# Lacadame/DiffSci

Hardware: AMD Instinct MI355X
Metric: samples/sec (50-step Karras Heun), PUNetG 64ch 128x128 (higher is better)
Workload: dtype f32 (3x3 convs: fp16 hi+lo split, 3 fp16 MFMA products, fp32 accumulate)

## Files before the change

diffsci_amd/_native.py:

```python
import ctypes
import os
from ctypes import POINTER, Structure, c_char_p, c_float, c_int, c_longlong, c_size_t, c_uint32, c_uint64, c_void_p

_HERE = os.path.dirname(os.path.abspath(__file__))
LIB_PATH = os.environ.get("DIFFSCI_HIP_LIB") or os.path.join(_HERE, "_lib", "libdiffsci_hip.so")

ABI_VERSION = 4
DS_IN_NETWORK, DS_IN_SCORE, DS_IN_DRIFT, DS_IN_FLOW = 0, 1, 2, 3
DS_LOAD_PLAIN, DS_LOAD_MAXPOOL2, DS_LOAD_UPSAMPLE2, DS_LOAD_AVGPOOL2 = 0, 1, 2, 3
DS_PAD_CIRCULAR = 16
DS_RES1_UPSAMPLED = 32


class EvalCoef(Structure):
    _fields_ = [("c_out", c_float), ("c_skip", c_float), ("sigma_sq", c_float),
                ("neg_mult", c_float), ("neg_lang", c_float), ("guidance", c_float),
                ("one_minus_guidance", c_float), ("input_kind", c_int), ("stochastic", c_int),
                ("scaled", c_int), ("scale", c_float), ("scale_mult", c_float), ("next_scale", c_float), ("xin_copies", c_int),
                ("nonfinite", c_void_p)]


class NativeLibraryError(RuntimeError):
    pass


_P = c_void_p
_PROTOS = {
    "ds_version": (c_int, []),
    "ds_last_error": (c_char_p, []),
    "ds_device_info": (c_int, [POINTER(c_int), POINTER(c_int), ctypes.c_char_p, c_int]),
    "ds_karras_scale": (c_int, [_P, _P, c_float, c_size_t, _P]),
    "ds_karras_drift": (c_int, [_P, _P, _P, _P, POINTER(EvalCoef), c_size_t, _P]),
    "ds_karras_score": (c_int, [_P, _P, _P, _P, POINTER(EvalCoef), c_size_t, _P]),
    "ds_philox_normal": (c_int, [_P, _P, c_uint64, c_size_t, _P]),
    "ds_karras_euler": (c_int, [_P, _P, _P, _P, _P, POINTER(EvalCoef), c_float, c_float,
                                _P, _P, c_uint64, c_float, c_float, c_size_t, _P]),
    "ds_karras_heun": (c_int, [_P, _P, _P, _P, _P, POINTER(EvalCoef), _P, _P, POINTER(EvalCoef),
                               c_float, c_float, c_size_t, _P]),
    "ds_karras_churn": (c_int, [_P, _P, _P, _P, _P, c_uint64, c_float, c_float, c_float, c_float, c_int, c_size_t, _P]),
    "ds_karras_denoiser": (c_int, [_P, _P, _P, _P, c_float, c_float, _P, _P, c_int, c_size_t, _P]),
    "ds_inorm_silu": (c_int, [_P, _P, _P, _P, c_int, c_int, c_int, c_float, c_int, _P]),
    "ds_conv2d_packed_floats": (c_size_t, [c_int, c_int, c_int]),
    "ds_conv2d_pack_weights": (c_int, [_P, _P, c_int, c_int, c_int, _P]),
    "ds_conv2d": (c_int, [_P, _P, _P, _P, _P, c_int, _P, _P, c_int, c_int, c_int, c_int, c_int,
                          c_int, c_int, _P]),
    "ds_conv2d_x6_packed_bytes": (c_size_t, [c_int, c_int]),
    "ds_conv2d_x6_pack_weights": (c_int, [_P, _P, c_int, c_int, _P]),
    "ds_conv2d_x6": (c_int, [_P, _P, _P, _P, _P, c_int, _P, _P, c_int, c_int, c_int, c_int, c_int, c_int, _P]),
    "ds_conv2d_h3_packed_bytes": (c_size_t, [c_int, c_int]),
    "ds_conv2d_h3_pack_weights": (c_int, [_P, _P, c_int, c_int, c_int, _P]),
    "ds_conv2d_h3": (c_int, [_P, _P, _P, c_int, _P, _P, c_int, _P, _P, c_int, c_int, c_int, c_int, c_int, c_int, _P, _P, _P, _P, _P]),
    "ds_absmax_rows": (c_int, [_P, _P, c_int, c_size_t, c_size_t, _P]),
    "ds_amax_merge": (c_int, [_P, _P, _P, c_int, _P]),
    "ds_absmax_channels": (c_int, [_P, _P, _P, _P, _P, c_int, c_int, c_size_t, c_int, _P]),
    "ds_input_amax": (c_int, [_P, c_int, c_int, _P, _P, _P, c_int, c_int, c_size_t, c_int, _P]),
    "ds_fill_u32": (c_int, [_P, c_uint32, c_size_t, _P]),
    "ds_conv2d_h3_up_supported": (c_int, [c_int, c_int]),
    "ds_conv2d_h3_up_packed_bytes": (c_size_t, [c_int, c_int]),
    "ds_conv2d_h3_up_pack_weights": (c_int, [_P, _P, c_int, c_int, c_int, _P]),
    "ds_conv2d_h3_up": (c_int, [_P, _P, _P, c_int, _P, _P, c_int, _P, _P, c_int, c_int, c_int, c_int, c_int, c_int, _P, _P, _P, _P, _P]),
    "ds_table_apply_images": (c_int, [_P, _P, _P, c_int, c_int, c_int, c_int, _P]),
    "ds_conv2d_h3_up_img": (c_int, [_P, _P, _P, c_int, _P, _P, c_int, _P, _P, c_int, c_int, c_int, c_int, c_int, _P, _P, _P]),
    "ds_conv_tile_count": (c_int, [c_int, c_int]),
    "ds_inorm_table": (c_int, [_P, _P, _P, _P, c_int, c_int, c_int, c_int, c_float, c_int, _P]),
    "ds_gnorm1_table": (c_int, [_P, _P, c_int, c_int, _P, c_int, c_int, _P, _P, _P, _P, c_int, c_int, c_longlong,
                                c_float, c_int, _P]),
    "ds_gnorm1_stats_tiles": (c_int, [_P, _P, c_int, c_int, _P, c_int, c_int, c_int, c_longlong, c_float, c_int, _P]),
    "ds_conv2d_direct": (c_int, [_P, _P, _P, _P, c_int, c_int, c_int, c_int, c_int, c_int, _P]),
    "ds_conv3d_direct": (c_int, [_P, _P, _P, _P, _P, c_int, _P, _P, c_int, c_int, c_int, c_int, c_int, c_int, c_int, _P]),
    "ds_volume_to_slices": (c_int, [_P, _P, c_int, c_int, c_int, c_size_t, c_int, c_int, c_int, _P]),
    "ds_slices_to_volume": (c_int, [_P, _P, _P, _P, c_int, c_int, c_int, c_size_t, c_int, _P]),
    "ds_conv_images_bytes": (c_size_t, [c_int, c_int, c_int, c_int]),
    "ds_inorm_silu_images_supported": (c_int, [c_int, c_int]),
    "ds_inorm_silu_images": (c_int, [_P, _P, _P, _P, c_int, c_int, c_int, c_int, c_float, c_int, _P]),
    "ds_conv2d_h3_img": (c_int, [_P, _P, _P, c_int, _P, _P, c_int, _P, _P, c_int, c_int, c_int, c_int, c_int, c_int, _P, _P, _P]),
    "ds_gnorm1_apply_images": (c_int, [_P, _P, _P, _P, _P, _P, _P, c_int, c_int, c_int, c_int, c_int, c_int, c_int, _P]),
    "ds_volume_stat_tiles": (c_int, [c_int, c_size_t]),
    "ds_volume_to_slices_act": (c_int, [_P, _P, _P, c_int, c_int, c_int, c_size_t, c_int, _P]),
    "ds_wrap_pad_slices": (c_int, [_P, c_int, c_int, c_int, c_size_t, _P]),
    "ds_slices_to_volume_stats": (c_int, [_P, _P, _P, _P, _P, c_int, c_int, c_int, c_size_t, c_int, _P]),
    "ds_slice_tables": (c_int, [_P, _P, _P, _P, c_int, c_int, c_int, c_int, c_longlong, c_float, c_int, c_int, _P]),
    "ds_avgpool3d": (c_int, [_P, _P, c_int, c_int, c_int, c_int, _P]),
    "ds_upsample3d": (c_int, [_P, _P, c_int, c_int, c_int, c_int, _P]),
    "ds_avgpool3d_f": (c_int, [_P, _P, c_int, c_int, c_int, c_int, c_int, _P]),
    "ds_upsample_f": (c_int, [_P, _P, c_int, c_int, c_int, c_int, c_int, c_int, _P]),
    "ds_conv1x1_h3_packed_bytes": (c_size_t, [c_int, c_int]),
    "ds_conv1x1_h3_pack_weights": (c_int, [_P, _P, c_int, c_int, c_int, _P]),
    "ds_conv1x1_h3": (c_int, [_P, _P, _P, c_int, _P, _P, c_int, _P, _P, c_int, c_int, c_int, c_int, c_int, c_int, _P, _P, _P, c_int, _P]),
    "ds_attention": (c_int, [_P, _P, c_int, c_int, c_int, _P]),
    "ds_attention_generic": (c_int, [_P, _P, c_int, c_int, c_int, _P]),
    "ds_attention_h3": (c_int, [_P, _P, c_int, c_int, c_int, _P, _P, _P]),
    "ds_attention_h3_workspace_bytes": (c_size_t, [c_int, c_int, c_int]),
    "ds_attention_h3_ws": (c_int, [_P, _P, _P, c_int, c_int, c_int, _P, _P, _P]),
    "ds_attention_h3_heads_workspace_bytes": (c_size_t, [c_int, c_int, c_int, c_int]),
    "ds_attention_h3_heads": (c_int, [_P, _P, _P, c_int, c_int, c_int, c_int, _P, _P, _P]),
    "ds_attention_heads_generic": (c_int, [_P, _P, c_int, c_int, c_int, c_int, _P]),
    "ds_token_l2_normalize": (c_int, [_P, c_int, c_int, c_int, c_int, c_int, c_float, c_float, _P]),
    "ds_linear": (c_int, [_P, _P, _P, _P, c_int, c_int, c_int, c_int, _P]),
    "ds_fourier_features": (c_int, [_P, _P, _P, _P, c_int, c_int, c_int, _P]),
    "ds_fourier_channels": (c_int, [_P, _P, _P, c_int, c_int, c_int, c_size_t, _P]),
    "ds_gnorm1_workspace_bytes": (c_size_t, [c_int]),
    "ds_gnorm1_stats": (c_int, [_P, _P, _P, c_int, c_int, c_int, c_float, c_int, _P]),
    "ds_gnorm1_apply": (c_int, [_P, _P, _P, _P, _P, _P, _P, c_int, c_int, c_int, c_int, c_int, c_int, c_int, _P]),
    "ds_gnorm1_apply_poolf": (c_int, [_P, _P, _P, _P, _P, _P, _P, c_int, c_int, c_int, c_int, c_int, c_int, c_int, _P]),
    "ds_concat2": (c_int, [_P, _P, _P, c_int, c_size_t, c_size_t, _P]),
    "ds_add_act": (c_int, [_P, _P, _P, c_int, c_int, c_int, c_int, _P]),
    "ds_mask_blend": (c_int, [_P, _P, _P, _P, c_size_t, c_int, _P]),
    "ds_axpby": (c_int, [_P, _P, c_float, _P, c_float, c_size_t, _P]),
    "ds_div_scalar": (c_int, [_P, _P, c_float, c_size_t, _P]),
    "ds_batchnorm_eval": (c_int, [_P, _P, _P, _P, _P, _P, c_float, c_float, c_int, c_int, c_int, c_int, c_size_t, _P]),
    "ds_lerp_stack": (c_int, [_P, _P, _P, c_int, c_size_t, _P]),
    "ds_add": (c_int, [_P, _P, _P, c_size_t, _P]),
    "ds_graph_begin_capture": (c_int, [_P]),
    "ds_graph_end_capture": (c_int, [_P, POINTER(_P), POINTER(c_int)]),
    "ds_graph_launch": (c_int, [_P, _P]),
    "ds_graph_destroy": (c_int, [_P]),
}

_lib = None


def exported_symbols():
    return sorted(_PROTOS)


def lib():
    global _lib
    if _lib is not None:
        return _lib
    if not os.path.exists(LIB_PATH):
        raise NativeLibraryError(
            f"{LIB_PATH} is missing: diffsci_amd has no CPU or PyTorch fallback. "
            "Run `python build.py` (needs hipcc; cross-compiles for gfx950 without a GPU).")
    try:
        L = ctypes.CDLL(LIB_PATH)
    except OSError as e:
        raise NativeLibraryError(f"cannot load {LIB_PATH}: {e}") from e
    for name, (res, args) in _PROTOS.items():
        try:
            fn = getattr(L, name)
        except AttributeError as e:
            raise NativeLibraryError(f"{LIB_PATH} does not export {name}; rebuild with build.py") from e
        fn.restype = res
        fn.argtypes = args
    if L.ds_version() != ABI_VERSION:
        raise NativeLibraryError(f"ABI version {L.ds_version()} != {ABI_VERSION}; rebuild with build.py")
    _lib = L
    return L


def check(rc, what):
    if rc != 0:
        msg = lib().ds_last_error().decode("utf-8", "replace")
        raise RuntimeError(f"{what} failed (status {rc}): {msg}")
```

diffsci_amd/csrc/ds_conv3h.hip:

```cpp
#include "ds_common.h"
#include <cstring>
#include "ds_conv3h_args.h"

#ifdef DS_STAMP
unsigned long long* g_stamps = nullptr;
#define STAMP_SLOTS 16
#define STAMP_AT(slot) a.stamps[((size_t)(blockIdx.z * gridDim.y + blockIdx.y) * gridDim.x + blockIdx.x) * STAMP_SLOTS + (slot)]
#define STAMP(slot) do { if (threadIdx.x == 0) STAMP_AT(slot) = __builtin_amdgcn_s_memrealtime(); } while (0)
#define STAMP_CLK(slot) do { if (threadIdx.x == 0) STAMP_AT(slot) = __builtin_amdgcn_s_memtime(); } while (0)
#define STAMP_PLACE() do { if (threadIdx.x == 0) { STAMP_AT(8) = __builtin_amdgcn_s_getreg((31 << 11) | 4); STAMP_AT(9) = __builtin_amdgcn_s_getreg((31 << 11) | 20); } } while (0)
#else
#define STAMP(slot) do {} while (0)
#define STAMP_CLK(slot) do {} while (0)
#define STAMP_PLACE() do {} while (0)
#endif

namespace {

using namespace ds_conv3;

template <int MT> struct Frags { f16x8 a[2][MT]; f16x8 b[2][2]; };

template <int MODE, bool W16, bool PRE, bool CIRC, int NW, bool S16 = false, bool IMGIN = false, bool TWO = false, bool VEC = false>
__global__ __launch_bounds__(64 * NW, TWO ? 2 : NW / 2) void k_conv3h(const Conv3hArgs a) {
// ... 385 lines not shown
    }
  };

  if constexpr (!IMGIN && !PRE) __builtin_amdgcn_sched_barrier(0);
  const unsigned amax_bits = ds_epi::act_bits((IMGIN || PRE) ? nullptr : a.in_amax, b);
  if constexpr (IMGIN) x_dma(0, 0); else
  x_fetch(0);
  rows_fetch(0);
  const float bias_shift = ds_epi::fetch_bias_shift(a.bias, a.shift, a.shift_stride, b, (cot + (TWO ? (tid >> 7) & 1 : 0)) * COT, a.Cout, COTS);
  w_fetch(0, 0);
  if (n_steps > 1) w_fetch(1, 1);
  STAMP(1);
  if constexpr (!IMGIN && !PRE) __builtin_amdgcn_sched_barrier(0);
  ascale = ds_epi::act_scale_of(PRE ? 0u : amax_bits, a.wshift);
  if constexpr (VEC && PRE) {
    typedef const __attribute__((address_space(4))) f32x4* cptr;
    const float inv0 = ((cptr)(reinterpret_cast<const f32x4*>(pre_b)))[0][3];
    ascale.inv_scale = inv0 == 0.f ? 1.0f : inv0;
    rows_park(0);
    __syncthreads();
  }
  if constexpr (!IMGIN) x_store(0);
  ds_epi::commit_bias_shift(BS, bias_shift, COTS);
  __syncthreads();
  STAMP(2);
  STAMP_CLK(6);

  f32x4 acc16[M16][4];
  if constexpr (S16) {
#pragma unroll
    for (int m = 0; m < M16; ++m)
#pragma unroll
      for (int n = 0; n < 4; ++n)
#pragma unroll
        for (int q = 0; q < 4; ++q) acc16[m][n][q] = 0.f;
    const int i16 = lane & 15, h16 = (lane >> 4) & 1;
    const bool tapB = lane >= 32;
    const int wlane = h16 * COT + i16 + 32 * mh + cw * WSLAB_VEC;
    int xlane[4];
#pragma unroll
    for (int n = 0; n < 4; ++n)
      xlane[n] = h16 * HS + (wave_row + ROWS_PER_R * (n >> 1)) * PW + (W16 ? (n & 1) * PW + i16 : 16 * (n & 1) + i16);
    struct F16 { f16x8 a[2][M16]; f16x8 b[2][4]; };
    auto pair = [&](int slotA, int kyA, int kxA, int xbA, int slotB, int kyB, int kxB, int xbB) __attribute__((always_inline)) {
      const int wofs = (tapB ? slotB * WSV + kxB * 2 * COT : slotA * WSV + kxA * 2 * COT) + wlane;
      const int xofs = tapB ? xbB * XBV + kyB * PW + kxB : xbA * XBV + kyA * PW + kxA;
      F16 f;
#pragma unroll
      for (int p = 0; p < 2; ++p) {
#pragma unroll
        for (int m = 0; m < M16; ++m) f.a[p][m] = *reinterpret_cast<const f16x8*>(&Ws[wofs + p * 6 * COT + 16 * m]);
#pragma unroll
        for (int n = 0; n < 4; ++n) f.b[p][n] = *reinterpret_cast<const f16x8*>(&Xs[xofs + p * PS + xlane[n]]);
      }
      constexpr int PA[3] = {1, 0, 0};
      constexpr int PB[3] = {0, 1, 0};
#pragma unroll
      for (int t = 0; t < 3; ++t)
#pragma unroll
        for (int m = 0; m < M16; ++m)
#pragma unroll
          for (int n = 0; n < 4; ++n)
            acc16[m][n] = __builtin_amdgcn_mfma_f32_16x16x32_f16(f.a[PA[t]][m], f.b[PB[t]][n], acc16[m][n], 0, 0, 0);
    };
    const bool early_stage = a.two_early != 0;
    auto stage_in = [&](int chunk, int ky) __attribute__((always_inline)) {
      const int g = chunk * 3 + ky;
      if (g + 2 < n_steps) w_fetch(g + 2, (ky + 2) % 3);
#ifdef DS_STAMP
      const bool fetch = !a.no_stage;
#else
      constexpr bool fetch = true;
#endif
      if constexpr (IMGIN) {
        if (ky == 0 && chunk + 1 < a.n_chunks) x_dma(chunk + 1, (chunk + 1) & 1);
      } else
      if (fetch && ky == 0 && chunk + 1 < a.n_chunks) { rows_fetch(chunk + 1); x_fetch(chunk + 1); }
      if constexpr (TWO && !IMGIN) {
        if (early_stage && wv < 4 && fetch && ky == 1 && chunk + 1 < a.n_chunks) x_store((chunk & 1) ^ 1);
      }
      __builtin_amdgcn_sched_barrier(0);
    };
    auto stage_out = [&](int chunk, int ky, int xbuf) __attribute__((always_inline)) {
      __builtin_amdgcn_sched_barrier(0);
#ifdef DS_STAMP
      const bool store = a.no_stage != 1;
#else
      constexpr bool store = true;
#endif
      if constexpr (!IMGIN) {
        if (store && ky == 0 && chunk + 1 < a.n_chunks) rows_park(xbuf ^ 1);
        if (store && ky == 1 && chunk + 1 < a.n_chunks && !(TWO && early_stage && wv < 4)) x_store(xbuf ^ 1);
      }
      __syncthreads();
    };
    for (int chunk = 0; chunk < a.n_chunks; chunk += 2) {
      stage_in(chunk, 0);     pair(0, 0, 0, 0, 0, 0, 1, 0); pair(0, 0, 2, 0, 1, 1, 0, 0);   stage_out(chunk, 0, 0);
      stage_in(chunk, 1);     pair(1, 1, 1, 0, 1, 1, 2, 0);                                 stage_out(chunk, 1, 0);
      stage_in(chunk, 2);     pair(2, 2, 0, 0, 2, 2, 1, 0); pair(2, 2, 2, 0, 0, 0, 0, 1);   stage_out(chunk, 2, 0);
      stage_in(chunk + 1, 0); pair(0, 0, 1, 1, 0, 0, 2, 1);                                 stage_out(chunk + 1, 0, 1);
      stage_in(chunk + 1, 1); pair(1, 1, 0, 1, 1, 1, 1, 1); pair(1, 1, 2, 1, 2, 2, 0, 1);   stage_out(chunk + 1, 1, 1);
      stage_in(chunk + 1, 2); pair(2, 2, 1, 1, 2, 2, 2, 1);                                 stage_out(chunk + 1, 2, 1);
    }
  } else {
  FragsT fA, fB;
  frag_load(fA, 0, 0, 0, 0);

  auto step = [&](FragsT& cur, FragsT& oth, int chunk, int ky, int xbuf) __attribute__((always_inline)) {
    const int g = chunk * 3 + ky;
    const int slot = ky;
    const bool more_chunks = chunk + 1 < a.n_chunks;
    if (g + 2 < n_steps) w_fetch(g + 2, (ky + 2) % 3);
    if (ky == 0 && more_chunks) x_fetch(chunk + 1);
    __builtin_amdgcn_sched_barrier(0);
    frag_load(oth, slot, xbuf, ky, 1);
    frag_mma(cur);
    reads_between_mfmas();
    __builtin_amdgcn_sched_barrier(0);
    frag_load(cur, slot, xbuf, ky, 2);
    frag_mma(oth);
    reads_between_mfmas();
    __builtin_amdgcn_sched_barrier(0);
    if (g + 1 < n_steps) {
      const int nky = ky == 2 ? 0 : ky + 1;
      frag_load(oth, nky, ky == 2 ? xbuf ^ 1 : xbuf, nky, 0);
    }
    frag_mma(cur);
    if (g + 1 < n_steps) reads_between_mfmas();
    __builtin_amdgcn_sched_barrier(0);
    if (ky == 1 && more_chunks) x_store(xbuf ^ 1);
    __syncthreads();
  };

  int chunk = 0;
  for (; chunk + 1 < a.n_chunks; chunk += 2) {
    step(fA, fB, chunk, 0, 0);
    step(fB, fA, chunk, 1, 0);
    step(fA, fB, chunk, 2, 0);
    step(fB, fA, chunk + 1, 0, 1);
    step(fA, fB, chunk + 1, 1, 1);
    step(fB, fA, chunk + 1, 2, 1);
  }
  if (chunk < a.n_chunks) {
    step(fA, fB, chunk, 0, 0);
    step(fB, fA, chunk, 1, 0);
    step(fA, fB, chunk, 2, 0);
  }

  }
  STAMP(3);
  STAMP_CLK(7);
  {
    ds_epi::Args e;
    e.out = a.out; e.bias = a.bias; e.shift = a.shift; e.res1 = a.res1; e.res2 = a.res2; e.res1_up = a.res1_up;
    e.unscale = PRE ? ds_epi::unscale_from_inv(ascale.inv_scale, a.wshift) : ds_epi::unscale_from_in(ascale.in_scale, a.wshift);
    e.shift_stride = a.shift_stride;
    e.out_amax = a.out_amax ? a.out_amax + b : nullptr;
    e.b = b; e.co_base = (cot + cw) * COT + 32 * mh; e.y0 = y0 + wave_row; e.x0 = x0;
    e.Cout = a.Cout; e.H = a.H; e.W = a.W;
    e.tile_stats = a.tile_stats; e.tile = ty * a.tiles_x + tx; e.ntiles = a.tiles_x * a.tiles_y;
    constexpr int WTILE = 32 * MT * 2 * 32;
    float* tile = reinterpret_cast<float*>(smem) + wv * WTILE;
    if constexpr (S16) {
      ds_epi::store_tile16<W16, MT>(acc16, tile, BS + 32 * mh + 128 * cw, e);
    } else {
      ds_epi::store_tile<W16, MT>(acc, tile, BS + 32 * mh, e);
    }
    if (a.tile_stats) {
      __syncthreads();
      if constexpr (TWO) {
        if (tid < 128) {
          e.co_base = (cot + (tid >> 6)) * COT;
          ds_epi::store_tile_stats<2>(reinterpret_cast<const float*>(smem) + (tid >> 6) * 4 * WTILE, WTILE, e, tid & 63);
        }
      } else {
        e.co_base = cot * COT;
        ds_epi::store_tile_stats<MT>(reinterpret_cast<const float*>(smem), WTILE, e);
      }
    }
  }
#ifdef DS_STAMP
  STAMP(4);
  asm volatile("s_waitcnt vmcnt(0)" ::: "memory");
  STAMP(5);
#endif
}

__global__ void k_pack3h(_Float16* packed, const float* __restrict__ w, int Cout, int Cin, int n_chunks, float scale,
                         size_t total) {
  size_t i = (size_t)blockIdx.x * blockDim.x + threadIdx.x;
  if (i >= total) return;
  size_t t = i;
  const int c8 = t % 8; t /= 8;
  const int co64 = t % COT; t /= COT;
  const int h = t % 2; t /= 2;
  const int kx = t % 3; t /= 3;
  const int piece = t % 2; t /= 2;
  const int ky = t % 3; t /= 3;
  const int chunk = t % n_chunks; t /= n_chunks;
  const int cot = (int)t;
  const int co = cot * COT + co64, ci = chunk * KC + 8 * h + c8;
  float v = 0.f;
  if (co < Cout && ci < Cin) v = w[((size_t)co * Cin + ci) * 9 + ky * 3 + kx] * scale;
  const _Float16 hi = (_Float16)v;
  const _Float16 lo = (_Float16)(v - (float)hi);
  packed[i] = piece == 0 ? hi : lo;
}

template <int MODE, bool W16, bool PRE, bool CIRC, int NW, bool S16 = false, bool IMGIN = false, bool TWO = false, bool VEC = false>
int launch_conv3h_w(const Conv3hArgs& a, hipStream_t s) {
  constexpr int LDSB = TWO ? LDS_BYTES_TWO : (S16 ? LDS_BYTES16 : LDS_BYTES);
  {
    const int rc = ds::ensure_dynamic_lds<&k_conv3h<MODE, W16, PRE, CIRC, NW, S16, IMGIN, TWO, VEC>>(LDSB, "hipFuncSetAttribute(conv3h)");
    if (rc != DS_OK) return rc;
  }
  const long long tiles = (long long)a.tiles_y * a.tiles_x;
  DS_REQUIRE(tiles > 0 && tiles < 65536 && a.B < 65536, DS_ERR_SHAPE,
             "ds_conv2d_h3: %lld pixel tiles x %d samples exceed the grid limits (65535 each)", tiles, a.B);
  hipLaunchKernelGGL((k_conv3h<MODE, W16, PRE, CIRC, NW, S16, IMGIN, TWO, VEC>), dim3((unsigned)(TWO ? a.n_cot / 2 : a.n_cot), (unsigned)tiles, (unsigned)a.B),
                     dim3(64 * NW), LDSB, s, a);
  DS_CHECK_LAUNCH("ds_conv2d_h3");
  return DS_OK;
}

inline bool conv3h_shape16() {
  static const bool on = [] { const char* e = getenv("DS_CONV_SHAPE"); return !(e && atoi(e) == 32); }();
  return on;
}

inline int conv3h_waves(bool pre) {
  static const int forced = [] { const char* e = getenv("DS_CONV_WAVES"); const int v = e ? atoi(e) : 0; return (v == 4 || v == 8) ? v : 0; }();
  return forced ? forced : (pre ? 8 : 4);
}

inline int conv3h_waves16() {
  static const int v = [] { const char* e = getenv("DS_CONV_WAVES16"); return (e && atoi(e) == 8) ? 8 : 4; }();
  return v;
}

inline int conv3h_two() {
  static const int v = [] { const char* e = getenv("DS_CONV_TWO"); return e ? atoi(e) : 1; }();
  return v;
}
inline long long conv3h_two_min() {
  static const long long v = [] { const char* e = getenv("DS_CONV_TWO_MIN"); return e ? atoll(e) : 256ll; }();
  return v;
}

inline bool conv3h_vec() {
  static const bool on = [] { const char* e = getenv("DS_CONV_VEC"); return !(e && atoi(e) == 0); }();
  return on;
}

template <int MODE, bool W16, bool PRE, bool CIRC>
int launch_conv3h_c(const Conv3hArgs& a, hipStream_t s) {
  bool vec = false;
  if constexpr (MODE == DS_LOAD_PLAIN && !W16)
    vec = conv3h_vec() && a.W % 32 == 0 && a.ox == 0 && a.Cin % KC == 0 && (reinterpret_cast<uintptr_t>(a.in) & 15u) == 0;
  if constexpr (MODE == DS_LOAD_PLAIN) {
    const int two = conv3h_two();
    if (conv3h_shape16() && a.n_chunks % 2 == 0 && a.n_cot % 2 == 0 && ((two == 1 && PRE && a.n_cot == 2 && (long long)a.tiles_y * a.tiles_x * a.B >= conv3h_two_min()) || two == 2)) {
      if constexpr (!W16) { if (vec) return launch_conv3h_w<MODE, W16, PRE, CIRC, 8, true, false, true, true>(a, s); }
      return launch_conv3h_w<MODE, W16, PRE, CIRC, 8, true, false, true>(a, s);
    }
  }
  if (conv3h_shape16() && a.n_chunks % 2 == 0) {
    if constexpr (PRE && MODE == DS_LOAD_PLAIN) {
      if (conv3h_waves16() == 8 && a.n_chunks <= 8) return launch_conv3h_w<MODE, W16, PRE, CIRC, 8, true>(a, s);
    }
    if constexpr (MODE == DS_LOAD_PLAIN && !W16) { if (vec) return launch_conv3h_w<MODE, W16, PRE, CIRC, 4, true, false, false, true>(a, s); }
    return launch_conv3h_w<MODE, W16, PRE, CIRC, 4, true>(a, s);
  }
  if constexpr (MODE == DS_LOAD_MAXPOOL2) return launch_conv3h_w<MODE, W16, PRE, CIRC, 4>(a, s);
  else return conv3h_waves(PRE) == 8 ? launch_conv3h_w<MODE, W16, PRE, CIRC, 8>(a, s) : launch_conv3h_w<MODE, W16, PRE, CIRC, 4>(a, s);
}

template <int MODE, bool W16, bool PRE>
int launch_conv3h(const Conv3hArgs& a, hipStream_t s) {
  return a.circular ? launch_conv3h_c<MODE, W16, PRE, true>(a, s) : launch_conv3h_c<MODE, W16, PRE, false>(a, s);
}

}

extern "C" {

size_t ds_conv2d_h3_packed_bytes(int Cout, int Cin) {
  if (Cout <= 0 || Cin <= 0) return 0;
  const size_t n_cot = (Cout + COT - 1) / COT, n_chunks = (Cin + KC - 1) / KC;
  return n_cot * n_chunks * 3 * (size_t)WSLAB_VEC * 16;
}

int ds_conv2d_h3_pack_weights(void* packed, const float* w, int Cout, int Cin, int wshift, void* stream) {
  DS_REQUIRE(packed && w, DS_ERR_NULL, "ds_conv2d_h3_pack_weights: NULL pointer");
  DS_REQUIRE(Cout > 0 && Cin > 0, DS_ERR_SHAPE, "ds_conv2d_h3_pack_weights: Cout=%d Cin=%d", Cout, Cin);
  DS_REQUIRE(wshift >= -40 && wshift <= 40, DS_ERR_SHAPE, "ds_conv2d_h3_pack_weights: wshift %d out of range", wshift);
  const int n_chunks = (Cin + KC - 1) / KC;
  const size_t total = ds_conv2d_h3_packed_bytes(Cout, Cin) / 2;
  hipLaunchKernelGGL(k_pack3h, dim3((unsigned)((total + 255) / 256)), dim3(256), 0, ds::as_stream(stream),
                     reinterpret_cast<_Float16*>(packed), w, Cout, Cin, n_chunks, ldexpf(1.0f, wshift), total);
  DS_CHECK_LAUNCH("ds_conv2d_h3_pack_weights");
  return DS_OK;
}

int ds_conv2d_h3(float* out, const float* in, const void* w_packed, int wshift, const float* bias, const float* shift,
                 int shift_stride, const float* res1, const float* res2, int B, int Cin, int Cout, int H, int W,
                 int load_mode, const float* prenorm, float* tile_stats, const unsigned* in_amax, unsigned* out_amax,
                 void* stream) {
  DS_REQUIRE(out && in && w_packed, DS_ERR_NULL, "ds_conv2d_h3: NULL pointer");
  DS_REQUIRE(!(prenorm && in_amax), DS_ERR_UNSUPPORTED, "ds_conv2d_h3: in_amax is for raw inputs (with prenorm the table's fourth column carries the exponent)");
  DS_REQUIRE(B >= 0 && Cin > 0 && Cout > 0 && H > 0 && W > 0, DS_ERR_SHAPE,
             "ds_conv2d_h3: bad shape B=%d Cin=%d Cout=%d H=%d W=%d", B, Cin, Cout, H, W);
  const int circular = (load_mode & DS_PAD_CIRCULAR) ? 1 : 0;
  const int res1_up = (load_mode & DS_RES1_UPSAMPLED) ? 1 : 0;
  const int oy = (int)((load_mode >> 8) & 15) - (((load_mode >> 8) & 8) ? 16 : 0);
  const int ox = (int)((load_mode >> 12) & 15) - (((load_mode >> 12) & 8) ? 16 : 0);
  load_mode &= ~(DS_PAD_CIRCULAR | DS_RES1_UPSAMPLED | 0xff00);
  DS_REQUIRE(!circular || (H >= (oy < 0 ? -oy : oy) + 1 && W >= (ox < 0 ? -ox : ox) + 1), DS_ERR_SHAPE,
             "ds_conv2d_h3: periodic padding with tap offset (%d, %d) needs a field at least as large as the window's reach (%d x %d)", oy, ox, H, W);
  DS_REQUIRE(!res1_up || (res1 && H % 2 == 0 && W % 2 == 0), DS_ERR_SHAPE, "ds_conv2d_h3: RES1_UPSAMPLED needs res1 and even H, W");
  DS_REQUIRE(load_mode >= 0 && load_mode <= 2, DS_ERR_UNSUPPORTED, "ds_conv2d_h3: load_mode %d", load_mode);
  DS_REQUIRE(load_mode != DS_LOAD_UPSAMPLE2 || (H % 2 == 0 && W % 2 == 0), DS_ERR_SHAPE,
             "ds_conv2d_h3: UPSAMPLE2 needs even output H, W (got %d x %d)", H, W);
  DS_REQUIRE(shift == nullptr || shift_stride == 0 || shift_stride >= Cout, DS_ERR_SHAPE,
             "ds_conv2d_h3: shift_stride %d < Cout %d", shift_stride, Cout);
  DS_REQUIRE((reinterpret_cast<uintptr_t>(w_packed) & 15u) == 0, DS_ERR_SHAPE, "ds_conv2d_h3: w_packed must be 16-byte aligned");
  DS_REQUIRE(load_mode != DS_LOAD_MAXPOOL2 || (reinterpret_cast<uintptr_t>(in) & 7u) == 0, DS_ERR_SHAPE,
             "ds_conv2d_h3: MAXPOOL2 input must be 8-byte aligned");
  DS_REQUIRE(wshift >= -40 && wshift <= 40, DS_ERR_SHAPE, "ds_conv2d_h3: wshift %d out of range", wshift);
  DS_REQUIRE(prenorm == nullptr || load_mode != DS_LOAD_MAXPOOL2, DS_ERR_UNSUPPORTED,
             "ds_conv2d_h3: prenorm cannot be combined with the max-pool load (pooling follows the activation)");
  DS_REQUIRE((reinterpret_cast<uintptr_t>(prenorm) & 15u) == 0, DS_ERR_SHAPE, "ds_conv2d_h3: prenorm must be 16-byte aligned");
  if (B == 0) return DS_OK;
  Conv3hArgs a;
  a.prenorm = prenorm; a.tile_stats = tile_stats; a.circular = circular; a.res1_up = res1_up; a.oy = oy; a.ox = ox;
  a.ntiles_magic40 = 0; a.ncot_magic40 = 0; a.pc_prio = 0; a.pc_skew_mask = 0;
  {
    static const int early = [] { const char* e = getenv("DS_CONV_TWO_EARLY"); return e ? atoi(e) : 1; }();
    a.two_early = early;
  }
  a.out = out; a.in = in; a.wp = reinterpret_cast<const u32x4*>(w_packed); a.bias = bias; a.shift = shift;
  a.res1 = res1; a.res2 = res2; a.shift_stride = shift_stride;
  a.wshift = wshift; a.in_amax = in_amax; a.out_amax = out_amax;
  a.B = B; a.Cin = Cin; a.Cout = Cout; a.H = H; a.W = W;
  a.Hin = load_mode == DS_LOAD_MAXPOOL2 ? 2 * H : (load_mode == DS_LOAD_UPSAMPLE2 ? H / 2 : H);
  a.Win = load_mode == DS_LOAD_MAXPOOL2 ? 2 * W : (load_mode == DS_LOAD_UPSAMPLE2 ? W / 2 : W);
  DS_REQUIRE((long long)Cin * a.Hin * a.Win < (1ll << 31), DS_ERR_SHAPE, "ds_conv2d_h3: per-sample input exceeds 2^31 floats");
  const long long pad32 = (long long)((W + 31) / 32 * 32) * ((H + 7) / 8 * 8);
  const long long pad16 = (long long)((W + 15) / 16 * 16) * ((H + 15) / 16 * 16);
  const bool w16 = pad16 < pad32;
  const int TW = w16 ? 16 : 32, TH = w16 ? 16 : 8;
  a.tiles_x = (W + TW - 1) / TW; a.tiles_y = (H + TH - 1) / TH;
  a.n_cot = (Cout + COT - 1) / COT;
  a.n_chunks = (Cin + KC - 1) / KC;
  a.tiles_x_magic = a.tiles_x == 1 ? 0u : (unsigned)((1ull << 32) / (unsigned)a.tiles_x) + 1u;
#ifdef DS_STAMP
  {
    static const struct Stg { unsigned ticks = 0, lo = 256, hi = 512; Stg() { const char* e = getenv("DS_CONV_STAGGER"); if (e) sscanf(e, "%u,%u,%u", &ticks, &lo, &hi); } } stg;
    a.stagger_ticks = stg.ticks; a.stagger_lo = stg.lo; a.stagger_hi = stg.hi;
    static const unsigned nostage = [] { const char* e = getenv("DS_CONV_NOSTAGE"); return e ? (unsigned)atoi(e) : 0u; }();
    a.no_stage = nostage;
  }
#endif
#ifdef DS_STAMP
  a.stamps = g_stamps;
#endif
  hipStream_t s = ds::as_stream(stream);
  if (!w16 && load_mode == DS_LOAD_PLAIN && conv3h_shape16()) {
    bool launched = false;
    const int rc = conv3p_try_launch(a, s, &launched);
    if (rc != DS_OK || launched) return rc;
  }
#define DS_L3(M, W) (prenorm ? launch_conv3h<M, W, true>(a, s) : launch_conv3h<M, W, false>(a, s))
  if (w16) {
    if (load_mode == DS_LOAD_PLAIN) return DS_L3(DS_LOAD_PLAIN, true);
    if (load_mode == DS_LOAD_MAXPOOL2) return launch_conv3h<DS_LOAD_MAXPOOL2, true, false>(a, s);
    return DS_L3(DS_LOAD_UPSAMPLE2, true);
  }
  if (load_mode == DS_LOAD_PLAIN) return DS_L3(DS_LOAD_PLAIN, false);
  if (load_mode == DS_LOAD_MAXPOOL2) return launch_conv3h<DS_LOAD_MAXPOOL2, false, false>(a, s);
  return DS_L3(DS_LOAD_UPSAMPLE2, false);
#undef DS_L3
}

size_t ds_conv_images_bytes(int B, int C, int H, int W) {
  if (B <= 0 || C <= 0 || H <= 0 || W <= 0) return 0;
  return (size_t)B * ((C + KC - 1) / KC) * 4 * (size_t)(H + 2) * (W + 2) * 16;
}

int ds_conv2d_h3_img(float* out, const void* images, const void* w_packed, int wshift, const float* bias, const float* shift,
                     int shift_stride, const float* res1, const float* res2, int B, int Cin, int Cout, int H, int W,
                     int flags, float* tile_stats, unsigned* out_amax, void* stream) {
  DS_REQUIRE(out && images && w_packed, DS_ERR_NULL, "ds_conv2d_h3_img: NULL pointer");
  DS_REQUIRE((flags & ~DS_RES1_UPSAMPLED) == 0, DS_ERR_UNSUPPORTED, "ds_conv2d_h3_img: flags %d (DS_RES1_UPSAMPLED only)", flags);
  DS_REQUIRE(!(flags & DS_RES1_UPSAMPLED) || (res1 && H % 2 == 0 && W % 2 == 0 && (reinterpret_cast<uintptr_t>(res1) & 7u) == 0),
             DS_ERR_SHAPE, "ds_conv2d_h3_img: RES1_UPSAMPLED needs res1 [B, Cout, H/2, W/2] (8-byte aligned) and even H, W");
  DS_REQUIRE(B >= 0 && Cin > 0 && Cout > 0 && H > 0 && W > 0, DS_ERR_SHAPE,
             "ds_conv2d_h3_img: bad shape B=%d Cin=%d Cout=%d H=%d W=%d", B, Cin, Cout, H, W);
  DS_REQUIRE(((Cin + KC - 1) / KC) % 2 == 0, DS_ERR_UNSUPPORTED,
             "ds_conv2d_h3_img: the image-input kernel is the 16x16x32 variant: an even number of 16-channel chunks (Cin = %d)", Cin);
  DS_REQUIRE(shift == nullptr || shift_stride == 0 || shift_stride >= Cout, DS_ERR_SHAPE,
             "ds_conv2d_h3_img: shift_stride %d < Cout %d", shift_stride, Cout);
  DS_REQUIRE((reinterpret_cast<uintptr_t>(w_packed) & 15u) == 0 && (reinterpret_cast<uintptr_t>(images) & 15u) == 0, DS_ERR_SHAPE,
             "ds_conv2d_h3_img: images and w_packed must be 16-byte aligned");
  DS_REQUIRE(wshift >= -40 && wshift <= 40, DS_ERR_SHAPE, "ds_conv2d_h3_img: wshift %d out of range", wshift);
  DS_REQUIRE((long long)4 * (H + 2) * (W + 2) < (1ll << 27), DS_ERR_SHAPE, "ds_conv2d_h3_img: image planes too large");
  if (B == 0) return DS_OK;
  Conv3hArgs a;
  memset(&a, 0, sizeof(a));
  a.out = out; a.in = reinterpret_cast<const float*>(images); a.wp = reinterpret_cast<const u32x4*>(w_packed);
  a.bias = bias; a.shift = shift; a.res1 = res1; a.res2 = res2; a.shift_stride = shift_stride; a.tile_stats = tile_stats;
  a.res1_up = (flags & DS_RES1_UPSAMPLED) ? 1 : 0;
  a.wshift = wshift; a.out_amax = out_amax;
  a.B = B; a.Cin = Cin; a.Cout = Cout; a.H = H; a.W = W; a.Hin = H; a.Win = W;
  const long long pad32 = (long long)((W + 31) / 32 * 32) * ((H + 7) / 8 * 8);
  const long long pad16 = (long long)((W + 15) / 16 * 16) * ((H + 15) / 16 * 16);
  const bool w16 = pad16 < pad32;
  const int TW = w16 ? 16 : 32, TH = w16 ? 16 : 8;
  a.tiles_x = (W + TW - 1) / TW; a.tiles_y = (H + TH - 1) / TH;
  a.n_cot = (Cout + COT - 1) / COT;
  a.n_chunks = (Cin + KC - 1) / KC;
  a.tiles_x_magic = a.tiles_x == 1 ? 0u : (unsigned)((1ull << 32) / (unsigned)a.tiles_x) + 1u;
#ifdef DS_STAMP
  a.stamps = g_stamps;
#endif
  hipStream_t s = ds::as_stream(stream);
  if (!w16) {
    bool launched = false;
    const int rc = conv3p_try_launch_img(a, s, &launched);
    if (rc != DS_OK || launched) return rc;
  }
  return w16 ? launch_conv3h_w<DS_LOAD_PLAIN, true, false, false, 4, true, true>(a, s)
             : launch_conv3h_w<DS_LOAD_PLAIN, false, false, false, 4, true, true>(a, s);
}

}
```

diffsci_amd/csrc/ds_conv3h_args.h:

```cpp
#pragma once
#include "ds_common.h"
#include "ds_conv_epilogue.h"
#include "ds_h3_common.h"

namespace ds_conv3 {

using ds_epi::f32x16;
using ds_epi::f32x4;
using ds_h3::u32x4;
using ds_h3::f16x8;
using ds_h3::split2;
using ds_h3::fast_silu;

constexpr int COT = 64, NT = 256;
constexpr int KC = 16;
template <bool W16> struct Geo {
  static constexpr int TH = W16 ? 16 : 8, TW = W16 ? 16 : 32;
  static constexpr int PH = TH + 2, PW = TW + 2, NPOS = PH * PW;
  static constexpr int XITEMS = 2 * NPOS;
  static constexpr int XBUF_VEC = 2 * 2 * NPOS;
};
constexpr int XBUF_VEC = Geo<false>::XBUF_VEC;
constexpr int HPAD16 = 12;
constexpr int XBUF_VEC16 = XBUF_VEC + 2 * HPAD16;
constexpr int WSLAB_VEC = 2 * 3 * 2 * COT;
constexpr int WPIECES = WSLAB_VEC / 64;
constexpr int STAGE_BYTES = (2 * XBUF_VEC + 3 * WSLAB_VEC) * 16;
constexpr int LDS_BYTES = STAGE_BYTES + 128 * 4;
constexpr int STAGE_BYTES16 = (2 * XBUF_VEC16 + 3 * WSLAB_VEC) * 16;
constexpr int LDS_BYTES16 = STAGE_BYTES16 + 128 * 4;
static_assert(2 * LDS_BYTES16 <= 160 * 1024, "two workgroups per CU");
constexpr int TWO_STAGE_BYTES = (2 * XBUF_VEC16 + 3 * 2 * WSLAB_VEC) * 16;
constexpr int TWO_EPI_BYTES = 8 * 64 * 2 * 32 * 4;
static_assert(TWO_EPI_BYTES >= TWO_STAGE_BYTES, "bias / shift rows behind the larger of the two");
constexpr int LDS_BYTES_TWO = TWO_EPI_BYTES + 2 * 128 * 4;

struct Conv3hArgs {
  float* out;
  const float* in;
  const u32x4* wp;
  const float* bias;
  const float* shift;
  const float* res1;
  const float* res2;
  const float* prenorm;
  float* tile_stats;
  const unsigned* in_amax;
  unsigned* out_amax;
  int wshift;
  int shift_stride;
  int res1_up;
  int circular;
  int oy, ox;
  int B, Cin, Cout, H, W, Hin, Win;
  int tiles_x, tiles_y, n_cot, n_chunks;
  unsigned tiles_x_magic;
  unsigned long long ntiles_magic40, ncot_magic40;
  int pc_prio;
  int pc_skew_mask;
  int two_early;
#ifdef DS_STAMP
  unsigned long long* stamps;
  unsigned stagger_lo, stagger_hi, stagger_ticks;
  unsigned no_stage;
#endif
};


int conv3p_try_launch(const Conv3hArgs& a, hipStream_t s, bool* launched);
int conv3p_try_launch_img(const Conv3hArgs& a, hipStream_t s, bool* launched);

}
```

diffsci_amd/csrc/ds_conv3p.hip:

```cpp
#include "ds_conv3h_args.h"

#include <atomic>
#include <cstdlib>
#include <type_traits>

namespace ds_conv3 {
namespace {

constexpr int P_WOFF = 2 * XBUF_VEC16 * 16;
constexpr int P_WSLOTS = 4;
constexpr int P_OUTOFF = P_WOFF + P_WSLOTS * WSLAB_VEC * 16;
constexpr int P_BSOFF = P_OUTOFF + 4 * 16384;
constexpr int P_BS_FLOATS = 132;
constexpr int P_LDS = P_BSOFF + 2 * P_BS_FLOATS * 4;
static_assert(P_LDS <= 160 * 1024, "one workgroup per CU");

#ifdef DS_STAMP
#define PSTAMP_SLOTS 64
#define PSTAMP(slot) do { if (a.stamps && (wv == 0 || wv == 4) && lane == 0 && (slot) < PSTAMP_SLOTS) a.stamps[((size_t)blockIdx.x * 2 + (wv >> 2)) * PSTAMP_SLOTS + (slot)] = __builtin_amdgcn_s_memtime(); } while (0)
#else
#define PSTAMP(slot) do {} while (0)
#endif
#ifdef DS_STAMP
#define PSTAMP_FINE(k) do { if (it == 1 && last_of_item) PSTAMP(48 + (k)); } while (0)
#else
#define PSTAMP_FINE(k) do {} while (0)
#endif

#define DS_VMCNT_CASE(n) case n: asm volatile("s_waitcnt vmcnt(" #n ")" ::: "memory"); break;
__device__ __forceinline__ void bar_counted(int young) {
  const int y = __builtin_amdgcn_readfirstlane(young);
  switch (y < 63 ? y : 63) {
    DS_VMCNT_CASE(0) DS_VMCNT_CASE(1) DS_VMCNT_CASE(2) DS_VMCNT_CASE(3) DS_VMCNT_CASE(4) DS_VMCNT_CASE(5) DS_VMCNT_CASE(6) DS_VMCNT_CASE(7)
    DS_VMCNT_CASE(8) DS_VMCNT_CASE(9) DS_VMCNT_CASE(10) DS_VMCNT_CASE(11) DS_VMCNT_CASE(12) DS_VMCNT_CASE(13) DS_VMCNT_CASE(14) DS_VMCNT_CASE(15)
    DS_VMCNT_CASE(16) DS_VMCNT_CASE(17) DS_VMCNT_CASE(18) DS_VMCNT_CASE(19) DS_VMCNT_CASE(20) DS_VMCNT_CASE(21) DS_VMCNT_CASE(22) DS_VMCNT_CASE(23)
    DS_VMCNT_CASE(24) DS_VMCNT_CASE(25) DS_VMCNT_CASE(26) DS_VMCNT_CASE(27) DS_VMCNT_CASE(28) DS_VMCNT_CASE(29) DS_VMCNT_CASE(30) DS_VMCNT_CASE(31)
    DS_VMCNT_CASE(32) DS_VMCNT_CASE(33) DS_VMCNT_CASE(34) DS_VMCNT_CASE(35) DS_VMCNT_CASE(36) DS_VMCNT_CASE(37) DS_VMCNT_CASE(38) DS_VMCNT_CASE(39)
    DS_VMCNT_CASE(40) DS_VMCNT_CASE(41) DS_VMCNT_CASE(42) DS_VMCNT_CASE(43) DS_VMCNT_CASE(44) DS_VMCNT_CASE(45) DS_VMCNT_CASE(46) DS_VMCNT_CASE(47)
    DS_VMCNT_CASE(48) DS_VMCNT_CASE(49) DS_VMCNT_CASE(50) DS_VMCNT_CASE(51) DS_VMCNT_CASE(52) DS_VMCNT_CASE(53) DS_VMCNT_CASE(54) DS_VMCNT_CASE(55)
    DS_VMCNT_CASE(56) DS_VMCNT_CASE(57) DS_VMCNT_CASE(58) DS_VMCNT_CASE(59) DS_VMCNT_CASE(60) DS_VMCNT_CASE(61) DS_VMCNT_CASE(62)
    default: asm volatile("s_waitcnt vmcnt(63)" ::: "memory"); break;
  }
  asm volatile("s_waitcnt lgkmcnt(0)\n\ts_barrier" ::: "memory");
}
#undef DS_VMCNT_CASE

struct Item { int cot, b, y0, x0, tile; };
#ifndef DS_PC_FETCH_LATE
#define DS_PC_FETCH_LATE 0
#endif
#ifndef DS_PC_SPREAD
#define DS_PC_SPREAD 1
#endif
#ifndef DS_PC_IMG_CDMA
#define DS_PC_IMG_CDMA 0
#endif
#ifndef DS_PC_CDMA
#define DS_PC_CDMA 1
#endif
#define DS_LPI 8

template <int XI> struct Packed { u32x4 h[XI], l[XI]; };
template <int BK> struct ResRegs { f32x4 r1[BK], r2[BK]; };
struct Frag { f16x8 a[2][4], b[2][4]; };

__device__ __forceinline__ void lds_dma16(const void* gsrc, unsigned lane_bytes, unsigned lds) {
  asm volatile("s_mov_b32 m0, %0\n\ts_nop 0\n\tglobal_load_lds_dwordx4 %1, %2" : : "s"(lds), "v"(lane_bytes), "s"(gsrc) : "memory", "m0");
}
__device__ __forceinline__ unsigned lds_address(const void* p) {
  return (unsigned)(unsigned long long)(const __attribute__((address_space(3))) void*)p;
}
__device__ __forceinline__ unsigned const_u32(const void* p, size_t i) {
  typedef const __attribute__((address_space(4))) unsigned* cptr;
  return ((cptr)p)[i];
}

template <bool PRE, bool CIRC, int NRES, int NPW, bool VEC = false, bool IMG = false>
__global__ __launch_bounds__(256 + 64 * NPW, NPW == 4 ? 2 : 3) void k_conv3p(const Conv3hArgs a) {
  static_assert(NPW == 4 || NPW == 8, "four or eight producer waves");
  static_assert(!VEC || NPW == 4, "16-byte patch loads: the four-producer form");
  static_assert(!IMG || (!PRE && !CIRC && !VEC && NPW == 4), "image input: plain zero-padded four-producer form");
  constexpr int XI = NPW == 4 ? 3 : 2;
  constexpr int BK = NPW == 4 ? 4 : 2;
  using Packed = ds_conv3::Packed<XI>;
  using ResRegs = ds_conv3::ResRegs<BK>;
  constexpr int PW = Geo<false>::PW, NPOS = Geo<false>::NPOS;
  constexpr int HS = NPOS + HPAD16, PS = 2 * NPOS + HPAD16, XBV = XBUF_VEC16;
  extern __shared__ __attribute__((aligned(16))) unsigned char smem[];
  u32x4* Xs = reinterpret_cast<u32x4*>(smem);
  u32x4* Ws = reinterpret_cast<u32x4*>(smem + P_WOFF);
  float* OUT = reinterpret_cast<float*>(smem + P_OUTOFF);
  float* BS = reinterpret_cast<float*>(smem + P_BSOFF);
  const int tid = threadIdx.x, lane = tid & 63;
  const int wv = __builtin_amdgcn_readfirstlane(tid >> 6);
  const bool consumer = wv < 4;
  const int rw = wv & 3;
  const int ptid = tid - 256;
  const int pw = wv - 4;
  const int rws = NPW == 4 ? rw : ((pw >> 1) & 3);
  const int joff = NPW == 4 ? 0 : 8 * (pw & 1);

  const unsigned ntiles = (unsigned)(a.tiles_x * a.tiles_y);
  const unsigned total = (unsigned)a.n_cot * ntiles * (unsigned)a.B;
  const unsigned Q = gridDim.x >> 3, xcd = blockIdx.x & 7u, q = blockIdx.x >> 3;
  const unsigned per = total >> 3, rem = total & 7u;
  const unsigned first = xcd * per + (xcd < rem ? xcd : rem), cnt = per + (xcd < rem ? 1u : 0u);
  const int n_items = q < cnt ? (int)((cnt - q + Q - 1) / Q) : 0;
  if (n_items == 0) return;
  auto div40 = [](unsigned n, unsigned long long magic) __attribute__((always_inline)) { return (unsigned)(((unsigned long long)n * magic) >> 40); };
  auto item_of = [&](int k) __attribute__((always_inline)) {
    const unsigned logical = first + q + Q * (unsigned)k;
    Item it;
    const unsigned rest = div40(logical, a.ncot_magic40);
    it.cot = (int)(logical - rest * (unsigned)a.n_cot);
    const unsigned bb = div40(rest, a.ntiles_magic40);
    it.tile = (int)(rest - bb * ntiles);
    it.b = (int)bb;
    const int ty = a.tiles_x == 1 ? it.tile : (int)__umulhi((unsigned)it.tile, a.tiles_x_magic);
    const int tx = it.tile - ty * a.tiles_x;
    it.y0 = 8 * ty; it.x0 = 32 * tx;
    return it;
  };
  const int n_chunks = a.n_chunks, n_steps = 3 * n_chunks;
  const int HW = a.H * a.W;

  f32x4 acc[4][4];
  const int i16 = lane & 15, h16 = (lane >> 4) & 1, g16 = lane >> 4;
  const bool tapB = lane >= 32;
  const int wlane = h16 * COT + i16;
  int xlane[4];
#pragma unroll
  for (int n = 0; n < 4; ++n) xlane[n] = h16 * HS + (2 * rw + (n >> 1)) * PW + 16 * (n & 1) + i16;
  auto load_pair = [&](Frag& f, int slotA, int kyA, int kxA, int xbA, int slotB, int kyB, int kxB, int xbB) __attribute__((always_inline)) {
    const int wofs = (tapB ? slotB * WSLAB_VEC + kxB * 2 * COT : slotA * WSLAB_VEC + kxA * 2 * COT) + wlane;
    const int xofs = tapB ? xbB * XBV + kyB * PW + kxB : xbA * XBV + kyA * PW + kxA;
#pragma unroll
    for (int p = 0; p < 2; ++p) {
#pragma unroll
      for (int m = 0; m < 4; ++m) f.a[p][m] = *reinterpret_cast<const f16x8*>(&Ws[wofs + p * 6 * COT + 16 * m]);
#pragma unroll
      for (int n = 0; n < 4; ++n) f.b[p][n] = *reinterpret_cast<const f16x8*>(&Xs[xofs + p * PS + xlane[n]]);
    }
  };
  auto mma_pair = [&](const Frag& f) __attribute__((always_inline)) {
    constexpr int PA[3] = {1, 0, 0};
    constexpr int PB[3] = {0, 1, 0};
#pragma unroll
    for (int t = 0; t < 3; ++t)
#pragma unroll
      for (int m = 0; m < 4; ++m)
#pragma unroll
        for (int n = 0; n < 4; ++n)
          acc[m][n] = __builtin_amdgcn_mfma_f32_16x16x32_f16(f.a[PA[t]][m], f.b[PB[t]][n], acc[m][n], 0, 0, 0);
  };
  auto reads_between = [&]() __attribute__((always_inline)) {
    __builtin_amdgcn_sched_group_barrier(0x008, 16, 0);
#pragma unroll
    for (int i = 0; i < 16; ++i) {
      __builtin_amdgcn_sched_group_barrier(0x008, 1, 0);
      __builtin_amdgcn_sched_group_barrier(0x100, 1, 0);
    }
    __builtin_amdgcn_sched_group_barrier(0x008, 16, 0);
  };
  auto park_tile = [&](int par) __attribute__((always_inline)) {
    const float* bs = BS + par * P_BS_FLOATS;
    float* tile = OUT + rw * 4096;
    const float unscale = bs[128];
    float bsv[4][4];
#pragma unroll
    for (int m = 0; m < 4; ++m)
#pragma unroll
      for (int e = 0; e < 4; ++e) {
        const int co = 16 * m + 4 * g16 + e;
        bsv[m][e] = bs[co] + bs[64 + co];
      }
    __builtin_amdgcn_sched_barrier(0);
#pragma unroll
    for (int m = 0; m < 4; ++m)
#pragma unroll
      for (int e = 0; e < 4; ++e) {
        const int co = 16 * m + 4 * g16 + e;
#pragma unroll
        for (int n = 0; n < 4; ++n) {
          tile[(co * 2 + (n >> 1)) * 32 + 16 * (n & 1) + i16] = __builtin_fmaf(acc[m][n][e], unscale, bsv[m][e]);
          acc[m][n][e] = 0.f;
        }
      }
  };

  const int tail_h = (rw >> 1) & 1;
  auto item_h = [&](int i) __attribute__((always_inline)) { return NPW == 8 ? ((pw >> 2) & 1) : (i == 0 ? 0 : (i == 1 ? 1 : tail_h)); };
  int xlds[XI], xrow[XI], xcol[XI];
  const bool live_tail = NPW == 4 ? (NT + (ptid & (NT / 2 - 1)) < NPOS) : (lane < 21);
  auto live = [&](int i) __attribute__((always_inline)) { return i < XI - 1 || live_tail; };
#pragma unroll
  for (int i = 0; i < XI; ++i) {
    int pos;
    if (NPW == 4) pos = i < 2 ? (ptid & 255) : NT + (ptid & (NT / 2 - 1));
    else pos = i == 0 ? 64 * (pw & 3) + lane : 256 + 21 * (pw & 3) + (lane < 21 ? lane : 20);
    xrow[i] = pos / PW;
    xcol[i] = pos - xrow[i] * PW;
    xlds[i] = item_h(i) * HS + pos;
  }
  int vr[XI], vx[XI], vch[XI], vlds[XI], vrow[XI];
  const bool halo_live = lane < 20;
  if constexpr (VEC) {
#pragma unroll
    for (int i = 0; i < XI; ++i) {
      vr[i] = 0; vx[i] = 0; vch[i] = 0; vlds[i] = 0; vrow[i] = 0;
      if (i < XI - 1 || pw < 2) {
        const int u = i * 256 + (ptid & 255);
        const int q = u & 3, G = u >> 5;
        const int h = G >= 10 ? 1 : 0, Gp = G - 10 * h;
        int r, g;
        if (Gp < 8) { r = 4 * (Gp >> 2) + ((u >> 3) & 3); g = 2 * (Gp & 3) + ((u >> 2) & 1); }
        else { r = 8 + ((u >> 3) & 1); g = 4 * (Gp - 8) + 2 * ((u >> 4) & 1) + ((u >> 2) & 1); }
        vr[i] = r; vx[i] = 4 * g;
        vch[i] = (8 * h + 2 * q) * HW;
        vlds[i] = 16 * (h * HS + r * PW + 1 + 4 * g) + 4 * q;
        vrow[i] = 8 * h + 2 * q;
      } else {
        const int e = halo_live ? lane : 19, h = pw - 2;
        vr[i] = e >> 1; vx[i] = (e & 1) ? PW - 2 : -1;
        vch[i] = 8 * h * HW;
        vlds[i] = 16 * (h * HS + vr[i] * PW + vx[i] + 1);
        vrow[i] = 8 * h;
      }
    }
  }
  auto pad_vec = [&](int c) __attribute__((always_inline)) { return c < HPAD16 ? NPOS + c : PS + NPOS + (c - HPAD16); };
  constexpr int NINST = (XBV + 63) / 64;
  const int Wp = a.W + 2, Hp = a.H + 2;
  unsigned dbase[6] = {};
  if constexpr (IMG) {
#pragma unroll
    for (int i = 0; i < 6; ++i) {
      const int k = pw + 4 * i;
      const int L = (k < NINST - 1 ? 64 * k : XBV - 64) + lane;
      const int piece = L >= PS ? 1 : 0, Lp = L - piece * PS;
      const int hh = Lp >= HS ? 1 : 0;
      int pos = Lp - hh * HS;
      pos = pos < NPOS ? pos : NPOS - 1;
      const int r = pos / PW, col = pos - r * PW;
      dbase[i] = 16u * (unsigned)(((2 * piece + hh) * Hp + r) * Wp + col);
    }
  }
  int i_k = 0, i_chunk = 0, i_b = 0;
  unsigned i_off = 0;
  auto xdma = [&](int buf) __attribute__((always_inline)) {
    const bool valid = i_k < n_items;
    if (valid && i_chunk == 0) { const Item it = item_of(i_k); i_off = 16u * (unsigned)(it.y0 * Wp + it.x0); i_b = it.b; }
    const u32x4* src = reinterpret_cast<const u32x4*>(a.in) + ((size_t)i_b * n_chunks + i_chunk) * 4 * (size_t)(Hp * Wp);
    u32x4* dst = Xs + buf * XBV;
    int n = 0;
#pragma unroll
    for (int i = 0; i < 6; ++i) {
      const int k = pw + 4 * i;
      if (k < NINST) { lds_dma16(src, dbase[i] + i_off, lds_address(dst + (k < NINST - 1 ? 64 * k : XBV - 64))); ++n; }
    }
    if (valid && ++i_chunk == n_chunks) { i_chunk = 0; ++i_k; }
    return n;
  };
  int f_k = 0, f_chunk = 0, f_b = 0;
  int xoff[XI] = {};
  unsigned f_xvalid = 0;
  float f_in_scale = 1.f;
  auto plan_fetch = [&](const Item& it) __attribute__((always_inline)) {
    f_xvalid = 0;
    if constexpr (VEC) {
#pragma unroll
      for (int i = 0; i < XI; ++i) {
        const bool halo = i == XI - 1 && pw >= 2;
        int gy = it.y0 + vr[i] - 1 + a.oy, gx = it.x0 + vx[i];
        if (CIRC) {
          gy = gy < 0 ? gy + a.H : (gy >= a.H ? gy - a.H : gy);
          gx = gx < 0 ? gx + a.W : (gx >= a.W ? gx - a.W : gx);
          gy = gy >= a.H ? a.H - 1 : gy;
        }
        const bool ok = (!halo || halo_live) && gy >= 0 && gy < a.H && gx >= 0 && gx < a.W;
        xoff[i] = ok ? gy * a.W + gx : 0;
        if (ok) f_xvalid |= 1u << i;
      }
      f_b = it.b;
      if constexpr (!PRE) f_in_scale = ds_epi::act_scale_of(a.in_amax ? const_u32(a.in_amax, it.b) : 0u, a.wshift).in_scale;
      return;
    }
#pragma unroll
    for (int i = 0; i < XI; ++i) {
      int gy = it.y0 + xrow[i] - 1 + a.oy, gx = it.x0 + xcol[i] - 1 + a.ox;
      if (CIRC) {
        gy = gy < 0 ? gy + a.H : (gy >= a.H ? gy - a.H : gy);
        gx = gx < 0 ? gx + a.W : (gx >= a.W ? gx - a.W : gx);
        gy = gy >= a.H ? a.H - 1 : gy;
        gx = gx >= a.W ? a.W - 1 : gx;
      }
      const bool ok = live(i) && gy >= 0 && gy < a.H && gx >= 0 && gx < a.W;
      xoff[i] = ok ? gy * a.W + gx : 0;
      if (ok) f_xvalid |= 1u << i;
    }
    f_b = it.b;
    if constexpr (!PRE) f_in_scale = ds_epi::act_scale_of(a.in_amax ? const_u32(a.in_amax, it.b) : 0u, a.wshift).in_scale;
  };
  const float* f_src = a.in;
  auto fetch_begin = [&](unsigned& tag, int& trow, float& tscale) __attribute__((always_inline)) {
    const bool valid = f_k < n_items;
    if (valid && f_chunk == 0) plan_fetch(item_of(f_k));
    tag = valid ? (0x80000000u | f_xvalid) : 0u;
    trow = (f_b * n_chunks + f_chunk) * KC;
    tscale = f_in_scale;
    f_src = a.in + ((size_t)f_b * a.Cin + (size_t)f_chunk * KC) * HW;
    if (valid && ++f_chunk == n_chunks) { f_chunk = 0; ++f_k; }
  };
  auto fetch_item = [&](auto halo_tag, float (&xr)[XI][8], int i) __attribute__((always_inline)) {
    constexpr bool HALO = decltype(halo_tag)::value;
    if constexpr (VEC) {
      const float* p0 = f_src + vch[i] + xoff[i];
      if (HALO && i == XI - 1) {
#pragma unroll
        for (int k = 0; k < 8; ++k) xr[i][k] = p0[(size_t)k * HW];
      } else {
        const f32x4 t0 = *reinterpret_cast<const f32x4*>(p0);
        const f32x4 t1 = *reinterpret_cast<const f32x4*>(p0 + HW);
#pragma unroll
        for (int k = 0; k < 4; ++k) { xr[i][k] = t0[k]; xr[i][4 + k] = t1[k]; }
      }
    } else {
      const float* p0 = f_src + xoff[i] + (size_t)(8 * item_h(i)) * HW;
#pragma unroll
      for (int k = 0; k < 8; ++k) xr[i][k] = p0[(size_t)k * HW];
    }
  };
  auto fetch_count = [&](auto halo_tag) __attribute__((always_inline)) {
    constexpr bool HALO = decltype(halo_tag)::value;
    return VEC ? (PRE ? 1 : 0) + (HALO ? 2 * (XI - 1) + 8 : 2 * XI) : DS_LPI * XI;
  };
  auto rows_fetch = [&](f32x4& prow, int trow) __attribute__((always_inline)) {
    if constexpr (VEC && PRE) prow = reinterpret_cast<const f32x4*>(a.prenorm)[trow + (lane & 15)];
  };
  auto rows_park = [&](const f32x4& prow, int buf) __attribute__((always_inline)) {
    if constexpr (VEC && PRE) {
      if (pw == 0 && lane < 16) Xs[buf * XBV + pad_vec(lane)] = __builtin_bit_cast(u32x4, prow);
    }
  };
  auto fetch = [&](auto halo_tag, float (&xr)[XI][8], f32x4& prow, unsigned& tag, int& trow, float& tscale) __attribute__((always_inline)) {
    fetch_begin(tag, trow, tscale);
    rows_fetch(prow, trow);
#pragma unroll
    for (int i = 0; i < XI; ++i) fetch_item(halo_tag, xr, i);
    return fetch_count(halo_tag);
  };
  auto activate_item = [&](auto halo_tag, float (&xr)[XI][8], unsigned tag, int trow, float tscale, Packed& pk, int i, int buf) __attribute__((always_inline)) {
    constexpr bool HALO = decltype(halo_tag)::value;
    if constexpr (VEC) {
      if (!(HALO && i == XI - 1)) {
        if constexpr (PRE) {
          const u32x4* rows = Xs + buf * XBV;
          const f32x4 p0 = __builtin_bit_cast(f32x4, rows[pad_vec(vrow[i])]);
          const f32x4 p1 = __builtin_bit_cast(f32x4, rows[pad_vec(vrow[i] + 1)]);
          const float inv = p0[3] == 0.f ? 1.0f : p0[3];
#pragma unroll
          for (int k = 0; k < 4; ++k) {
            xr[i][k] = ds_h3::fast_silu_scaled((xr[i][k] - p0[0]) * p0[1] + p0[2], inv);
            xr[i][4 + k] = ds_h3::fast_silu_scaled((xr[i][4 + k] - p1[0]) * p1[1] + p1[2], inv);
          }
        }
        const bool item_ok = (tag >> i) & 1u;
#pragma unroll
        for (int k = 0; k < 4; ++k) {
          float v0 = item_ok ? xr[i][k] : 0.f;
          float v1 = item_ok ? xr[i][4 + k] : 0.f;
          if constexpr (!PRE) { v0 *= tscale; v1 *= tscale; }
          unsigned ph, pl;
          split2(v0, v1, ph, pl);
          pk.h[i][k] = ph; pk.l[i][k] = pl;
        }
        return;
      }
    }
    if constexpr (PRE) {
      typedef const __attribute__((address_space(4))) f32x4* cptr;
      cptr pp = (cptr)(reinterpret_cast<const f32x4*>(a.prenorm)) + trow;
      const int h = VEC ? pw - 2 : item_h(i);
      f32x4 p[8];
#pragma unroll
      for (int k = 0; k < 8; ++k) p[k] = pp[8 * h + k];
      const float inv = p[0][3] == 0.f ? 1.0f : p[0][3];
#pragma unroll
      for (int k = 0; k < 8; ++k) xr[i][k] = ds_h3::fast_silu_scaled((xr[i][k] - p[k][0]) * p[k][1] + p[k][2], inv);
    }
    const bool item_ok = (tag >> i) & 1u;
#pragma unroll
    for (int k = 0; k < 4; ++k) {
      float v0 = item_ok ? xr[i][2 * k] : 0.f;
      float v1 = item_ok ? xr[i][2 * k + 1] : 0.f;
      if constexpr (!PRE) { v0 *= tscale; v1 *= tscale; }
      unsigned ph, pl;
      split2(v0, v1, ph, pl);
      pk.h[i][k] = ph; pk.l[i][k] = pl;
    }
  };
  auto activate = [&](auto halo_tag, float (&xr)[XI][8], unsigned tag, int trow, float tscale, Packed& pk, int buf) __attribute__((always_inline)) {
#pragma unroll
    for (int i = 0; i < XI; ++i) activate_item(halo_tag, xr, tag, trow, tscale, pk, i, buf);
  };
  auto activate_first_slots = [&](auto halo_tag, float (&xr)[XI][8], unsigned tag, int trow, float tscale, Packed& pk, int buf) __attribute__((always_inline)) {
#pragma unroll
    for (int i = 0; i < XI - 1; ++i) activate_item(halo_tag, xr, tag, trow, tscale, pk, i, buf);
  };
  auto fetch_beside_last_slot = [&](auto halo_tag, float (&xn)[XI][8], f32x4& prown, unsigned& tagn, int& trown, float& tscn,
                                    float (&xo)[XI][8], unsigned tago, int trowo, float tsco, Packed& pk, int bufo) __attribute__((always_inline)) {
#if DS_PC_FETCH_LATE == 1
    activate_item(halo_tag, xo, tago, trowo, tsco, pk, XI - 1, bufo);
    __builtin_amdgcn_sched_barrier(0);
    fetch_begin(tagn, trown, tscn);
    rows_fetch(prown, trown);
#pragma unroll
    for (int i = 0; i < XI; ++i) fetch_item(halo_tag, xn, i);
#elif DS_PC_FETCH_LATE == 2
    fetch_begin(tagn, trown, tscn);
    rows_fetch(prown, trown);
#pragma unroll
    for (int i = 0; i < XI; ++i) fetch_item(halo_tag, xn, i);
    __builtin_amdgcn_sched_barrier(0);
    activate_item(halo_tag, xo, tago, trowo, tsco, pk, XI - 1, bufo);
#else
    fetch_begin(tagn, trown, tscn);
    rows_fetch(prown, trown);
#pragma unroll
    for (int i = 0; i < XI - 1; ++i) fetch_item(halo_tag, xn, i);
    __builtin_amdgcn_sched_barrier(0);
    activate_item(halo_tag, xo, tago, trowo, tsco, pk, XI - 1, bufo);
    __builtin_amdgcn_sched_barrier(0);
    fetch_item(halo_tag, xn, XI - 1);
#endif
    return fetch_count(halo_tag);
  };
  auto store_x = [&](auto halo_tag, const Packed& pk, unsigned tag, int buf) __attribute__((always_inline)) {
    constexpr bool HALO = decltype(halo_tag)::value;
    if (!(tag >> 31)) return;
    if constexpr (VEC) {
      unsigned char* xbytes = smem + (size_t)buf * XBV * 16;
#pragma unroll
      for (int i = 0; i < XI; ++i) {
        if (HALO && i == XI - 1) {
          if (halo_live) {
            *reinterpret_cast<u32x4*>(xbytes + vlds[i]) = pk.h[i];
            *reinterpret_cast<u32x4*>(xbytes + vlds[i] + PS * 16) = pk.l[i];
          }
        } else {
#pragma unroll
          for (int k = 0; k < 4; ++k) {
            *reinterpret_cast<unsigned*>(xbytes + vlds[i] + 16 * k) = pk.h[i][k];
            *reinterpret_cast<unsigned*>(xbytes + vlds[i] + 16 * k + PS * 16) = pk.l[i][k];
          }
        }
      }
      return;
    }
    u32x4* xb = Xs + buf * XBV;
#pragma unroll
    for (int i = 0; i < XI; ++i) {
      if (live(i)) {
        xb[xlds[i]] = pk.h[i];
        xb[PS + xlds[i]] = pk.l[i];
      }
    }
  };
  int w_k = 0, w_step = 0, w_cot = 0;
  constexpr bool cdma = DS_PC_CDMA != 0 && (!IMG || DS_PC_IMG_CDMA != 0);
  auto wdma = [&](int slot, int widx, int nwv) __attribute__((always_inline)) {
    const bool valid = w_k < n_items;
    if (valid && w_step == 0) w_cot = item_of(w_k).cot;
    const u32x4* src = a.wp + ((size_t)w_cot * n_steps + w_step) * WSLAB_VEC;
    u32x4* dst = Ws + slot * WSLAB_VEC;
#pragma unroll
    for (int i = 0; i < 3; ++i) {
      const int k = widx + nwv * i;
      if (k < 12) lds_dma16(src + 64 * k, 16u * (unsigned)lane, lds_address(dst + 64 * k));
    }
    if (valid && ++w_step == n_steps) { w_step = 0; ++w_k; }
    return 0;
  };
  auto bs_fetch = [&](const Item& it, float& vb, float& vs) __attribute__((always_inline)) {
    const int co = it.cot * COT + (ptid & 63);
    vb = a.bias ? a.bias[co] : 0.f;
    vs = a.shift ? a.shift[(size_t)it.b * a.shift_stride + co] : 0.f;
  };
  auto unscale_of = [&](const Item& it) __attribute__((always_inline)) {
    if constexpr (PRE) {
      const float inv = __builtin_bit_cast(float, const_u32(a.prenorm, (size_t)it.b * n_chunks * KC * 4 + 3));
      return ds_epi::unscale_from_inv(inv == 0.f ? 1.0f : inv, a.wshift);
    } else {
      return ds_epi::act_scale_of(a.in_amax ? const_u32(a.in_amax, it.b) : 0u, a.wshift).unscale;
    }
  };
  auto bs_commit = [&](float vb, float vs, float unscale, int par) __attribute__((always_inline)) {
    if (ptid < 128) BS[par * P_BS_FLOATS + ptid] = ptid < 64 ? vb : vs;
    else if (ptid == 128) BS[par * P_BS_FLOATS + 128] = unscale;
  };

  int s_b = 0, s_cot = 0, s_tile = 0;
  f32x4 pend0[BK];
  size_t s_idx = 0;
  const size_t s_step = 4 * (size_t)HW;
  float s_amax = 0.f;
  const int p4 = 4 * (lane & 7);
  const bool stats = a.tile_stats != nullptr, want_amax = a.out_amax != nullptr;
  constexpr int nres = BK * NRES;
  auto plan_store = [&](const Item& it) __attribute__((always_inline)) {
    s_b = it.b; s_cot = it.cot; s_tile = it.tile;
    const int gy = it.y0 + 2 * rws + ((lane >> 3) & 1), gx = it.x0 + p4;
    const size_t ch = (size_t)it.b * a.Cout + it.cot * COT + 4 * joff + (lane >> 4);
    s_idx = ch * HW + (size_t)gy * a.W + gx;
    s_amax = 0.f;
  };
  auto res_prefetch = [&](ResRegs& R, int half) __attribute__((always_inline)) {
#pragma unroll
    for (int k = 0; k < BK; ++k) {
      const int j = half * BK + k;
      if constexpr (NRES >= 1) R.r1[k] = *reinterpret_cast<const f32x4*>(a.res1 + s_idx + (size_t)j * s_step);
      if constexpr (NRES >= 2) R.r2[k] = *reinterpret_cast<const f32x4*>(a.res2 + s_idx + (size_t)j * s_step);
    }
    return nres;
  };
  auto store_batch = [&](const ResRegs& R, int half) __attribute__((always_inline)) {
    float* tile = OUT + rws * 4096;
    f32x4 v[BK];
#pragma unroll
    for (int k = 0; k < BK; ++k) {
      const int seg = (joff + half * BK + k) * 8 + (lane >> 3);
      v[k] = *reinterpret_cast<const f32x4*>(&tile[seg * 32 + p4]);
    }
    if constexpr (NRES >= 1) {
#pragma unroll
      for (int k = 0; k < BK; ++k) v[k] = v[k] + R.r1[k];
    }
    if constexpr (NRES >= 2) {
#pragma unroll
      for (int k = 0; k < BK; ++k) v[k] = v[k] + R.r2[k];
    }
#pragma unroll
    for (int k = 0; k < BK; ++k) *reinterpret_cast<f32x4*>(a.out + s_idx + (size_t)(half * BK + k) * s_step) = v[k];
    if (want_amax) {
#pragma unroll
      for (int k = 0; k < BK; ++k) s_amax = fmaxf(s_amax, ds_epi::abs_max4(v[k]));
    }
    if (stats) {
      f32x4 o[BK];
#pragma unroll
      for (int k = 0; k < BK; ++k) {
        const float K = ds_epi::row16_first(v[k].x);
        const f32x4 d = v[k] - K;
        const float sv = ds_epi::row16_sum((d.x + d.y) + (d.z + d.w));
        const float qv = ds_epi::row16_sum((d.x * d.x + d.y * d.y) + (d.z * d.z + d.w * d.w));
        o[k] = f32x4{K, sv, qv, 64.f};
      }
      if (NPW == 8 && half == 0) {
#pragma unroll
        for (int k = 0; k < BK; ++k) pend0[k] = o[k];
      } else if ((lane & 15) == 0) {
        if (NPW == 8 && half == 1) {
#pragma unroll
          for (int k = 0; k < BK; ++k) *reinterpret_cast<f32x4*>(&tile[4 * (4 * (joff + k) + (lane >> 4))]) = pend0[k];
        }
#pragma unroll
        for (int k = 0; k < BK; ++k) *reinterpret_cast<f32x4*>(&tile[4 * (4 * (joff + half * BK + k) + (lane >> 4))]) = o[k];
      }
    }
    return BK;
  };
  auto commit_amax_asm = [&]() __attribute__((always_inline)) {
    float m = s_amax;
#pragma unroll
    for (int o = 32; o > 0; o >>= 1) m = fmaxf(m, __shfl_xor(m, o, 64));
    if (lane == 0) atomicMax(a.out_amax + s_b, __builtin_bit_cast(unsigned, m));
  };
  auto store_stats = [&]() __attribute__((always_inline)) {
    const float* tiles = OUT;
    f32x4 pw[4];
#pragma unroll
    for (int w = 0; w < 4; ++w) pw[w] = *reinterpret_cast<const f32x4*>(&tiles[w * 4096 + 4 * lane]);
    const float K = pw[0][0];
    float S = 0.f, Qs = 0.f, n = 0.f;
#pragma unroll
    for (int w = 0; w < 4; ++w) {
      const float dk = pw[w][3] > 0.f ? pw[w][0] - K : 0.f;
      S += pw[w][1] + pw[w][3] * dk;
      Qs += pw[w][2] + 2.f * dk * pw[w][1] + pw[w][3] * dk * dk;
      n += pw[w][3];
    }
    *reinterpret_cast<f32x4*>(a.tile_stats + (((size_t)s_b * a.Cout + s_cot * COT + lane) * ntiles + s_tile) * 4) = f32x4{K, S, Qs, n};
  };

  float xrA[XI][8], xrB[XI][8];
  unsigned tagA = 0, tagB = 0, tagP = 0;
  int trowA = 0, trowB = 0;
  float tscA = 1.f, tscB = 1.f;
  Packed pk;
  f32x4 prowA = {0.f, 0.f, 0.f, 0.f}, prowB = {0.f, 0.f, 0.f, 0.f};
  ResRegs RA, RB;
  float bsb = 0.f, bss = 0.f;
  Frag F0, F1;

  auto run = [&](auto role_tag) __attribute__((always_inline)) {
    constexpr int ROLE = decltype(role_tag)::value;
    constexpr bool CONS = ROLE == 0;
    const std::integral_constant<bool, ROLE == 2> halo{};
    int young = 0, prev = 0, nx = 0;
    const int ndma = NPW == 4 ? 3 : (pw < 4 ? 2 : 1);
    auto barrier = [&]() __attribute__((always_inline)) {
      if constexpr (CONS) bar_counted(cdma ? 3 : 0);
      else {
        if constexpr (IMG) bar_counted(prev + nx + (cdma ? 0 : ndma) + young);
        else bar_counted(cdma ? 63 : prev + ndma + young);
        prev = young; young = 0; nx = 0;
      }
    };
    int stamp = 1;
    (void)stamp;
    constexpr bool SPREAD = DS_PC_SPREAD != 0;
    auto chunk_pair = [&](auto base_tag, Frag& Fa, Frag& Fb, bool head, bool second, bool last_of_item, int it) __attribute__((always_inline)) {
      constexpr int B = decltype(base_tag)::value;
      constexpr int E0 = (B + 0) & 3, E1 = (B + 1) & 3, E2 = (B + 2) & 3;
      constexpr int O0 = (B + 3) & 3, O1 = (B + 4) & 3, O2 = (B + 5) & 3;
      constexpr int N0 = (B + 6) & 3;
      constexpr int G[10][8] = {{E0, 0, 0, 0, E0, 0, 1, 0}, {E0, 0, 2, 0, E1, 1, 0, 0}, {E1, 1, 1, 0, E1, 1, 2, 0}, {E2, 2, 0, 0, E2, 2, 1, 0},
                                {E2, 2, 2, 0, O0, 0, 0, 1}, {O0, 0, 1, 1, O0, 0, 2, 1}, {O1, 1, 0, 1, O1, 1, 1, 1}, {O1, 1, 2, 1, O2, 2, 0, 1},
                                {O2, 2, 1, 1, O2, 2, 2, 1}, {N0, 0, 0, 0, N0, 0, 1, 0}};
      auto group = [&](auto k_tag) __attribute__((always_inline)) {
        constexpr int k = decltype(k_tag)::value;
        if constexpr (NPW == 4) {
          Frag& cur = (k & 1) ? Fb : Fa;
          Frag& nxt = (k & 1) ? Fa : Fb;
          load_pair(nxt, G[k + 1][0], G[k + 1][1], G[k + 1][2], G[k + 1][3], G[k + 1][4], G[k + 1][5], G[k + 1][6], G[k + 1][7]);
          mma_pair(cur);
          reads_between();
        } else {
          load_pair(Fa, G[k][0], G[k][1], G[k][2], G[k][3], G[k][4], G[k][5], G[k][6], G[k][7]);
          mma_pair(Fa);
        }
      };
#define DS_GROUP(k) group(std::integral_constant<int, k>{})
      if constexpr (CONS) {
        if (cdma) { wdma((B + 3) & 3, rw, 4); __builtin_amdgcn_sched_barrier(0); }
        if (head) park_tile((it - 1) & 1);
        DS_GROUP(0); DS_GROUP(1);
      } else {
        if constexpr (IMG) nx = xdma(1);
        if (!cdma) wdma((B + 3) & 3, pw, NPW);
        __builtin_amdgcn_sched_barrier(0);
        if (head) { plan_store(item_of(it - 1)); young += res_prefetch(RA, 0); }
        if constexpr (!IMG) {
          young += fetch_beside_last_slot(halo, xrB, prowB, tagB, trowB, tscB, xrA, tagA, trowA, tscA, pk, 1);
          tagP = tagA;
        }
      }
      if (stamp < 48) PSTAMP(stamp);
      ++stamp;
      barrier();
      if constexpr (CONS) {
        if (cdma) { wdma((B + 4) & 3, rw, 4); __builtin_amdgcn_sched_barrier(0); }
        DS_GROUP(2);
      } else {
        if (!cdma) wdma((B + 4) & 3, pw, NPW);
        __builtin_amdgcn_sched_barrier(0);
        if constexpr (!IMG) {
          store_x(halo, pk, tagP, 1);
          rows_park(prowB, 0);
        }
        if (head) {
          young += store_batch(RA, 0);
          young += res_prefetch(RB, 1);
        }
        if constexpr (SPREAD) {
          if (second) { young += store_batch(RA, 2); young += res_prefetch(RB, 3); }
        }
      }
      if (stamp < 48) PSTAMP(stamp);
      ++stamp;
      barrier();
      if constexpr (CONS) {
        if (cdma) { wdma((B + 5) & 3, rw, 4); __builtin_amdgcn_sched_barrier(0); }
        DS_GROUP(3); DS_GROUP(4);
      } else {
        if (!cdma) wdma((B + 5) & 3, pw, NPW);
        __builtin_amdgcn_sched_barrier(0);
        if constexpr (!IMG) activate_first_slots(halo, xrB, tagB, trowB, tscB, pk, 0);
        __builtin_amdgcn_sched_barrier(0);
        if constexpr (!SPREAD) {
          if (head) {
            young += store_batch(RB, 1);
            young += res_prefetch(RA, 2);
          }
        }
      }
      if (stamp < 48) PSTAMP(stamp);
      ++stamp;
      barrier();
      if constexpr (CONS) {
        if (cdma) { wdma((B + 6) & 3, rw, 4); __builtin_amdgcn_sched_barrier(0); }
        DS_GROUP(5);
      } else {
        PSTAMP_FINE(0);
        if constexpr (IMG) nx = xdma(0);
        if (!cdma) wdma((B + 6) & 3, pw, NPW);
        __builtin_amdgcn_sched_barrier(0);
        PSTAMP_FINE(1);
        if constexpr (!IMG) young += fetch_beside_last_slot(halo, xrA, prowA, tagA, trowA, tscA, xrB, tagB, trowB, tscB, pk, 0);
        __builtin_amdgcn_sched_barrier(0);
        PSTAMP_FINE(2);
        if constexpr (!SPREAD) {
          if (head) {
            young += store_batch(RA, 2);
            young += res_prefetch(RB, 3);
          }
        }
        if (last_of_item && it + 1 < n_items) bs_fetch(item_of(it + 1), bsb, bss);
      }
      if (stamp < 48) PSTAMP(stamp);
      ++stamp;
      barrier();
      if constexpr (CONS) {
        if (cdma) { wdma((B + 7) & 3, rw, 4); __builtin_amdgcn_sched_barrier(0); }
        DS_GROUP(6); DS_GROUP(7);
      } else {
        PSTAMP_FINE(4);
        if (!cdma) wdma((B + 7) & 3, pw, NPW);
        __builtin_amdgcn_sched_barrier(0);
        PSTAMP_FINE(5);
        if constexpr (!IMG) {
          store_x(halo, pk, tagB, 0);
          rows_park(prowA, 1);
        }
        PSTAMP_FINE(6);
        if constexpr (SPREAD) {
          if (head) { young += store_batch(RB, 1); young += res_prefetch(RA, 2); }
          if (second) { young += store_batch(RB, 3); if (want_amax) commit_amax_asm(); }
        } else {
          if (head) {
            young += store_batch(RB, 3);
            if (want_amax) commit_amax_asm();
          }
        }
      }
      if (stamp < 48) PSTAMP(stamp);
      ++stamp;
      barrier();
      if constexpr (CONS) {
        if (cdma) { wdma((B + 8) & 3, rw, 4); __builtin_amdgcn_sched_barrier(0); }
        DS_GROUP(8);
      } else {
        if (!cdma) wdma((B + 8) & 3, pw, NPW);
        __builtin_amdgcn_sched_barrier(0);
        if constexpr (!IMG) activate_first_slots(halo, xrA, tagA, trowA, tscA, pk, 1);
        __builtin_amdgcn_sched_barrier(0);
        if ((SPREAD ? second : head) && stats && wv == 4) store_stats();
        if (last_of_item && it + 1 < n_items) bs_commit(bsb, bss, unscale_of(item_of(it + 1)), (it + 1) & 1);
      }
      if (stamp < 48) PSTAMP(stamp);
      ++stamp;
      barrier();
#undef DS_GROUP
    };

    {
      const unsigned skew = (blockIdx.x * 11u) & (unsigned)a.pc_skew_mask;
      for (unsigned i = 0; i < skew; ++i) __builtin_amdgcn_s_sleep(8);
    }
    if constexpr (!CONS) {
      if constexpr (IMG) xdma(0);
      if (!cdma) { wdma(0, pw, NPW); wdma(1, pw, NPW); wdma(2, pw, NPW); }
      if constexpr (!IMG) {
        fetch(halo, xrB, prowB, tagB, trowB, tscB);
        fetch(halo, xrA, prowA, tagA, trowA, tscA);
      }
      bs_fetch(item_of(0), bsb, bss);
      if constexpr (VEC && PRE) {
        asm volatile("s_waitcnt vmcnt(0)" ::: "memory");
        rows_park(prowB, 0);
        rows_park(prowA, 1);
        asm volatile("s_waitcnt lgkmcnt(0)\n\ts_barrier" ::: "memory");
      }
      if constexpr (!IMG) {
        activate(halo, xrB, tagB, trowB, tscB, pk, 0);
        store_x(halo, pk, tagB, 0);
        activate_first_slots(halo, xrA, tagA, trowA, tscA, pk, 1);
      }
      bs_commit(bsb, bss, unscale_of(item_of(0)), 0);
      if constexpr (VEC || IMG) asm volatile("s_waitcnt vmcnt(0)" ::: "memory");
      else asm volatile("s_waitcnt vmcnt(20)" ::: "memory");
    } else {
      if (cdma) { wdma(0, rw, 4); wdma(1, rw, 4); wdma(2, rw, 4); }
      if constexpr (VEC && PRE) asm volatile("s_waitcnt lgkmcnt(0)\n\ts_barrier" ::: "memory");
#pragma unroll
      for (int m = 0; m < 4; ++m)
#pragma unroll
        for (int n = 0; n < 4; ++n)
#pragma unroll
          for (int e = 0; e < 4; ++e) acc[m][n][e] = 0.f;
    }
    PSTAMP(0);
    if constexpr (CONS) asm volatile("s_waitcnt vmcnt(0)" ::: "memory");
    asm volatile("s_waitcnt lgkmcnt(0)\n\ts_barrier" ::: "memory");
    young = 0; prev = (VEC || IMG) ? 0 : DS_LPI * XI;
    if constexpr (CONS && NPW == 4) load_pair(F0, 0, 0, 0, 0, 0, 0, 1, 0);

    const int ncp = n_chunks >> 1;
    for (int it = 0; it < n_items; ++it) {
      for (int cp = 0; cp < ncp; cp += 2) {
        chunk_pair(std::integral_constant<int, 0>{}, F0, F1, cp == 0 && it > 0, false, false, it);
        if constexpr (NPW == 4) chunk_pair(std::integral_constant<int, 6>{}, F1, F0, false, cp == 0 && it > 0, cp + 2 == ncp, it);
        else chunk_pair(std::integral_constant<int, 6>{}, F0, F1, false, cp == 0 && it > 0, cp + 2 == ncp, it);
      }
    }
    if constexpr (CONS) {
      park_tile((n_items - 1) & 1);
    } else {
      plan_store(item_of(n_items - 1));
      res_prefetch(RA, 0);
    }
    bar_counted(0);
    if constexpr (!CONS) {
      store_batch(RA, 0);
      res_prefetch(RB, 1);
    }
    bar_counted(0);
    if constexpr (!CONS) {
      store_batch(RB, 1);
      res_prefetch(RA, 2);
      store_batch(RA, 2);
      res_prefetch(RB, 3);
      store_batch(RB, 3);
      if (want_amax) commit_amax_asm();
    }
    bar_counted(0);
    if constexpr (!CONS) {
      if (stats && wv == 4) store_stats();
    }
  };
  if (consumer) {
    run(std::integral_constant<int, 0>{});
  } else {
    if (a.pc_prio == 1) __builtin_amdgcn_s_setprio(1);
    else if (a.pc_prio == 2) __builtin_amdgcn_s_setprio(2);
    else if (a.pc_prio == 3) __builtin_amdgcn_s_setprio(3);
    if (VEC && pw >= 2) run(std::integral_constant<int, VEC ? 2 : 1>{});
    else run(std::integral_constant<int, 1>{});
  }
}

int conv3p_producer_waves() {
  static const int v = [] { const char* e = getenv("DS_CONV_PC_WAVES"); const int n = e ? atoi(e) : 4; return n == 8 ? 8 : 4; }();
  return v;
}

template <bool PRE, bool CIRC, int NRES, int NPW, bool VEC = false, bool IMG = false>
int launch_conv3p_w(const Conv3hArgs& a, int wgs, hipStream_t s) {
  const int rc = ds::ensure_dynamic_lds<&k_conv3p<PRE, CIRC, NRES, NPW, VEC, IMG>>(P_LDS, "hipFuncSetAttribute(conv3p)");
  if (rc != DS_OK) return rc;
  hipLaunchKernelGGL((k_conv3p<PRE, CIRC, NRES, NPW, VEC, IMG>), dim3((unsigned)wgs), dim3(256 + 64 * NPW), P_LDS, s, a);
  DS_CHECK_LAUNCH("ds_conv2d_h3 (persistent)");
  return DS_OK;
}
bool conv3p_vec() {
  static const bool on = [] { const char* e = getenv("DS_CONV_VEC"); return !(e && atoi(e) == 0); }();
  return on;
}
template <bool PRE, bool CIRC, int NRES>
int launch_conv3p_r(const Conv3hArgs& a, int wgs, hipStream_t s) {
  if (conv3p_producer_waves() == 8) return launch_conv3p_w<PRE, CIRC, NRES, 8>(a, wgs, s);
  if (conv3p_vec() && a.ox == 0 && (reinterpret_cast<uintptr_t>(a.in) & 15u) == 0) return launch_conv3p_w<PRE, CIRC, NRES, 4, true>(a, wgs, s);
  return launch_conv3p_w<PRE, CIRC, NRES, 4>(a, wgs, s);
}
void conv3p_fill_args(Conv3hArgs& a) {
  a.ntiles_magic40 = (1ull << 40) / (unsigned long long)(a.tiles_x * a.tiles_y) + 1ull;
  a.ncot_magic40 = (1ull << 40) / (unsigned long long)a.n_cot + 1ull;
  static const int prio = [] { const char* e = getenv("DS_CONV_PC_PRIO"); const int v = e ? atoi(e) : 0; return v < 0 || v > 3 ? 0 : v; }();
  a.pc_prio = prio;
  static const int skew = [] { const char* e = getenv("DS_CONV_PC_SKEW"); const int v = e ? atoi(e) : 0; return v < 0 || v > 31 ? 0 : v; }();
  a.pc_skew_mask = skew;
  if (!a.res1 && a.res2) { a.res1 = a.res2; a.res2 = nullptr; }
}
template <bool PRE, bool CIRC>
int launch_conv3p(Conv3hArgs a, int wgs, hipStream_t s) {
  conv3p_fill_args(a);
  if (!a.res1) return launch_conv3p_r<PRE, CIRC, 0>(a, wgs, s);
  return a.res2 ? launch_conv3p_r<PRE, CIRC, 2>(a, wgs, s) : launch_conv3p_r<PRE, CIRC, 1>(a, wgs, s);
}

int conv3p_mode() {
  static const int v = [] { const char* e = getenv("DS_CONV_PC"); return e ? atoi(e) : 2; }();
  return v;
}
int conv3p_min_items() {
  static const int v = [] { const char* e = getenv("DS_CONV_PC_MIN"); const int n = e ? atoi(e) : 1; return n < 1 ? 1 : n; }();
  return v;
}
int conv3p_cus() {
  static std::atomic<int> cus[64];
  int dev = 0;
  if (hipGetDevice(&dev) != hipSuccess) return 256;
  int c = cus[dev & 63].load(std::memory_order_acquire);
  if (c == 0) {
    hipDeviceProp_t p;
    c = hipGetDeviceProperties(&p, dev) == hipSuccess ? p.multiProcessorCount : 256;
    cus[dev & 63].store(c, std::memory_order_release);
  }
  return c;
}

}

int conv3p_try_launch_img(const Conv3hArgs& a0, hipStream_t s, bool* launched) {
  *launched = false;
  static const bool on = [] { const char* e = getenv("DS_CONV_PC_IMG"); return !(e && atoi(e) == 0); }();
  if (!on || conv3p_mode() == 0 || conv3p_producer_waves() != 4) return DS_OK;
  if (a0.H % 8 != 0 || a0.W % 32 != 0 || a0.Cout % COT != 0 || a0.Cin % (4 * KC) != 0 || a0.res1_up) return DS_OK;
  const long long total = (long long)a0.n_cot * a0.tiles_x * a0.tiles_y * a0.B;
  const int wgs = conv3p_cus() / 8 * 8;
  if (wgs <= 0 || total < (long long)wgs * conv3p_min_items() || total >= (1ll << 22)) return DS_OK;
  if ((long long)4 * (a0.H + 2) * (a0.W + 2) * 16 >= (1ll << 31)) return DS_OK;
  Conv3hArgs a = a0;
  conv3p_fill_args(a);
  int rc;
  if (!a.res1) rc = launch_conv3p_w<false, false, 0, 4, false, true>(a, wgs, s);
  else rc = a.res2 ? launch_conv3p_w<false, false, 2, 4, false, true>(a, wgs, s) : launch_conv3p_w<false, false, 1, 4, false, true>(a, wgs, s);
  if (rc == DS_OK) *launched = true;
  return rc;
}

int conv3p_try_launch(const Conv3hArgs& a, hipStream_t s, bool* launched) {
  *launched = false;
  const int mode = conv3p_mode();
  if (mode == 0) return DS_OK;
  if (a.H % 8 != 0 || a.W % 32 != 0 || a.Cout % COT != 0 || a.Cin % (4 * KC) != 0) return DS_OK;
  if (a.Hin != a.H || a.Win != a.W || a.res1_up) return DS_OK;
  const long long total = (long long)a.n_cot * a.tiles_x * a.tiles_y * a.B;
  const int wgs = conv3p_cus() / 8 * 8;
  if (wgs <= 0 || total < (long long)wgs * conv3p_min_items() || total >= (1ll << 22)) return DS_OK;
  if (a.n_cot % 2 == 0 && a.prenorm && mode < 2) return DS_OK;
  if (!a.prenorm && mode < 3) return DS_OK;
  int rc;
  if (a.prenorm) rc = a.circular ? launch_conv3p<true, true>(a, wgs, s) : launch_conv3p<true, false>(a, wgs, s);
  else rc = a.circular ? launch_conv3p<false, true>(a, wgs, s) : launch_conv3p<false, false>(a, wgs, s);
  if (rc == DS_OK) *launched = true;
  return rc;
}

}
```

diffsci_amd/models/nets/punetg.py:

```python
import math
import os
from typing import Any

import torch

from ... import ops
from ..._native import DS_LOAD_MAXPOOL2, DS_LOAD_UPSAMPLE2
from . import precision
from .punetg_config import PUNetGConfig


class _AffineHolder(torch.nn.Module):

    def __init__(self, C, affine=True):
        super().__init__()
        self.weight = torch.nn.Parameter(torch.ones(C)) if affine else None
        self.bias = torch.nn.Parameter(torch.zeros(C)) if affine else None


NORM_KINDS = {"GroupLN": 0, "GroupRMS": 1, "GroupPix": 3}


def make_norm(name, C, affine=True):
    if name == "GroupLN":
# ... 393 lines not shown
            trace.append(f"{name}: {times} x (k = {k}) at stride {stride} -> {rf}")
        if c.in_embedding:
            trace.append("convin is a per-pixel Fourier embedding: unchanged")
        else:
            widen(c.in_out_kernel_size, "convin")
        levels = len(c.channel_expansion)
        for lv in range(levels):
            for b in range(c.number_resnet_downward_block):
                widen(c.kernel_size, f"down[{lv}].resnet[{b}]", 2)
            widen(c.transition_scale_factor, f"down[{lv}].maxpool")
            stride *= c.transition_scale_factor
            widen(c.transition_kernel_size, f"down[{lv}].conv")
        for name, n in (("before_block", c.number_resnet_before_attn_block), ("attn_resnet_block", c.number_resnet_attn_block),
                        ("after_block", c.number_resnet_after_attn_block)):
            for b in range(n):
                widen(c.kernel_size, f"{name}[{b}]", 2)
        for lv in range(levels - 1, -1, -1):
            stride //= c.transition_scale_factor
            widen(c.transition_kernel_size, f"up[{lv}].conv")
            for b in range(c.number_resnet_upward_block):
                widen(c.kernel_size, f"up[{lv}].resnet[{b}]", 2)
        widen(c.in_out_kernel_size, "convout")
        return {'rf': rf, 'has_attention': False, 'num_attention_layers': 0, 'trace': trace, 'feasible_chunking': True,
                'downsampling_factor': c.transition_scale_factor ** levels,
                'config_summary': {k: getattr(c, k) for k in (
                    'number_resnet_attn_block', 'number_resnet_downward_block', 'number_resnet_upward_block',
                    'number_resnet_before_attn_block', 'number_resnet_after_attn_block', 'kernel_size', 'in_out_kernel_size',
                    'transition_kernel_size', 'transition_scale_factor', 'channel_expansion')}}

    def export_description(self) -> dict[str, Any]:
        cemb = self.conditional_embedding
        cemb_args = cemb.export_description() if getattr(cemb, "export_description", None) else None
        return dict(config=self.config.export_description(),
                    conditional_embedding_args=cemb_args,
                    has_conditional_embedding=cemb is not None)

    def set_conditional_embedding(self, conditional_embedding: torch.nn.Module | None = None):
        self.conditional_embedding = conditional_embedding

    @ops.device_guard
    def forward(self, x, t=None, y=None):
        out = self.forward_unguarded(x, t, y)
        if precision.needs_escalation(self, out, x):
            precision.escalate(self)
            out = self.forward_unguarded(x, t, y)
        return out

    @ops.device_guard
    def forward_unguarded(self, x, t=None, y=None):
        ops.require_device(x, "x")
        B = x.shape[0]
        ye = self.embed_condition(y)
        if ye is not None and ye.dim() > 2:
            shifts = self.field_shifts(None if t is None else self.embed_time(t.reshape(-1).to(x)), ye, B)
        else:
            if t is None:
                te = torch.zeros(B, self.config.model_channels, device=x.device)
                if ye is not None:
                    te = te + ye
            else:
                te = self.embed_time(t.reshape(-1).to(x), ye)
            shifts = self.time_shifts(te)
        return self.forward_with_shifts(x.contiguous(), shifts, row=None)

    def embed_condition(self, y):
        if y is None:
            return None
        ye = y if self.conditional_embedding is None else self.conditional_embedding(y)
        if ye.dim() == 2 + self.dim and self.dim == 2:
            if ye.shape[1] != self.config.model_channels:
                raise ValueError("a field-valued conditional embedding must have model_channels channels")
            ops.require_device(ye, "conditional embedding")
            return ye.detach().to(torch.float32).contiguous()
        if ye.dim() != 2:
            raise NotImplementedError("field-valued conditional embeddings are implemented for 2-D networks ([B, C, H, W])")
        return ye.to(torch.float32).contiguous()

    def condition_is_field(self, y):
        ye = None if y is None else self.embed_condition(y)
        return ye is not None and ye.dim() > 2

    def field_shifts(self, te, ye, B):
        if ye.shape[0] not in (1, B):
            raise ValueError("conditional embedding batch must be 1 or match x")
        if te is not None and te.shape[0] not in (1, B):
            raise ValueError("time batch must be 1 or match x")
        ws = self._ws
        field = ws.take((B,) + tuple(ye.shape[1:]), ye.device)
        if te is None:
            field.copy_(ye.expand(B, -1, -1, -1))
        else:
            torch.add(te[:, :, None, None].expand(B, -1, 1, 1), ye, out=field)
        return _FieldShifts(field, ws, self.conv_precision == "fp16x3", owned=True)

    def _field_shift(self, blk, fs, H, W):
        pk, ws = self._timeblock_convs(), fs.ws
        te, a0 = fs.level(H, W)
        B, dev = te.shape[0], te.device
        n = blk.timeblock.net
        a1 = fs.am.row() if fs.am is not None else None
        a2 = fs.am.row() if fs.am is not None else None
        h = ops.conv(te, pk[id(n[0])], bias=n[0].bias, out=ws.take((B, n[0].out_features, H, W), dev),
                     **self._amax_kw(in_amax=a0, out_amax=a1))
        ops.inorm_silu(h, None, None, kind=2, out=h)
        h2 = ops.conv(h, pk[id(n[2])], bias=n[2].bias, out=ws.take((B, n[2].out_features, H, W), dev),
                      **self._amax_kw(in_amax=a1, out_amax=a2))
        ops.inorm_silu(h2, None, None, kind=2, out=h2)
        out = ops.conv(h2, pk[id(n[4])], bias=n[4].bias, out=ws.take((B, n[4].out_features, H, W), dev), **self._amax_kw(in_amax=a2))
        ws.give(h)
        ws.give(h2)
        return out

    def _timeblock_convs(self):
        lins = list(self._timeblock_linears())
        sig = (self.conv_precision,) + tuple((l.weight.data_ptr(), l.weight._version) for l in lins)
        if getattr(self, "_tb_packed_sig", None) != sig:
            with torch.no_grad():
                self._tb_packed = {}
                for l in lins:
                    w = mp_weight(l.weight.detach()) if self.mp else l.weight.detach()
                    self._tb_packed[id(l)] = ops.pack_conv(w.reshape(w.shape[0], w.shape[1], 1, 1).contiguous(),
                                                           "fp16x3" if self.conv_precision == "fp16x3" else "fp32")
            self._tb_packed_sig = sig
        return self._tb_packed

    def embed_time(self, t, ye=None):
        if ye is not None and ye.shape[0] not in (1, t.numel()):
            raise ValueError("conditional embedding batch must be 1 or match t")
        return ops.fourier_features(t.contiguous(), self.time_projection.W, add=ye)

    def time_shifts(self, te):
        out = []
        pk = self.packed_weights() if self.mp else None

        def wgt(lin):
            return pk[(id(lin), "eff")] if pk is not None else lin.weight

        for blk in self._resblocks():
            n = blk.timeblock.net
            h = ops.linear(te, wgt(n[0]), n[0].bias, act=1)
            h = ops.linear(h, wgt(n[2]), n[2].bias, act=1)
            out.append(ops.linear(h, wgt(n[4]), n[4].bias, act=0))
        return out

    def _resblocks(self):
        for lv in self.downward_blocks:
            yield from lv
        yield from self.before_block
        yield from self.attn_resnet_block
        yield from self.after_block
        for lv in self.upward_blocks:
            yield from lv

    def _shift_of(self, blk, te):
        pk = self.packed_weights() if self.mp else None
        n = blk.timeblock.net
        wgt = (lambda lin: pk[(id(lin), "eff")]) if pk is not None else (lambda lin: lin.weight)
        h = ops.linear(te, wgt(n[0]), n[0].bias, act=1)
        h = ops.linear(h, wgt(n[2]), n[2].bias, act=1)
        return ops.linear(h, wgt(n[4]), n[4].bias, act=0)

    def _run_blocks(self, x, te, resnet_block, attn_block=()):
        if self.dim != 2:
            raise NotImplementedError("the public stage methods are implemented for 2-D networks")
        pk, ws = self.packed_weights(), self._ws
        h, hs, own = x, None, False
        for i, blk in enumerate(resnet_block):
            h2, hs2 = self._res(blk, h, self._shift_of(blk, te), pk, ws, xs=hs)
            if own:
                ws.give(h)
                if hs is not None:
                    ws.give(hs)
            h, hs, own = h2, hs2, True
            if i < len(attn_block):
                hs2 = self._stats_buf(ws, h.shape[0], h.shape[1], h.shape[2], h.shape[3], h.device)
                h2 = self._attention(attn_block[i], h, pk, ws, tile_stats=hs2)
                ws.give(h)
                if hs is not None:
                    ws.give(hs)
                h, hs = h2, hs2
        return h, hs, own

    def _release(self, h, hs, own):
        out = h.clone() if own else h
        if own:
            self._ws.give(h)
        if hs is not None:
            self._ws.give(hs)
        return out

    @ops.device_guard
    def resnet_block_forward(self, x, te, resnet_block):
        require_eval(self, self.config.dropout, self.config.cond_dropout, self.config.cond_drop)
        ops.require_device(x, "x")
        return self._release(*self._run_blocks(x.contiguous(), te, resnet_block))

    @ops.device_guard
    def resnet_attn_block_forward(self, x, te, resnet_block, attn_block):
        require_eval(self, self.config.dropout, self.config.cond_dropout, self.config.cond_drop)
        ops.require_device(x, "x")
        return self._release(*self._run_blocks(x.contiguous(), te, resnet_block, attn_block))

    def encode(self, x, te):
        pk = self.packed_weights()
        intermediate_outputs = []
        for resnet_block, downsampler in zip(self.downward_blocks, self.downsamplers):
            x = self.resnet_block_forward(x, te, resnet_block)
            intermediate_outputs.append(x.clone())
            x = self._conv(downsampler.conv, x, pk, load_mode=DS_LOAD_MAXPOOL2)
        return x, intermediate_outputs

    def decode(self, x, te, intermediate_outputs):
        pk = self.packed_weights()
        for resnet_block, upsampler in zip(self.upward_blocks, self.upsamplers):
            x = self._conv(upsampler.conv, x.contiguous(), pk, load_mode=DS_LOAD_UPSAMPLE2, res1=intermediate_outputs.pop())
            x = self.resnet_block_forward(x, te, resnet_block)
        return x

    def bottom_forward(self, x, te):
        x = self.resnet_block_forward(x, te, self.before_block)
        xa = self.resnet_attn_block_forward(x, te, self.attn_resnet_block, self.attn_block)
        x = ops.add(x, xa)
        return self.resnet_block_forward(x, te, self.after_block)

    def _conv_modules(self):
        if not isinstance(self.convin, _FourierInput):
            yield self.convin
        yield self.convout
        for blk in self._resblocks():
            yield blk.conv1
            yield blk.conv2
        for s in list(self.downsamplers) + list(self.upsamplers):
            yield s.conv

    def _timeblock_linears(self):
        for blk in self._resblocks():
            n = blk.timeblock.net
            yield from (n[0], n[2], n[4])

    def packed_weights(self):
        mods = list(self._conv_modules())
        tracked = [m.weight for m in mods]
        for a in self.attn_block:
            tracked += ([a.mhattn.q_proj_matrix, a.mhattn.k_proj_matrix, a.mhattn.v_proj_matrix, a.mhattn.o_proj_matrix]
                        if self.inhouse_attn else [a.mhattn.in_proj_weight, a.mhattn.out_proj.weight])
        if self.mp:
            tracked += [lin.weight for lin in self._timeblock_linears()]
        sig = (self.conv_precision, getattr(self, "upsample_parity", True), self.exact_input_layer) + tuple((t.data_ptr(), t._version) for t in tracked)
        if self._packed is not None and sig == self._packed_sig:
            return self._packed
        pk = {}
        with torch.no_grad():
            ups = {id(u.conv) for u in self.upsamplers} if getattr(self, "upsample_parity", True) else set()
            for m in mods:
                w = m.weight.detach()
                if getattr(m, "mp", False):
                    w = mp_weight(w)
                    pk[(id(m), "eff")] = w
                if self.dim == 2:
                    pk[id(m)] = ops.pack_conv(w, self.conv_precision, upsampled=id(m) in ups)
                    if m is self.convin and self.conv_precision == "fp16x3":
                        pk[(id(m), "wmax")] = w.abs().amax(dim=(0, 2, 3)).contiguous()
                        if self.exact_input_layer:
                            pk[(id(m), "exact")] = ops.pack_conv(w, "fp32")
                elif self.conv_precision == "fp16x3":
                    pk[(id(m), "3d")] = ops.pack_conv3d(w, upsampled=id(m) in ups)
            prec = "fp16x3" if self.conv_precision == "fp16x3" else "fp32"
            for a in self.attn_block:
                E = a.mhattn.embed_dim
                if self.inhouse_attn:
                    w_in, w_out = a.mhattn.projection_weights()
                else:
                    w_in, w_out = a.mhattn.in_proj_weight.detach(), a.mhattn.out_proj.weight.detach()
                pk[(id(a), "in")] = ops.pack_conv(w_in.reshape(3 * E, E, 1, 1), prec)
                pk[(id(a), "out")] = ops.pack_conv(w_out.reshape(E, E, 1, 1), prec)
            if self.mp:
                for lin in self._timeblock_linears():
                    pk[(id(lin), "eff")] = mp_weight(lin.weight.detach()).contiguous()
        self._packed, self._packed_sig = pk, sig
        return pk

    def _amax_kw(self, **kw):
        return kw if self.conv_precision == "fp16x3" else {}

    def _conv(self, m, x, pk, in_amax=None, out_amax=None, **kw):
        return ops.conv(x, pk[id(m)], bias=m.bias, circular=self.circular, **self._amax_kw(in_amax=in_amax, out_amax=out_amax), **kw)

    def _out_is_direct(self, m):
        return m.out_channels <= 4 and getattr(self, "direct_out", True) and self.config.in_out_kernel_size == 3

    def _out_conv(self, m, h, pk, out, circular, in_amax=None):
        if self._out_is_direct(m):
            return ops.conv_direct(h, pk.get((id(m), "eff"), m.weight), m.bias, circular=circular, out=out)
        return ops.conv(h, pk[id(m)], bias=m.bias, circular=circular, out=out, **self._amax_kw(in_amax=in_amax))

    def _fused(self):
        return self.fuse_norm and self.conv_precision == "fp16x3"

    def _stats_buf(self, ws, B, C, H, W, dev):
        if not self._fused():
            return None
        return ws.take((B, C, ops.conv_tile_count(H, W), 4), dev)

    def _res(self, blk, x, shift, pk, ws, res2=None, xs=None, want_stats=True, out_amax=None):
        B, C, H, W = x.shape
        dev = x.device
        if self.extra_residual is not None:
            er = self.extra_residual(x)
            ops.require_device(er, "extra_residual output")
            if tuple(er.shape) != tuple(x.shape):
                raise ValueError("extra_residual must preserve the shape of its input")
            saved, self.extra_residual = self.extra_residual, None
            try:
                y, _ = self._res(blk, x, shift, pk, ws, res2=None, xs=xs, want_stats=False)
            finally:
                self.extra_residual = saved
            ops.add(y, er.contiguous(), out=y)
            if res2 is not None:
                ops.add(y, res2, out=y)
            if out_amax is not None:
                ops.absmax_rows(y, out=out_amax)
            return y, None
        if isinstance(shift, _FieldShifts):
            yt = self._field_shift(blk, shift, H, W)
            got = self._res_body(blk, x, None, yt, pk, ws, res2, xs, want_stats, out_amax)
            ws.give(yt)
            return got
        yt = None
        if shift is not None and shift.dim() == 4:
            yt, shift = self._rescale_shift_field(shift, H, W), None
        return self._res_body(blk, x, shift, yt, pk, ws, res2, xs, want_stats, out_amax)

    def _res_body(self, blk, x, shift, yt, pk, ws, res2, xs, want_stats, out_amax):
        B, C, H, W = x.shape
        dev = x.device
        k1, k2 = self.norm_kinds
        w1, b1 = getattr(blk.gnorm1, "weight", None), getattr(blk.gnorm1, "bias", None)
        w2, b2 = getattr(blk.gnorm2, "weight", None), getattr(blk.gnorm2, "bias", None)
        if (self._fused() and xs is not None and (C + 63) // 64 <= self.fuse_max_cot and k1 != 3 and k2 != 3
                and self.config.kernel_size == 3):
            tab = ws.take((B, ops.table_channels(C), 4), dev)
            ops.inorm_table(xs, w1, b1, k1, H * W, eps=1e-5, out=tab)
            ys = self._stats_buf(ws, B, C, H, W, dev)
            y = self._conv(blk.conv1, x, pk, shift=shift, res1=yt, prenorm=tab, tile_stats=ys, out=ws.take(x.shape, dev))
            ops.inorm_table(ys, w2, b2, k2, H * W, eps=1e-5, out=tab)
            os_ = self._stats_buf(ws, B, C, H, W, dev) if want_stats else None
            out = self._conv(blk.conv2, y, pk, res1=x, res2=res2, prenorm=tab, tile_stats=os_, out=ws.take(x.shape, dev),
                             out_amax=out_amax)
            ws.give(y)
            ws.give(ys)
            ws.give(tab)
            return out, os_
        windowed = k1 in (0, 1) and k2 in (0, 1) and self._norms_in_window(blk)
        if windowed and self._norm_images_ok(blk, C, H, W, k1, k2):
            img = ops.inorm_silu_images(x, w1, b1, k1, eps=1e-5, out=ws.take((ops.conv_images_floats(B, C, H, W),), dev))
            y = ops.conv_img(img, pk[id(blk.conv1)], B, C, H, W, bias=blk.conv1.bias, shift=shift, res1=yt, out=ws.take(x.shape, dev))
            ops.inorm_silu_images(y, w2, b2, k2, eps=1e-5, out=img)
            os_ = self._stats_buf(ws, B, C, H, W, dev) if want_stats else None
            out = ops.conv_img(img, pk[id(blk.conv2)], B, C, H, W, bias=blk.conv2.bias, res1=x, res2=res2, tile_stats=os_,
                               out=ws.take(x.shape, dev), out_amax=out_amax)
            ws.give(img)
            ws.give(y)
            return out, os_
        if windowed and self._table_images_ok(blk, C, k1, k2) and self._fused() and xs is not None:
            tab = ws.take((B, ops.table_channels(C), 4), dev)
            ops.inorm_table(xs, w1, b1, k1, H * W, eps=1e-5, out=tab)
            img = ops.table_apply_images(x, tab, out=ws.take((ops.conv_images_floats(B, C, H, W),), dev))
            ys = self._stats_buf(ws, B, C, H, W, dev)
            y = ops.conv_img(img, pk[id(blk.conv1)], B, C, H, W, bias=blk.conv1.bias, shift=shift, res1=yt, tile_stats=ys,
                             out=ws.take(x.shape, dev))
            ops.inorm_table(ys, w2, b2, k2, H * W, eps=1e-5, out=tab)
            ops.table_apply_images(y, tab, out=img)
            os_ = self._stats_buf(ws, B, C, H, W, dev) if want_stats else None
            out = ops.conv_img(img, pk[id(blk.conv2)], B, C, H, W, bias=blk.conv2.bias, res1=x, res2=res2, tile_stats=os_,
                               out=ws.take(x.shape, dev), out_amax=out_amax)
            for t in (img, y, ys, tab):
                ws.give(t)
            return out, os_
        a = ops.inorm_silu(x, w1, b1, kind=k1, eps=1e-5, out=ws.take(x.shape, dev))
        y = self._conv(blk.conv1, a, pk, shift=shift, res1=yt, out=ws.take(x.shape, dev), in_amax=self._act_amax(a, windowed))
        ops.inorm_silu(y, w2, b2, kind=k2, eps=1e-5, out=a)
        os_ = self._stats_buf(ws, B, C, H, W, dev) if want_stats else None
        self._conv(blk.conv2, a, pk, res1=x, res2=res2, tile_stats=os_, out=y, in_amax=self._act_amax(a, windowed), out_amax=out_amax)
        ws.give(a)
        return y, os_

    def _consumes_stats(self, blk, C, H, W):
        if blk is None or not self._fused() or self.extra_residual is not None:
            return False
        k1, k2 = self.norm_kinds
        if (C + 63) // 64 <= self.fuse_max_cot and k1 != 3 and k2 != 3 and self.config.kernel_size == 3:
            return True
        windowed = k1 in (0, 1) and k2 in (0, 1) and self._norms_in_window(blk)
        if windowed and self._norm_images_ok(blk, C, H, W, k1, k2):
            return False
        return windowed and self._table_images_ok(blk, C, k1, k2)

    def _act_amax(self, a, windowed):
        if windowed or self.conv_precision != "fp16x3":
            return ops.NORMALISED
        return self._am.of(a) if self._am is not None else None

    def _norms_in_window(self, blk):
        return precision.norms_in_window(self._window_cache, id(blk), (blk.gnorm1, blk.gnorm2))

    def _table_images_ok(self, blk, C, k1, k2):
        return (getattr(self, "norm_images", True) and self.conv_precision == "fp16x3" and not self.circular
                and self.config.kernel_size == 3 and k1 in (0, 1, 2) and k2 in (0, 1, 2) and ((C + 15) // 16) % 2 == 0
                and blk.conv1.out_channels == C and blk.conv2.out_channels == C)

    def _norm_images_ok(self, blk, C, H, W, k1, k2):
        return (getattr(self, "norm_images", True) and self.conv_precision == "fp16x3" and not self.circular
                and self.config.kernel_size == 3 and k1 in (0, 1) and k2 in (0, 1) and ((C + 15) // 16) % 2 == 0
                and blk.conv1.out_channels == C and blk.conv2.out_channels == C and ops.inorm_silu_images_supported(H, W))

    @staticmethod
    def _rescale_shift_field(yt, H, W):
        h, w = yt.shape[2:]
        if (h, w) == (H, W):
            return yt
        if h > H:
            f = h // H
            if H * f != h or W * f != w:
                raise ValueError(f"yt_dims {(h, w)} and y_dims {(H, W)} are not compatible")
            return yt[:, :, ::f, ::f].contiguous()
        raise NotImplementedError("a conditional-embedding field coarser than a block's resolution (the reference's "
                                  "upscaling branch passes the factor as torch.nn.Upsample's size and fails as well)")

    def forward_with_shifts(self, x, shifts, row=None, out=None):
        require_eval(self, self.config.dropout, self.config.cond_dropout, self.config.cond_drop)
        if self.dim == 3:
            return self._forward3d(x, shifts, row=row, out=out)
        pk = self.packed_weights()
        ws = self._ws
        cfg = self.config
        B = x.shape[0]
        dev = x.device
        lazy_shifts = shifts if isinstance(shifts, _FieldShifts) else None
        it = iter(range(len(shifts))) if lazy_shifts is None else None

        def sh():
            if lazy_shifts is not None:
                return lazy_shifts
            s = shifts[next(it)]
            if s.dim() == 4:
                return s
            if row is not None:
                if s.dim() == 3:
                    if s.shape[1] != B:
                        raise ValueError("time embedding batch does not match x")
                    return s[row]
                return s[row:row + 1]
            if s.shape[0] not in (1, B):
                raise ValueError("time embedding batch does not match x")
            return s

        def give(t, ts):
            ws.give(t)
            if ts is not None:
                ws.give(ts)

        h3 = self.conv_precision == "fp16x3"
        lazy = h3 and not isinstance(self.convin, _FourierInput) and not self.exact_input_layer
        am = self._am = _AmaxArena(ws, B, dev, zero=not lazy) if h3 else None

        def slot(needed=True):
            return am.row() if (h3 and needed) else None

        def amax_of(t, ta):
            if not h3:
                return None
            return ta if ta is not None else am.of(t)

        try:
            H, W = x.shape[2:]
            xe = None
            if not cfg.bias:
                ones = ws.take((B, 1, H, W), dev)
                ones.fill_(1.0)
                xe = ops.concat2(x, ones, out=ws.take((B, x.shape[1] + 1, H, W), dev))
                ws.give(ones)
                x = xe
            ndown = len(self.downward_blocks)
            bottom = list(self.before_block) + list(self.attn_resnet_block) + list(self.after_block)

            def stats_for(nxt, C_, H_, W_):
                return self._stats_buf(ws, B, C_, H_, W_, dev) if self._consumes_stats(nxt, C_, H_, W_) else None

            def first_block_after_level(lv):
                if lv + 1 < ndown and len(self.downward_blocks[lv + 1]):
                    return self.downward_blocks[lv + 1][0]
                return bottom[0] if bottom else None
            if isinstance(self.convin, _FourierInput):
                hs = None
                h = ops.fourier_channels(x, self.convin.W, out=ws.take((B, cfg.model_channels, H, W), dev))
            elif h3 and self.exact_input_layer:
                hs = None
                h = ops.conv(x, pk[(id(self.convin), "exact")], bias=self.convin.bias, circular=self.circular,
                             out=ws.take((B, cfg.model_channels, H, W), dev))
            else:
                first = self.downward_blocks[0][0] if (ndown and len(self.downward_blocks[0])) else (bottom[0] if bottom else None)
                hs = stats_for(first, cfg.model_channels, H, W)
                h = self._conv(self.convin, x, pk, tile_stats=hs, out=ws.take((B, cfg.model_channels, H, W), dev),
                               in_amax=am.of_input(x, precision.input_layer_flag(self, dev), pk[(id(self.convin), "wmax")]) if h3 else None)
            ha = None
            if xe is not None:
                ws.give(xe)
            skips = []
            for lv, blocks in enumerate(self.downward_blocks):
                for j, blk in enumerate(blocks):
                    ha2 = slot(j == len(blocks) - 1)
                    nxt = blocks[j + 1] if j + 1 < len(blocks) else None
                    h2, hs2 = self._res(blk, h, sh(), pk, ws, xs=hs, out_amax=ha2,
                                        want_stats=self._consumes_stats(nxt, h.shape[1], h.shape[2], h.shape[3]))
                    give(h, hs)
                    h, hs, ha = h2, hs2, ha2
                skips.append(h)
                if hs is not None:
                    ws.give(hs)
                ds = self.downsamplers[lv].conv
                Ho, Wo = h.shape[2] // 2, h.shape[3] // 2
                hs = stats_for(first_block_after_level(lv), ds.out_channels, Ho, Wo)
                h = self._conv(ds, h, pk, load_mode=DS_LOAD_MAXPOOL2, tile_stats=hs,
                               out=ws.take((B, ds.out_channels, Ho, Wo), dev), in_amax=amax_of(h, ha))
                ha = None
            nattn, nafter = len(self.attn_resnet_block), len(self.after_block)
            for j, blk in enumerate(self.before_block):
                ha2 = slot(j == len(self.before_block) - 1 and nattn == 0 and nafter == 0 and ndown > 0)
                nxt = bottom[j + 1] if (j + 1 < len(self.before_block) or nattn > 0) else None
                h2, hs2 = self._res(blk, h, sh(), pk, ws, xs=hs, out_amax=ha2,
                                    want_stats=self._consumes_stats(nxt, h.shape[1], h.shape[2], h.shape[3]))
                give(h, hs)
                h, hs, ha = h2, hs2, ha2
            xa, xas, xaa = h, hs, ha
            for i, blk in enumerate(self.attn_resnet_block):
                last = i == nattn - 1
                attn_next = i < len(self.attn_block)
                xaa2 = slot(attn_next or (last and nafter == 0 and ndown > 0))
                nb = len(self.before_block)
                nxt = None if attn_next else (bottom[nb + i + 1] if nb + i + 1 < len(bottom) else None)
                xa2, xas2 = self._res(blk, xa, sh(), pk, ws, xs=xas,
                                      res2=h if (last and not attn_next) else None, out_amax=xaa2,
                                      want_stats=self._consumes_stats(nxt, xa.shape[1], xa.shape[2], xa.shape[3]))
                if xa is not h:
                    give(xa, xas)
                xa, xas, xaa = xa2, xas2, xaa2
                if attn_next:
                    nxt = bottom[nb + i + 1] if nb + i + 1 < len(bottom) else None
                    xas2 = stats_for(nxt, xa.shape[1], xa.shape[2], xa.shape[3])
                    xaa2 = slot(last and nafter == 0 and ndown > 0)
                    xa2 = self._attention(self.attn_block[i], xa, pk, ws, res2=h if last else None, tile_stats=xas2,
                                          in_amax=amax_of(xa, xaa), out_amax=xaa2)
                    give(xa, xas)
                    xa, xas, xaa = xa2, xas2, xaa2
            if nattn == 0:
                xa, xas, xaa = ops.add(h, h, out=ws.take(h.shape, dev)), None, None
            give(h, hs if xas is not hs else None)
            h, hs, ha = xa, xas, xaa
            for j, blk in enumerate(self.after_block):
                ha2 = slot(j == nafter - 1 and ndown > 0)
                nxt = self.after_block[j + 1] if j + 1 < nafter else None
                h2, hs2 = self._res(blk, h, sh(), pk, ws, xs=hs, out_amax=ha2,
                                    want_stats=self._consumes_stats(nxt, h.shape[1], h.shape[2], h.shape[3]))
                give(h, hs)
                h, hs, ha = h2, hs2, ha2
            nup = len(self.upward_blocks)
            direct_out = self._out_is_direct(self.convout)
            for lv, blocks in enumerate(self.upward_blocks):
                us = self.upsamplers[lv].conv
                skip = skips.pop()
                hs2 = stats_for(blocks[0] if len(blocks) else None, skip.shape[1], skip.shape[2], skip.shape[3])
                h2 = self._conv(us, h, pk, load_mode=DS_LOAD_UPSAMPLE2, res1=skip, tile_stats=hs2,
                                out=ws.take(skip.shape, dev), in_amax=amax_of(h, ha))
                give(h, hs)
                ws.give(skip)
                h, hs, ha = h2, hs2, None
                for j, blk in enumerate(blocks):
                    lastb = j == len(blocks) - 1
                    final = lv == nup - 1 and lastb
                    ha2 = slot(lastb and (not final or not direct_out))
                    nxt = None if lastb else blocks[j + 1]
                    h2, hs2 = self._res(blk, h, sh(), pk, ws, xs=hs, out_amax=ha2,
                                        want_stats=self._consumes_stats(nxt, h.shape[1], h.shape[2], h.shape[3]))
                    give(h, hs)
                    h, hs, ha = h2, hs2, ha2
            y = self._out_conv(self.convout, h, pk, out, self.circular, in_amax=None if direct_out else amax_of(h, ha))
            give(h, hs)
            return y
        finally:
            if am is not None:
                am.release()
            self._am = None
            if lazy_shifts is not None:
                lazy_shifts.release()

    def _forward3d(self, x, shifts, row=None, out=None):
        if x.dim() != 5:
            raise ValueError("a dimension=3 network takes [B, C, D, H, W] volumes")
        pk = self.packed_weights()
        ws = self._ws
        cfg = self.config
        B, dev = x.shape[0], x.device
        it = iter(range(len(shifts)))
        k1, k2 = self.norm_kinds

        def sh():
            s = shifts[next(it)]
            if row is not None:
                if s.dim() == 3:
                    if s.shape[1] != B:
                        raise ValueError("time embedding batch does not match x")
                    return s[row]
                return s[row:row + 1]
            if s.shape[0] not in (1, B):
                raise ValueError("time embedding batch does not match x")
            return s

        fold = self._fused() and self.extra_residual is None and k1 != 3 and k2 != 3 and cfg.kernel_size == 3

        def stats_buf(shape):
            Bc, C, D, H, W = shape
            return ws.take((Bc, C, ops.volume_stat_tiles(D, H * W), 4), dev)

        def conv(m, h, load_mode=0, dst=None, fresh=False, want_stats=False, normalised=False, **kw):
            f = {0: (1, 1), DS_LOAD_MAXPOOL2: (1, 2), DS_LOAD_UPSAMPLE2: (2, 1)}[load_mode]
            shape = (h.shape[0], m.out_channels) + tuple(v * f[0] // f[1] for v in h.shape[2:])
            if dst is None and not fresh:
                dst = ws.take(shape, dev)
            packs = pk.get((id(m), "3d"))
            k = m.weight.shape[-1]
            if packs is None and k != 3:
                raise NotImplementedError(f"{k}x{k}x{k} kernels on volumes are implemented on the fp16x3 convolution only "
                                          f"(conv_precision={self.conv_precision!r})")
            if packs is not None and ((m.out_channels > 4 and m.in_channels > 4) or k != 3):
                st = stats_buf(shape) if (fold and want_stats) else None
                return ops.conv3d_mfma(h, packs, bias=m.bias, circular=self.circular, load_mode=load_mode, out=dst, ws=ws,
                                       out_stats=st, in_amax=ops.NORMALISED if normalised else None, **kw), st
            return ops.conv3d(h, pk.get((id(m), "eff"), m.weight), bias=m.bias, circular=self.circular, load_mode=load_mode,
                              out=dst, **kw), None

        def give(t, ts=None):
            ws.give(t)
            if ts is not None:
                ws.give(ts)

        def res(blk, h, hs, res2=None, want_stats=True):
            w1, b1 = getattr(blk.gnorm1, "weight", None), getattr(blk.gnorm1, "bias", None)
            w2, b2 = getattr(blk.gnorm2, "weight", None), getattr(blk.gnorm2, "bias", None)
            C = h.shape[1]
            p1, p2 = pk.get((id(blk.conv1), "3d")), pk.get((id(blk.conv2), "3d"))
            windowed = k1 in (0, 1) and k2 in (0, 1) and self._norms_in_window(blk)
            if (fold and windowed and hs is not None and p1 is not None and p2 is not None and C > 4
                    and (C + 63) // 64 <= self.fuse_max_cot):
                tab = ops.inorm_table(hs, w1, b1, k1, h[0, 0].numel(), eps=1e-5, out=ws.take((B, ops.table_channels(C), 4), dev))
                os_ = stats_buf(h.shape) if want_stats else None
                y = ops.resblock3d_fused(h, tab, p1, blk.conv1.bias, sh(), p2, blk.conv2.bias, w2, b2, k2, res2=res2,
                                         out=ws.take(h.shape, dev), out_stats=os_, ws=ws, circular=self.circular)
                ws.give(tab)
                return y, os_
            a = ops.inorm_silu(h, w1, b1, kind=k1, eps=1e-5, out=ws.take(h.shape, dev))
            y, _ = conv(blk.conv1, a, shift=sh(), normalised=windowed)
            ops.inorm_silu(y, w2, b2, kind=k2, eps=1e-5, out=a)
            if self.extra_residual is None:
                _, os_ = conv(blk.conv2, a, res1=h, res2=res2, dst=y, want_stats=want_stats, normalised=windowed)
            else:
                conv(blk.conv2, a, res1=h, dst=y, normalised=windowed)
                ops.add(y, self.extra_residual(h).contiguous(), out=y)
                if res2 is not None:
                    ops.add(y, res2, out=y)
                os_ = None
            ws.give(a)
            return y, os_

        def attn(att, h, res2=None):
            Bq, E, D, H, W = h.shape
            r2 = None if res2 is None else res2.view(Bq, E, D * H, W)
            y = self._attention(att, h.view(Bq, E, D * H, W), pk, ws, res2=r2)
            o = ws.take(h.shape, dev)
            o.copy_(y.view(h.shape))
            ws.give(y)
            return o

        x = x.contiguous()
        xe = None
        if not cfg.bias:
            ones = ws.take((B, 1) + tuple(x.shape[2:]), dev)
            ones.fill_(1.0)
            xe = ops.concat2(x, ones, out=ws.take((B, x.shape[1] + 1) + tuple(x.shape[2:]), dev))
            ws.give(ones)
            x = xe
        hs = None
        if isinstance(self.convin, _FourierInput):
            h = ops.fourier_channels(x, self.convin.W, out=ws.take((B, cfg.model_channels) + tuple(x.shape[2:]), dev))
        else:
            h, hs = conv(self.convin, x, want_stats=True)
        if xe is not None:
            ws.give(xe)
        skips = []
        for lv, blocks in enumerate(self.downward_blocks):
            for blk in blocks:
                h2, hs2 = res(blk, h, hs)
                give(h, hs)
                h, hs = h2, hs2
            skips.append(h)
            if hs is not None:
                ws.give(hs)
            h, hs = conv(self.downsamplers[lv].conv, h, load_mode=DS_LOAD_MAXPOOL2, want_stats=True)
        for blk in self.before_block:
            h2, hs2 = res(blk, h, hs)
            give(h, hs)
            h, hs = h2, hs2
        xa, xas = h, hs
        nattn = len(self.attn_resnet_block)
        for i, blk in enumerate(self.attn_resnet_block):
            last = i == nattn - 1
            xa2, xas2 = res(blk, xa, xas, res2=h if (last and i >= len(self.attn_block)) else None)
            if xa is not h:
                give(xa, xas)
            xa, xas = xa2, xas2
            if i < len(self.attn_block):
                xa2 = attn(self.attn_block[i], xa, res2=h if last else None)
                give(xa, xas)
                xa, xas = xa2, None
        if nattn == 0:
            xa, xas = ops.add(h, h, out=ws.take(h.shape, dev)), None
        give(h, hs if xas is not hs else None)
        h, hs = xa, xas
        for blk in self.after_block:
            h2, hs2 = res(blk, h, hs)
            give(h, hs)
            h, hs = h2, hs2
        nup = len(self.upward_blocks)
        for lv, blocks in enumerate(self.upward_blocks):
            skip = skips.pop()
            h2, hs2 = conv(self.upsamplers[lv].conv, h, load_mode=DS_LOAD_UPSAMPLE2, res1=skip, want_stats=True)
            give(h, hs)
            ws.give(skip)
            h, hs = h2, hs2
            for j, blk in enumerate(blocks):
                final = lv == nup - 1 and j == len(blocks) - 1
                h2, hs2 = res(blk, h, hs, want_stats=not final)
                give(h, hs)
                h, hs = h2, hs2
        y, _ = conv(self.convout, h, dst=out, fresh=out is None)
        give(h, hs)
        return y

    def _attention(self, att, x, pk, ws, res2=None, tile_stats=None, in_amax=None, out_amax=None):
        B, E, Hh, Ww = x.shape
        L = Hh * Ww
        m = att.mhattn
        in_bias = None if self.inhouse_attn else m.in_proj_bias
        out_bias = None if self.inhouse_attn else m.out_proj.bias
        am = self._am if self.conv_precision == "fp16x3" else None
        own = None
        if am is None and self.conv_precision == "fp16x3":
            own = am = _AmaxArena(ws, B, x.device)
        split = 2 * E if E % 32 == 0 else 0
        a_qkv = am.rows(2) if am is not None else None
        a_o = am.row() if am is not None else None
        if am is not None and in_amax is None:
            in_amax = am.of(x)
        direct = not self.cosine_attn and split > 0
        qkv = ops.conv(x, pk[(id(att), "in")], bias=in_bias, out=ws.take((B, 3 * E, Hh, Ww), x.device),
                       **self._amax_kw(in_amax=in_amax, out_amax=a_qkv if direct else None, amax_split=split if direct else 0))
        if self.cosine_attn:
            ops.token_l2_normalize(qkv.view(B, 3 * E, L), 0, E, eps=1e-8, gain=math.sqrt(E))
            ops.token_l2_normalize(qkv.view(B, 3 * E, L), E, E, eps=1e-8, gain=1.0)
        if am is not None and not direct:
            ops.absmax_rows(qkv[:, :2 * E], out=a_qkv[:B])
            ops.absmax_rows(qkv[:, 2 * E:], out=a_qkv[B:])
        nws = ops.attention_workspace_floats(B, E, L, self.conv_precision)
        aws = ws.take((nws,), x.device) if nws else None
        o = ops.attention(qkv.view(B, 3 * E, L), E, out=ws.take((B, E, L), x.device),
                          precision=self.conv_precision, workspace=aws, **self._amax_kw(in_amax=a_qkv, out_amax=a_o))
        if aws is not None:
            ws.give(aws)
        res1 = x if self.config.attn_residual else None
        y = ops.conv(o.view(B, E, Hh, Ww), pk[(id(att), "out")], bias=out_bias,
                     res1=res1, res2=res2, tile_stats=tile_stats, out=ws.take(x.shape, x.device),
                     **self._amax_kw(in_amax=a_o, out_amax=out_amax))
        ws.give(qkv)
        ws.give(o)
        if own is not None:
            own.release()
        return y


class PUNetGCond(PUNetG):

    def __init__(self, config: PUNetGConfig, conditional_embedding: torch.nn.Module | None = None,
                 channel_conditional_items: list[str] | None = False, extra_residual: torch.nn.Module | None = None):
        super().__init__(config, conditional_embedding, extra_residual=extra_residual)
        self.channel_conditional_items = channel_conditional_items
        self._ycat = None
        self._ycat_static = {}

    def export_description(self) -> dict[str, Any]:
        args = super().export_description()
        args["channel_conditional_items"] = self.channel_conditional_items
        return args

    def _split_condition(self, y):
        if y is None:
            raise TypeError("PUNetGCond needs the condition dictionary y on every call (punetg.py:721-723)")
        fields = [y[item] for item in self.channel_conditional_items]
        rest = {k: v for k, v in y.items() if k not in self.channel_conditional_items}
        for f in fields:
            ops.require_device(f, "channel condition")
            if f.dim() < 3 or tuple(f.shape[2:]) != tuple(fields[0].shape[2:]) or f.shape[0] != fields[0].shape[0]:
                raise ValueError("channel condition fields must be [B or 1, C_i, *spatial] with equal batch and spatial sizes")
        shape = (fields[0].shape[0], sum(f.shape[1] for f in fields)) + tuple(fields[0].shape[2:])
        key = (shape, str(fields[0].device))
        buf = self._ycat_static.get(key)
        if buf is None:
            with torch.inference_mode(False):
                buf = torch.empty(shape, dtype=torch.float32, device=fields[0].device)
            self._ycat_static[key] = buf
        c0 = 0
        for f in fields:
            buf[:, c0:c0 + f.shape[1]].copy_(f)
            c0 += f.shape[1]
        return (rest if len(rest) else None), buf

    def _with_condition(self, x, ycat, ws):
        B = x.shape[0]
        yexp = None
# ... 40 lines not shown
```

diffsci_amd/ops.py:

```python
import ctypes

import torch

from . import _native as N
from ._native import EvalCoef


def require_device(t, what="tensor"):
    if not isinstance(t, torch.Tensor):
        raise TypeError(f"{what} must be a torch.Tensor")
    if not t.is_cuda:
        raise RuntimeError(
            f"{what} lives on {t.device}: diffsci_amd computes only on an AMD GPU through "
            "libdiffsci_hip.so (there is no CPU path; move the module and inputs to 'cuda').")
    if t.dtype != torch.float32:
        raise TypeError(f"{what} has dtype {t.dtype}; the HIP path is fp32 only")
    if t.device.index != torch.cuda.current_device():
        raise RuntimeError(f"{what} lives on {t.device} but the current device is cuda:{torch.cuda.current_device()}: "
                           "wrap the call in `with torch.cuda.device(tensor.device):` (KarrasModule / SIModule / the "
                           "networks do this for their own entry points)")


def on_device_of(t):
    return torch.cuda.device(t.device)
# ... 387 lines not shown
    circ = 1 if circular else 0
    N.check(N.lib().ds_volume_to_slices_act(_p(s1), _p(h.contiguous()), _p(tab1), B, C, D, H * W, circ, _stream()),
            "ds_volume_to_slices_act")
    s2 = take((ns, C, H, W))
    if not circular:
        s2[0].zero_()
        s2[ns - 1].zero_()
    ts = take((ns - 2, C, conv_tile_count(H, W), 4))
    rows, rows_buf = _slice_rows(shift, B, D, C, ws)
    _depth_taps(s1, s2, packs1, bias1, rows, N.DS_LOAD_PLAIN, bool(circular), tile_stats=ts, in_amax=NORMALISED)
    if circular:
        N.check(N.lib().ds_wrap_pad_slices(_p(s2), B, C, D, H * W, _stream()), "ds_wrap_pad_slices")
    tab2 = take((ns, table_channels(C), 4))
    N.check(N.lib().ds_slice_tables(_p(tab2), _p(ts), _p(w2), _p(b2), B, C, D, ts.shape[2], D * H * W, float(eps), int(kind2),
                                    circ, _stream()), "ds_slice_tables")
    _depth_taps(s2, s1, packs2, bias2, None, N.DS_LOAD_PLAIN, bool(circular), prenorm=tab2)
    _from_slices(out, s1, h, res2, B, C, D, H * W, out_stats)
    if ws is not None:
        for t in (s1, s2, ts, tab2, rows_buf):
            if t is not None:
                ws.give(t)
    return out


def conv3d_mfma(x, packs, bias=None, shift=None, res1=None, res2=None, load_mode=N.DS_LOAD_PLAIN, circular=False, out=None,
                ws=None, out_stats=None, in_amax=None):
    require_device(x, "x")
    B, Cin, Din, Hi, Wi = x.shape
    Cout = packs[0].Cout
    if load_mode == N.DS_LOAD_MAXPOOL2:
        if Din % 2 or Hi % 2 or Wi % 2:
            raise ValueError("pooling load needs an even input volume")
        D, H, W, depth_mode = Din // 2, Hi // 2, Wi // 2, 1
    elif load_mode == N.DS_LOAD_UPSAMPLE2:
        D, H, W, depth_mode = 2 * Din, 2 * Hi, 2 * Wi, 2
    else:
        D, H, W, depth_mode = Din, Hi, Wi, 0
    if out is None:
        out = torch.empty((B, Cout, D, H, W), dtype=torch.float32, device=x.device)
    elif tuple(out.shape) != (B, Cout, D, H, W):
        raise ValueError(f"out has shape {tuple(out.shape)}, expected {(B, Cout, D, H, W)}")
    for r in (res1, res2):
        if r is not None and tuple(r.shape) != (B, Cout, D, H, W):
            raise ValueError("residual shape mismatch")
    P = len(packs) // 2
    if circular and P > D:
        raise ValueError(f"periodic padding of {P} slices needs a depth of at least {P}; got {D}")
    ns = B * (D + 2 * P)

    def take(shape):
        return torch.empty(shape, dtype=torch.float32, device=x.device) if ws is None else ws.take(shape, x.device)
    s_in = take((ns, Cin, Hi, Wi))
    N.check(N.lib().ds_volume_to_slices(_p(s_in), _p(x.contiguous()), B, Cin, D, Hi * Wi, depth_mode, 1 if circular else 0, P,
                                        _stream()), "ds_volume_to_slices")
    s_out = take((ns, Cout, H, W))
    rows, rows_buf = _slice_rows(shift, B, D, Cout, ws, pad=P)
    am_buf = None
    if in_amax is not NORMALISED:
        if ws is None:
            in_amax = absmax_rows(s_in)
        else:
            am_buf = ws.take((ns,), x.device)
            in_amax = absmax_rows(s_in, out=amax_zero(am_buf.view(torch.int32)))
    _depth_taps(s_in, s_out, packs, bias, rows, load_mode, circular, in_amax=in_amax)
    _from_slices(out, s_out, res1, res2, B, Cout, D, H * W, out_stats, pad=P)
    if rows_buf is not None:
        ws.give(rows_buf)
    if am_buf is not None:
        ws.give(am_buf)
    if ws is not None:
        ws.give(s_in)
        ws.give(s_out)
    return out


def avgpool3d(x, out=None):
    require_device(x, "x")
    B, C, Di, Hi, Wi = x.shape
    if Di % 2 or Hi % 2 or Wi % 2:
        raise ValueError("avgpool3d needs even D, H, W")
    if out is None:
        out = torch.empty((B, C, Di // 2, Hi // 2, Wi // 2), dtype=torch.float32, device=x.device)
    N.check(N.lib().ds_avgpool3d(_p(out, "out"), _p(x, "x"), B * C, Di // 2, Hi // 2, Wi // 2, _stream()), "ds_avgpool3d")
    return out


def upsample3d(x, out=None):
    require_device(x, "x")
    B, C, Di, Hi, Wi = x.shape
    if out is None:
        out = torch.empty((B, C, 2 * Di, 2 * Hi, 2 * Wi), dtype=torch.float32, device=x.device)
    N.check(N.lib().ds_upsample3d(_p(out, "out"), _p(x, "x"), B * C, Di, Hi, Wi, _stream()), "ds_upsample3d")
    return out


def _factor(factor):
    import operator
    try:
        f = operator.index(factor)
    except TypeError:
        f = None
    if f is None or isinstance(factor, bool) or f < 1:
        raise ValueError(f"resampling factor {factor!r} must be an integer >= 1")
    return f


def _film_args(film, B, C):
    if film is None:
        return None, None, 0
    if film.dim() != 2 or film.shape[1] != 2 * C or film.shape[0] not in (1, B):
        raise ValueError("film must be [1 or B, 2C]")
    require_device(film, "film")
    if not film.is_contiguous():
        raise ValueError("film must be contiguous")
    return film.data_ptr(), film.data_ptr() + 4 * C, (0 if film.shape[0] == 1 else 2 * C)


def gnorm1_apply_poolf(x, stats, w, b, kind, factor, film=None, out=None):
    f = _factor(factor)
    require_device(x, "x")
    B, C, H, W = x.shape
    if f > min(H, W):
        raise ValueError(f"pooling factor {f} exceeds the field {H}x{W}")
    if out is None:
        out = torch.empty((B, C, H // f, W // f), dtype=torch.float32, device=x.device)
    elif tuple(out.shape) != (B, C, H // f, W // f):
        raise ValueError(f"out has shape {tuple(out.shape)}, expected {(B, C, H // f, W // f)}")
    f1, f2, stride = _film_args(film, B, C)
    N.check(N.lib().ds_gnorm1_apply_poolf(_p(out), _p(x), _p(stats), _p(w), _p(b), f1, f2, stride, B, C, H, W, int(kind), f,
                                          _stream()), "ds_gnorm1_apply_poolf")
    return out


def avgpool_f(x, factor, out=None):
    f = _factor(factor)
    require_device(x, "x")
    if x.dim() == 4:
        return gnorm1_apply_poolf(x, None, None, None, 2, f, out=out)
    if x.dim() != 5:
        raise ValueError("avgpool_f takes [B, C, H, W] fields or [B, C, D, H, W] volumes")
    B, C, Di, Hi, Wi = x.shape
    if f > min(Di, Hi, Wi):
        raise ValueError(f"pooling factor {f} exceeds the volume {Di}x{Hi}x{Wi}")
    shape = (B, C, Di // f, Hi // f, Wi // f)
    if out is None:
        out = torch.empty(shape, dtype=torch.float32, device=x.device)
    elif tuple(out.shape) != shape:
        raise ValueError(f"out has shape {tuple(out.shape)}, expected {shape}")
    N.check(N.lib().ds_avgpool3d_f(_p(out, "out"), _p(x, "x"), B * C, Di, Hi, Wi, f, _stream()), "ds_avgpool3d_f")
    return out


def upsample_f(x, factor, out=None):
    f = _factor(factor)
    require_device(x, "x")
    if x.dim() not in (4, 5):
        raise ValueError("upsample_f takes [B, C, H, W] fields or [B, C, D, H, W] volumes")
    vol = x.dim() == 5
    B, C = x.shape[:2]
    Di, Hi, Wi = (x.shape[2:] if vol else (1,) + tuple(x.shape[2:]))
    shape = (B, C) + ((f * Di,) if vol else ()) + (f * Hi, f * Wi)
    if out is None:
        out = torch.empty(shape, dtype=torch.float32, device=x.device)
    elif tuple(out.shape) != shape:
        raise ValueError(f"out has shape {tuple(out.shape)}, expected {shape}")
    N.check(N.lib().ds_upsample_f(_p(out, "out"), _p(x, "x"), B * C, Di, Hi, Wi, f, 1 if vol else 0, _stream()),
            "ds_upsample_f")
    return out


def gnorm1_stats(x, kind, eps=1e-5, stats=None, workspace=None):
    B, C = x.shape[0], x.shape[1]
    HW = x.numel() // max(B * C, 1)
    if stats is None:
        stats = torch.empty((B, 2), dtype=torch.float32, device=x.device)
    need = N.lib().ds_gnorm1_workspace_bytes(B)
    if workspace is None:
        workspace = torch.empty(need // 4, dtype=torch.float32, device=x.device)
    elif workspace.numel() * 4 < need:
        raise ValueError("gnorm1 workspace too small")
    N.check(N.lib().ds_gnorm1_stats(_p(stats), _p(workspace), _p(x), B, C, HW, float(eps), int(kind), _stream()),
            "ds_gnorm1_stats")
    return stats


def gnorm1_apply(x, stats, w, b, kind, pool=False, film=None, out=None):
    B, C, H, W = x.shape
    Ho, Wo = (H // 2, W // 2) if pool else (H, W)
    if out is None:
        out = torch.empty((B, C, Ho, Wo), dtype=torch.float32, device=x.device)
    f1 = f2 = None
    stride = 0
    if film is not None:
        if film.dim() != 2 or film.shape[1] != 2 * C or film.shape[0] not in (1, B):
            raise ValueError("film must be [1 or B, 2C]")
        require_device(film, "film")
        stride = 0 if film.shape[0] == 1 else 2 * C
        f1, f2 = film.data_ptr(), film.data_ptr() + 4 * C
    N.check(N.lib().ds_gnorm1_apply(_p(out), _p(x), _p(stats), _p(w), _p(b), f1, f2, stride, B, C, H, W, int(kind),
                                    1 if pool else 0, _stream()), "ds_gnorm1_apply")
    return out


def concat2(a, b, out=None):
    B = a.shape[0]
    na, nb = a.numel() // max(B, 1), b.numel() // max(B, 1)
    if out is None:
        out = torch.empty((B, a.shape[1] + b.shape[1]) + tuple(a.shape[2:]), dtype=torch.float32, device=a.device)
    N.check(N.lib().ds_concat2(_p(out), _p(a), _p(b), B, na, nb, _stream()), "ds_concat2")
    return out


def add_act(a, add=None, act=0, out=None):
    M, Nn = a.shape
    out = torch.empty_like(a) if out is None else out
    rows = 0
    if add is not None:
        add = add.reshape(-1, Nn)
        rows = add.shape[0]
    N.check(N.lib().ds_add_act(_p(out), _p(a), _p(add), rows, M, Nn, int(act), _stream()), "ds_add_act")
    return out


def pack_conv_weight(w):
    require_device(w, "conv weight")
    Cout, Cin, k, k2 = w.shape
    if k != k2 or k not in (1, 3):
        raise NotImplementedError(f"conv kernel {k}x{k2}: only 1x1 and 3x3 are implemented")
    n = N.lib().ds_conv2d_packed_floats(Cout, Cin, k)
    packed = torch.empty(n, dtype=torch.float32, device=w.device)
    N.check(N.lib().ds_conv2d_pack_weights(_p(packed), _p(w.contiguous()), Cout, Cin, k, _stream()),
            "ds_conv2d_pack_weights")
    return packed


class PackedConv:
    __slots__ = ("data", "Cout", "Cin", "ks", "kind", "wshift", "up", "up_wshift", "subs")

    def __init__(self, data, Cout, Cin, ks, kind, wshift=0, up=None, up_wshift=0, subs=None):
        self.data, self.Cout, self.Cin, self.ks, self.kind, self.wshift = data, Cout, Cin, ks, kind, wshift
        self.up, self.up_wshift = up, up_wshift
        self.subs = subs

    @property
    def x6(self):
        return self.kind == "bf16x6"


CONV_PRECISIONS = ("fp16x3", "bf16x6", "fp32")


def pack_conv(w, precision="bf16x6", upsampled=False):
    require_device(w, "conv weight")
    if precision not in CONV_PRECISIONS:
        raise ValueError(f"unknown conv precision {precision!r}; choose from {CONV_PRECISIONS}")
    Cout, Cin, k, k2 = w.shape
    w = w.contiguous()
    if k != k2 or k % 2 == 0:
        raise NotImplementedError(f"conv kernel {k}x{k2}: square kernels of odd size are implemented")
    if k > 3:
        if precision != "fp16x3":
            raise NotImplementedError(f"{k}x{k} kernels are implemented on the fp16x3 convolution only (conv_precision={precision!r})")
        ng = (k + 2) // 3
        starts = [min(3 * g, k - 3) for g in range(ng)]
        subs = []
        for gy, sy in enumerate(starts):
            for gx, sx in enumerate(starts):
                blk = w[:, :, sy:sy + 3, sx:sx + 3].clone()
                blk[:, :, :3 * gy - sy, :] = 0
                blk[:, :, :, :3 * gx - sx] = 0
                subs.append((sy + 1 - k // 2, sx + 1 - k // 2, pack_conv(blk.contiguous(), "fp16x3")))
        return PackedConv(None, Cout, Cin, k, "fp16x3", subs=subs)
    if precision == "bf16x6" and k == 3:
        nbytes = N.lib().ds_conv2d_x6_packed_bytes(Cout, Cin)
        data = torch.empty(nbytes // 4, dtype=torch.float32, device=w.device)
        N.check(N.lib().ds_conv2d_x6_pack_weights(data.data_ptr(), _p(w), Cout, Cin, _stream()),
                "ds_conv2d_x6_pack_weights")
        return PackedConv(data, Cout, Cin, 3, "bf16x6")
    if precision == "fp16x3" and k in (1, 3):
        wmax = float(w.abs().max())
        wshift = 0
        if wmax > 0 and wmax == wmax and wmax != float("inf"):
            import math
            wshift = max(-40, min(40, 13 - math.floor(math.log2(wmax))))
        size_fn, pack_fn = ((N.lib().ds_conv2d_h3_packed_bytes, N.lib().ds_conv2d_h3_pack_weights) if k == 3 else
                            (N.lib().ds_conv1x1_h3_packed_bytes, N.lib().ds_conv1x1_h3_pack_weights))
        data = torch.empty(size_fn(Cout, Cin) // 4, dtype=torch.float32, device=w.device)
        N.check(pack_fn(data.data_ptr(), _p(w), Cout, Cin, wshift, _stream()), "ds_conv*_h3_pack_weights")
        up, up_wshift = None, 0
        if upsampled and k == 3:
            up_wshift = max(-40, wshift - 2)
            up = torch.empty(N.lib().ds_conv2d_h3_up_packed_bytes(Cout, Cin) // 4, dtype=torch.float32, device=w.device)
            N.check(N.lib().ds_conv2d_h3_up_pack_weights(up.data_ptr(), _p(w), Cout, Cin, up_wshift, _stream()),
                    "ds_conv2d_h3_up_pack_weights")
        return PackedConv(data, Cout, Cin, k, "fp16x3", wshift, up, up_wshift)
    return PackedConv(pack_conv_weight(w), Cout, Cin, k, "fp32")


def conv(x, pw, **kw):
    if pw.subs is None:
        return conv2d(x, pw.data, pw.Cout, pw.ks, kind=pw.kind, wshift=pw.wshift, w_up=pw.up, up_wshift=pw.up_wshift, **kw)
    if kw.get("res1_upsampled", False):
        raise NotImplementedError("res1_upsampled with kernels larger than 3x3")
    stats, out, out_amax = kw.pop("tile_stats", None), kw.pop("out", None), kw.pop("out_amax", None)
    first = dict(bias=kw.pop("bias", None), shift=kw.pop("shift", None), res1=kw.pop("res1", None), res2=kw.pop("res2", None))
    if kw.get("in_amax", None) is None and kw.get("prenorm", None) is None:
        kw["in_amax"] = absmax_rows(x)
    n = len(pw.subs)
    for i, (oy, ox, sub) in enumerate(pw.subs):
        extra = first if i == 0 else dict(res1=out)
        out = conv2d(x, sub.data, sub.Cout, 3, kind="fp16x3", wshift=sub.wshift, tap_offset=(oy, ox), out=out,
                     tile_stats=stats if i == n - 1 else None, out_amax=out_amax if i == n - 1 else None, **extra, **kw)
    return out


def conv_direct(x, w, bias=None, circular=False, out=None):
    B, Cin, H, W = x.shape
    Cout = w.shape[0]
    if tuple(w.shape) != (Cout, Cin, 3, 3):
        raise ValueError("conv_direct: weight must be [Cout, Cin, 3, 3]")
    if out is None:
        out = torch.empty((B, Cout, H, W), dtype=torch.float32, device=x.device)
    elif tuple(out.shape) != (B, Cout, H, W):
        raise ValueError(f"out has shape {tuple(out.shape)}, expected {(B, Cout, H, W)}")
    N.check(N.lib().ds_conv2d_direct(_p(out), _p(x), _p(w), _p(bias), B, Cin, Cout, H, W, 1 if circular else 0,
                                     _stream()), "ds_conv2d_direct")
    return out


def conv_tile_count(H, W):
    return N.lib().ds_conv_tile_count(int(H), int(W))


def table_channels(C):
    return (C + 15) // 16 * 16


def inorm_table(tile_stats, w, b, kind, count, eps=1e-5, out=None):
    B, C, nt, _ = tile_stats.shape
    if out is None:
        out = torch.empty((B, table_channels(C), 4), dtype=torch.float32, device=tile_stats.device)
    elif tuple(out.shape) != (B, table_channels(C), 4):
        raise ValueError(f"table must be {(B, table_channels(C), 4)}")
    N.check(N.lib().ds_inorm_table(_p(out), _p(tile_stats), _p(w), _p(b), B, C, nt, int(count), float(eps), int(kind),
                                   _stream()), "ds_inorm_table")
    return out


def gnorm1_table(stats_a, w, b, kind, count, stats_b=None, film=None, eps=1e-5, out=None):
    B, Ca, nta, _ = stats_a.shape
    Cb, ntb = (0, 0) if stats_b is None else (stats_b.shape[1], stats_b.shape[2])
    C = Ca + Cb
    if out is None:
        out = torch.empty((B, table_channels(C), 4), dtype=torch.float32, device=stats_a.device)
    elif tuple(out.shape) != (B, table_channels(C), 4):
        raise ValueError(f"table must be {(B, table_channels(C), 4)}")
    f1 = f2 = None
    stride = 0
    if film is not None:
        if film.dim() != 2 or film.shape[1] != 2 * C or film.shape[0] not in (1, B):
            raise ValueError("film must be [1 or B, 2C]")
        require_device(film, "film")
        stride = 0 if film.shape[0] == 1 else 2 * C
        f1, f2 = film.data_ptr(), film.data_ptr() + 4 * C
    N.check(N.lib().ds_gnorm1_table(_p(out), _p(stats_a), Ca, nta, _p(stats_b), Cb, ntb, _p(w), _p(b), f1, f2, stride,
                                    B, int(count), float(eps), int(kind), _stream()), "ds_gnorm1_table")
    return out


def gnorm1_stats_tiles(stats_a, kind, count, stats_b=None, eps=1e-5, stats=None):
    require_device(stats_a, "stats_a")
    B, Ca, nta, _ = stats_a.shape
    Cb, ntb = (0, 0) if stats_b is None else (stats_b.shape[1], stats_b.shape[2])
    if stats is None:
        stats = torch.empty((B, 2), dtype=torch.float32, device=stats_a.device)
    elif tuple(stats.shape) != (B, 2):
        raise ValueError(f"stats must be {(B, 2)}")
    N.check(N.lib().ds_gnorm1_stats_tiles(_p(stats), _p(stats_a), Ca, nta, _p(stats_b), Cb, ntb, B, int(count), float(eps),
                                          int(kind), _stream()), "ds_gnorm1_stats_tiles")
    return stats


def conv2d(x, w_packed, Cout, ks, bias=None, shift=None, res1=None, res2=None,
           load_mode=N.DS_LOAD_PLAIN, out=None, kind="fp32", wshift=0, prenorm=None, tile_stats=None, circular=False,
           res1_upsampled=False, w_up=None, up_wshift=0, tap_offset=None, in_amax=None, out_amax=None, amax_split=0):
    B, Cin, Hin, Win = x.shape
    if load_mode in (N.DS_LOAD_MAXPOOL2, N.DS_LOAD_AVGPOOL2):
        if Hin % 2 or Win % 2:
            raise ValueError("pooling load needs even input H, W")
        if (load_mode == N.DS_LOAD_AVGPOOL2) != (kind == "fp16x3" and ks == 1):
            raise ValueError("load modes: AVGPOOL2 is for the fp16x3 1x1 kernel, MAXPOOL2 for the others")
        H, W = Hin // 2, Win // 2
    elif load_mode == N.DS_LOAD_UPSAMPLE2:
        H, W = Hin * 2, Win * 2
    else:
        H, W = Hin, Win
    if out is None:
        out = torch.empty((B, Cout, H, W), dtype=torch.float32, device=x.device)
    elif tuple(out.shape) != (B, Cout, H, W):
        raise ValueError(f"out has shape {tuple(out.shape)}, expected {(B, Cout, H, W)}")
    expect = {"bf16x6": lambda: N.lib().ds_conv2d_x6_packed_bytes(Cout, Cin) // 4,
              "fp16x3": lambda: (N.lib().ds_conv2d_h3_packed_bytes if ks == 3 else
                                 N.lib().ds_conv1x1_h3_packed_bytes)(Cout, Cin) // 4,
              "fp32": lambda: N.lib().ds_conv2d_packed_floats(Cout, Cin, ks)}[kind]()
    if w_packed.numel() != expect or (kind == "bf16x6" and ks != 3) or ks not in (1, 3):
        raise ValueError("packed weight size does not match (Cout, Cin, ks)")
    stride = 0
    if shift is not None:
        if shift.dim() != 2 or shift.shape[1] != Cout or shift.shape[0] not in (1, B):
            raise ValueError(f"shift must be [1 or B, Cout]; got {tuple(shift.shape)}")
        stride = 0 if shift.shape[0] == 1 else Cout
    if res1_upsampled:
        if kind != "fp16x3" or ks != 3 or res1 is None or H % 2 or W % 2 or tuple(res1.shape) != (B, Cout, H // 2, W // 2):
            raise ValueError("res1_upsampled: fp16x3 3x3 convolution with res1 of shape [B, Cout, H/2, W/2]")
    for r in ((res2,) if res1_upsampled else (res1, res2)):
        if r is not None and tuple(r.shape) != (B, Cout, H, W):
            raise ValueError("residual shape mismatch")
    if bias is not None and bias.numel() != Cout:
        raise ValueError("bias must have Cout entries")
    if (prenorm is not None or tile_stats is not None) and kind != "fp16x3":
        raise ValueError("prenorm / tile_stats are features of the fp16x3 kernels")
    pin = pout = None
    if kind == "fp16x3":
        pin = _in_amax(x, in_amax, B, raw=prenorm is None)
        if amax_split and (ks != 1 or amax_split % 64):
            raise ValueError("amax_split: the fp16x3 1x1 convolution, a multiple of 64")
        pout = _pi(out_amax, 2 * B if amax_split else B, "out_amax")
    elif out_amax is not None:
        raise ValueError("out_amax is a feature of the fp16x3 kernels (use absmax_rows on the result)")
    if circular and ks == 3 and kind != "fp16x3":
        raise NotImplementedError("periodic padding is implemented in the fp16x3 convolution only")
    if prenorm is not None and (ks != 3 or tuple(prenorm.shape) != (B, table_channels(Cin), 4)):
        raise ValueError(f"prenorm must be [B, ceil16(Cin), 4] on a 3x3 convolution; got {tuple(prenorm.shape)}")
    if tile_stats is not None and tuple(tile_stats.shape) != (B, Cout, conv_tile_count(H, W), 4):
        raise ValueError(f"tile_stats must be {(B, Cout, conv_tile_count(H, W), 4)}; got {tuple(tile_stats.shape)}")
    tap = 0
    if tap_offset is not None and tuple(tap_offset) != (0, 0):
        oy, ox = (int(v) for v in tap_offset)
        if kind != "fp16x3" or ks != 3 or not (-8 <= oy <= 7 and -8 <= ox <= 7):
            raise ValueError("tap_offset: fp16x3 3x3 convolution, offsets in [-8, 7]")
        tap = ((oy & 15) << 8) | ((ox & 15) << 12)
        w_up = None
    if kind == "fp16x3" and ks == 1:
        N.check(N.lib().ds_conv1x1_h3(_p(out), _p(x), _p(w_packed), int(wshift), _p(bias), _p(shift), stride,
                                      _p(res1), _p(res2), B, Cin, Cout, H, W, load_mode, _p(tile_stats), pin, pout,
                                      int(amax_split), _stream()), "ds_conv1x1_h3")
    elif kind == "fp16x3" and load_mode == N.DS_LOAD_UPSAMPLE2 and w_up is not None \
            and N.lib().ds_conv2d_h3_up_supported(Hin, Win):
        if w_up.numel() != N.lib().ds_conv2d_h3_up_packed_bytes(Cout, Cin) // 4:
            raise ValueError("w_up size does not match (Cout, Cin)")
        N.check(N.lib().ds_conv2d_h3_up(_p(out), _p(x), _p(w_up), int(up_wshift), _p(bias), _p(shift), stride,
                                        _p(res1), _p(res2), B, Cin, Cout, Hin, Win,
                                        (N.DS_PAD_CIRCULAR if circular else 0) | (N.DS_RES1_UPSAMPLED if res1_upsampled else 0),
                                        _p(prenorm), _p(tile_stats), pin, pout, _stream()), "ds_conv2d_h3_up")
    elif kind == "fp16x3":
        N.check(N.lib().ds_conv2d_h3(_p(out), _p(x), _p(w_packed), int(wshift), _p(bias), _p(shift), stride,
                                     _p(res1), _p(res2), B, Cin, Cout, H, W,
                                     load_mode | tap | (N.DS_PAD_CIRCULAR if circular else 0) | (N.DS_RES1_UPSAMPLED if res1_upsampled else 0),
                                     _p(prenorm), _p(tile_stats), pin, pout,
                                     _stream()), "ds_conv2d_h3")
    elif kind == "bf16x6":
        N.check(N.lib().ds_conv2d_x6(_p(out), _p(x), _p(w_packed), _p(bias), _p(shift), stride, _p(res1),
                                     _p(res2), B, Cin, Cout, H, W, load_mode, _stream()), "ds_conv2d_x6")
    else:
        N.check(N.lib().ds_conv2d(_p(out), _p(x), _p(w_packed), _p(bias), _p(shift), stride, _p(res1), _p(res2),
                                  B, Cin, Cout, H, W, ks, load_mode, _stream()), "ds_conv2d")
    return out


def conv_images_floats(B, C, H, W):
    return N.lib().ds_conv_images_bytes(int(B), int(C), int(H), int(W)) // 4


def inorm_silu_images_supported(H, W):
    return bool(N.lib().ds_inorm_silu_images_supported(int(H), int(W)))


def inorm_silu_images(x, w, b, kind, eps=1e-5, out=None):
    require_device(x, "x")
    B, C, H, W = x.shape
    n = conv_images_floats(B, C, H, W)
    if out is None:
        out = torch.empty(n, dtype=torch.float32, device=x.device)
    elif out.numel() != n:
        raise ValueError("images buffer size does not match x")
    if w is not None and (w.numel() != C or b.numel() != C):
        raise ValueError("norm affine parameters must have C entries")
    N.check(N.lib().ds_inorm_silu_images(_p(out), _p(x), _p(w), _p(b), B, C, H, W, float(eps), int(kind), _stream()),
            "ds_inorm_silu_images")
    return out


def conv_img(images, pw, B, Cin, H, W, bias=None, shift=None, res1=None, res2=None, tile_stats=None, out=None,
             res1_upsampled=False, out_amax=None):
    require_device(images, "images")
    if pw.kind != "fp16x3" or pw.ks != 3 or pw.subs is not None:
        raise ValueError("conv_img: a 3x3 fp16x3 packing")
    Cout = pw.Cout
    if images.numel() != conv_images_floats(B, Cin, H, W):
        raise ValueError("images size does not match (B, Cin, H, W)")
    if out is None:
        out = torch.empty((B, Cout, H, W), dtype=torch.float32, device=images.device)
    elif tuple(out.shape) != (B, Cout, H, W):
        raise ValueError(f"out has shape {tuple(out.shape)}, expected {(B, Cout, H, W)}")
    stride = 0
    if shift is not None:
        if shift.dim() != 2 or shift.shape[1] != Cout or shift.shape[0] not in (1, B):
            raise ValueError(f"shift must be [1 or B, Cout]; got {tuple(shift.shape)}")
        stride = 0 if shift.shape[0] == 1 else Cout
    if res1_upsampled and (res1 is None or H % 2 or W % 2 or tuple(res1.shape) != (B, Cout, H // 2, W // 2)):
        raise ValueError("res1_upsampled: res1 of shape [B, Cout, H/2, W/2]")
    for r in ((res2,) if res1_upsampled else (res1, res2)):
        if r is not None and tuple(r.shape) != (B, Cout, H, W):
            raise ValueError("residual shape mismatch")
    if tile_stats is not None and tuple(tile_stats.shape) != (B, Cout, conv_tile_count(H, W), 4):
        raise ValueError(f"tile_stats must be {(B, Cout, conv_tile_count(H, W), 4)}")
    N.check(N.lib().ds_conv2d_h3_img(_p(out), _p(images), _p(pw.data), int(pw.wshift), _p(bias), _p(shift), stride, _p(res1),
                                     _p(res2), B, Cin, Cout, H, W, N.DS_RES1_UPSAMPLED if res1_upsampled else 0,
                                     _p(tile_stats), _pi(out_amax, B, "out_amax"), _stream()), "ds_conv2d_h3_img")
    return out


def table_apply_images(x, table, out=None):
    require_device(x, "x")
    require_device(table, "table")
    B, C, H, W = x.shape
    if tuple(table.shape) != (B, table_channels(C), 4):
        raise ValueError(f"table must be {(B, table_channels(C), 4)}; got {tuple(table.shape)}")
    n = conv_images_floats(B, C, H, W)
    if out is None:
        out = torch.empty(n, dtype=torch.float32, device=x.device)
    elif out.numel() != n:
        raise ValueError("images buffer size does not match x")
    N.check(N.lib().ds_table_apply_images(_p(out), _p(x), _p(table), B, C, H, W, _stream()), "ds_table_apply_images")
    return out


def conv_up_img_supported(pw, Hl, Wl):
    return (pw.kind == "fp16x3" and pw.ks == 3 and pw.subs is None and pw.up is not None
            and bool(N.lib().ds_conv2d_h3_up_supported(int(Hl), int(Wl))))


def conv_up_img(images, pw, B, Cin, Hl, Wl, bias=None, shift=None, res1=None, res2=None, tile_stats=None, out=None,
                out_amax=None):
    require_device(images, "images")
    if not conv_up_img_supported(pw, Hl, Wl):
        raise ValueError("conv_up_img: a 3x3 fp16x3 packing with parity kernels and an input of whole 8x32 / 16x16 tiles")
    Cout, H, W = pw.Cout, 2 * Hl, 2 * Wl
    if images.numel() != conv_images_floats(B, Cin, Hl, Wl):
        raise ValueError("images size does not match (B, Cin, Hl, Wl)")
    if out is None:
        out = torch.empty((B, Cout, H, W), dtype=torch.float32, device=images.device)
    elif tuple(out.shape) != (B, Cout, H, W):
        raise ValueError(f"out has shape {tuple(out.shape)}, expected {(B, Cout, H, W)}")
    stride = 0
    if shift is not None:
        if shift.dim() != 2 or shift.shape[1] != Cout or shift.shape[0] not in (1, B):
            raise ValueError(f"shift must be [1 or B, Cout]; got {tuple(shift.shape)}")
        stride = 0 if shift.shape[0] == 1 else Cout
    for r in (res1, res2):
        if r is not None and tuple(r.shape) != (B, Cout, H, W):
            raise ValueError("residual shape mismatch")
    if tile_stats is not None and tuple(tile_stats.shape) != (B, Cout, conv_tile_count(H, W), 4):
        raise ValueError(f"tile_stats must be {(B, Cout, conv_tile_count(H, W), 4)}")
    N.check(N.lib().ds_conv2d_h3_up_img(_p(out), _p(images), _p(pw.up), int(pw.up_wshift), _p(bias), _p(shift), stride, _p(res1),
                                        _p(res2), B, Cin, Cout, Hl, Wl, _p(tile_stats), _pi(out_amax, B, "out_amax"), _stream()),
            "ds_conv2d_h3_up_img")
    return out


def gnorm1_apply_images(x, stats, w, b, kind, pool=False, film=None, out=None):
    require_device(x, "x")
    B, C, H, W = x.shape
    if pool and (H % 2 or W % 2):
        raise ValueError("pooling needs even H, W")
    Ho, Wo = (H // 2, W // 2) if pool else (H, W)
    n = conv_images_floats(B, C, Ho, Wo)
    if out is None:
        out = torch.empty(n, dtype=torch.float32, device=x.device)
    elif out.numel() != n:
        raise ValueError("images buffer size does not match x")
    f1 = f2 = None
    stride = 0
    if film is not None:
        if film.dim() != 2 or film.shape[1] != 2 * C or film.shape[0] not in (1, B):
            raise ValueError("film must be [1 or B, 2C]")
        require_device(film, "film")
        stride = 0 if film.shape[0] == 1 else 2 * C
        f1, f2 = film.data_ptr(), film.data_ptr() + 4 * C
    N.check(N.lib().ds_gnorm1_apply_images(_p(out), _p(x), _p(stats), _p(w), _p(b), f1, f2, stride, B, C, Ho, Wo, int(kind),
                                           1 if pool else 0, _stream()), "ds_gnorm1_apply_images")
    return out


def token_l2_normalize(x, c0, C, eps=1e-8, gain=1.0):
    require_device(x, "x")
    B, Ctot, L = x.shape
    N.check(N.lib().ds_token_l2_normalize(_p(x), B, Ctot, int(c0), int(C), L, float(eps), float(gain), _stream()),
            "ds_token_l2_normalize")
    return x


ATTN_IMAGES_MIN_L = 2048
ATTN_IMAGES_MIN_L_WIDE = 1024


def _attention_uses_images(E, L, precision):
    if precision != "fp16x3" or E not in (32, 64, 128, 256) or L % 32:
        return False
    return L >= ATTN_IMAGES_MIN_L or (E == 256 and L >= ATTN_IMAGES_MIN_L_WIDE)


def _check_heads(E, heads):
    heads = int(heads)
    if heads < 1 or E % heads:
        raise ValueError(f"attention: E={E} is not a multiple of heads={heads}")
    return heads


def attention_workspace_floats(B, E, L, precision="fp16x3", heads=1):
    heads = _check_heads(E, heads)
    if heads > 1:
        if _attention_uses_images(E // heads, L, precision):
            return N.lib().ds_attention_h3_heads_workspace_bytes(B, E, heads, L) // 4
        return 0
    if _attention_uses_images(E, L, precision):
        return N.lib().ds_attention_h3_workspace_bytes(B, E, L) // 4
    return 0


def attention(qkv, E, out=None, precision="fp32", workspace=None, in_amax=None, out_amax=None, heads=1):
    B, E3, L = qkv.shape
    if E3 != 3 * E:
        raise ValueError("qkv must be [B, 3E, L]")
    heads = _check_heads(E, heads)
    if heads > 1:
        return _attention_heads(qkv, E, heads, out, precision, workspace, in_amax, out_amax)
    if out is None:
        out = torch.empty((B, E, L), dtype=torch.float32, device=qkv.device)
    h3 = precision == "fp16x3" and L % 32 == 0 and E in (32, 64, 128, 256)
    if h3:
        if in_amax is None:
            in_amax = amax_new(2 * B, qkv.device)
            absmax_rows(qkv[:, :2 * E], out=in_amax[:B])
            absmax_rows(qkv[:, 2 * E:], out=in_amax[B:])
        pin, pout = (None if in_amax is NORMALISED else _pi(in_amax, 2 * B, "in_amax")), _pi(out_amax, B, "out_amax")
    if h3 and _attention_uses_images(E, L, precision):
        need = attention_workspace_floats(B, E, L)
        if workspace is None:
            workspace = torch.empty(need, dtype=torch.float32, device=qkv.device)
        elif workspace.numel() < need:
            raise ValueError("attention workspace too small")
        N.check(N.lib().ds_attention_h3_ws(_p(out), _p(qkv), _p(workspace, "workspace"), B, E, L, pin, pout, _stream()),
                "ds_attention_h3_ws")
    elif h3:
        N.check(N.lib().ds_attention_h3(_p(out), _p(qkv), B, E, L, pin, pout, _stream()), "ds_attention_h3")
    else:
        if L % 32 != 0 or E not in (32, 64, 128, 256, 384, 512):
            N.check(N.lib().ds_attention_generic(_p(out), _p(qkv), B, E, L, _stream()), "ds_attention_generic")
        else:
            N.check(N.lib().ds_attention(_p(out), _p(qkv), B, E, L, _stream()), "ds_attention")
        if out_amax is not None:
            absmax_rows(out, B, out=out_amax)
    return out


def _attention_heads(qkv, E, heads, out, precision, workspace, in_amax, out_amax):
    B, _, L = qkv.shape
    if out is None:
        out = torch.empty((B, E, L), dtype=torch.float32, device=qkv.device)
    d = E // heads
    if precision == "fp16x3" and L % 32 == 0 and d in (32, 64, 128, 256):
        if in_amax is None:
            in_amax = amax_new(2 * B, qkv.device)
            absmax_rows(qkv[:, :2 * E], out=in_amax[:B])
            absmax_rows(qkv[:, 2 * E:], out=in_amax[B:])
        pin, pout = (None if in_amax is NORMALISED else _pi(in_amax, 2 * B, "in_amax")), _pi(out_amax, B, "out_amax")
        need = attention_workspace_floats(B, E, L, precision, heads)
        if need and workspace is None:
            workspace = torch.empty(need, dtype=torch.float32, device=qkv.device)
        elif need and workspace.numel() < need:
            raise ValueError("attention workspace too small")
        pws = _p(workspace, "workspace") if need else None
        N.check(N.lib().ds_attention_h3_heads(_p(out), _p(qkv), pws, B, E, heads, L, pin, pout, _stream()),
                "ds_attention_h3_heads")
    else:
        N.check(N.lib().ds_attention_heads_generic(_p(out), _p(qkv), B, E, heads, L, _stream()), "ds_attention_heads_generic")
        if out_amax is not None:
            absmax_rows(out, B, out=out_amax)
    return out


def linear(x, w, b=None, act=0, out=None):
    M, K = x.shape
    Nn, K2 = w.shape
    if K != K2:
        raise ValueError("linear: inner dimensions differ")
    if out is None:
        out = torch.empty((M, Nn), dtype=torch.float32, device=x.device)
    N.check(N.lib().ds_linear(_p(out), _p(x), _p(w), _p(b), M, K, Nn, act, _stream()), "ds_linear")
    return out


def fourier_features(t, W, add=None, out=None):
    M, half = t.numel(), W.numel()
    if out is None:
        out = torch.empty((M, 2 * half), dtype=torch.float32, device=t.device)
    add_rows = 0
    if add is not None:
        add = add.reshape(-1, 2 * half)
        add_rows = add.shape[0]
    N.check(N.lib().ds_fourier_features(_p(out), _p(t), _p(W), _p(add), add_rows, M, half, _stream()),
            "ds_fourier_features")
    return out


def fourier_channels(x, W, out=None):
    require_device(x, "x")
    B, C = x.shape[0], x.shape[1]
    if W.dim() != 2 or W.shape[0] != C:
        raise ValueError(f"fourier_channels: W must be [{C}, D]; got {tuple(W.shape)}")
    D = W.shape[1]
    HW = x.numel() // max(B * C, 1)
    if out is None:
        out = torch.empty((B, 2 * D) + tuple(x.shape[2:]), dtype=torch.float32, device=x.device)
    N.check(N.lib().ds_fourier_channels(_p(out, "out"), _p(x, "x"), _p(W, "W"), B, C, D, HW, _stream()), "ds_fourier_channels")
    return out


class Graph:

    def __init__(self):
        self._h = ctypes.c_void_p()
        self.nodes = 0

    @staticmethod
    def _allocations():
        return torch.cuda.memory_stats().get("allocation.all.allocated", 0)

    def __enter__(self):
        self._stream = _stream()
        self._alloc0 = self._allocations()
        N.check(N.lib().ds_graph_begin_capture(self._stream), "ds_graph_begin_capture")
        return self

    def __exit__(self, et, ev, tb):
        n = ctypes.c_int(0)
        rc = N.lib().ds_graph_end_capture(self._stream, ctypes.byref(self._h), ctypes.byref(n))
        if et is None:
            N.check(rc, "ds_graph_end_capture")
            made = self._allocations() - self._alloc0
            if made:
                raise RuntimeError(f"{made} device allocation(s) happened inside a captured region; the graph would "
                                   "write to memory it does not own on replay")
        self.nodes = n.value
        return False

    def launch(self):
        N.check(N.lib().ds_graph_launch(self._h, _stream()), "ds_graph_launch")

    def __del__(self):
# ... 6 lines not shown
```

include/diffsci_hip.h:

```cpp
#ifndef DIFFSCI_HIP_H
#define DIFFSCI_HIP_H

#include <stddef.h>
#include <stdint.h>

#ifdef __cplusplus
extern "C" {
#endif

typedef enum ds_status {
  DS_OK = 0,
  DS_ERR_SHAPE = -1,
  DS_ERR_NULL = -2,
  DS_ERR_HIP = -3,
  DS_ERR_UNSUPPORTED = -4
} ds_status;

int ds_version(void);
const char* ds_last_error(void);
int ds_device_info(int* cu_count, int* lds_bytes_per_cu, char* arch_name, int arch_name_len);

typedef struct ds_eval_coef {
  float c_out;
  float c_skip;
  float sigma_sq;
  float neg_mult;
  float neg_lang;
  float guidance;
  float one_minus_guidance;
  int   input_kind;
  int   stochastic;
  int   scaled;
  float scale;
  float scale_mult;
  float next_scale;
  int   xin_copies;
  uint32_t* nonfinite;
} ds_eval_coef;

enum { DS_IN_NETWORK = 0, DS_IN_SCORE = 1, DS_IN_DRIFT = 2,
       DS_IN_FLOW = 3  };

int ds_karras_scale(float* out, const float* x, float s, size_t n, void* stream);

int ds_karras_drift(float* d_out, const float* x, const float* f, const float* fu,
                    const ds_eval_coef* k, size_t n, void* stream);

int ds_karras_score(float* s_out, const float* x, const float* f, const float* fu,
                    const ds_eval_coef* k, size_t n, void* stream);

int ds_philox_normal(float* out, const uint64_t* philox_state, uint64_t philox_offset, size_t n, void* stream);

int ds_karras_euler(float* x_out, float* xin_out, const float* x, const float* f, const float* fu,
                    const ds_eval_coef* k, float dt, float c_in_next,
                    const float* eps, const uint64_t* philox_state, uint64_t philox_offset,
                    float noise_coef, float sqrt_abs_dt, size_t n, void* stream);

int ds_karras_heun(float* x_out, float* xin_out, const float* x,
                   const float* f1, const float* f1u, const ds_eval_coef* k1,
                   const float* f2, const float* f2u, const ds_eval_coef* k2,
                   float dt, float c_in_next, size_t n, void* stream);

int ds_karras_churn(float* xhat_out, float* xin_out, const float* x, const float* eps,
                    const uint64_t* philox_state, uint64_t philox_offset,
                    float coef, float c_in, float ratio, float scale, int xin_copies ,
                    size_t n, void* stream);

int ds_karras_denoiser(float* out, const float* x, const float* f, const float* fu, float guidance,
                       float one_minus_guidance,
                       const float* c_out, const float* c_skip, int B, size_t n_per_sample, void* stream);


int ds_inorm_silu(float* out, const float* x, const float* w, const float* b,
                  int B, int C, int HW, float eps, int kind, void* stream);

size_t ds_conv2d_packed_floats(int Cout, int Cin, int ks);
int ds_conv2d_pack_weights(float* packed, const float* w, int Cout, int Cin, int ks, void* stream);

enum { DS_LOAD_PLAIN = 0, DS_LOAD_MAXPOOL2 = 1, DS_LOAD_UPSAMPLE2 = 2, DS_LOAD_AVGPOOL2 = 3 ,
       DS_RES1_UPSAMPLED = 32 ,
       DS_PAD_CIRCULAR = 16  };
#define DS_TAP_OFFSET(oy, ox) ((((oy) & 15) << 8) | (((ox) & 15) << 12))

int ds_conv2d(float* out, const float* in, const float* w_packed, const float* bias,
              const float* shift, int shift_stride, const float* res1, const float* res2,
              int B, int Cin, int Cout, int H, int W, int ks, int load_mode, void* stream);

size_t ds_conv2d_x6_packed_bytes(int Cout, int Cin);
int ds_conv2d_x6_pack_weights(void* packed, const float* w, int Cout, int Cin, void* stream);
int ds_conv2d_x6(float* out, const float* in, const void* w_packed, const float* bias,
                 const float* shift, int shift_stride, const float* res1, const float* res2,
                 int B, int Cin, int Cout, int H, int W, int load_mode, void* stream);

size_t ds_conv2d_h3_packed_bytes(int Cout, int Cin);
int ds_conv2d_h3_pack_weights(void* packed, const float* w, int Cout, int Cin, int wshift, void* stream);
int ds_conv2d_h3(float* out, const float* in, const void* w_packed, int wshift, const float* bias,
                 const float* shift, int shift_stride, const float* res1, const float* res2,
                 int B, int Cin, int Cout, int H, int W, int load_mode,
                 const float* prenorm, float* tile_stats, const unsigned* in_amax, unsigned* out_amax, void* stream);
int ds_absmax_rows(unsigned* out, const float* x, int rows, size_t n_per_row, size_t row_stride, void* stream);
int ds_amax_merge(unsigned* out, const unsigned* a, const unsigned* b , int n, void* stream);
int ds_fill_u32(unsigned* p, unsigned value, size_t n, void* stream);
int ds_absmax_channels(unsigned* out, unsigned* flag, unsigned* scratch, const float* x, const float* wmax, int B, int C,
                       size_t HW, int gap, void* stream);
int ds_input_amax(unsigned* arena, int arena_rows, int out_row, unsigned* flag, const float* x, const float* wmax, int B, int C,
                  size_t HW, int gap, void* stream);
int ds_conv_tile_count(int H, int W);

int ds_inorm_silu_images_supported(int H, int W);
int ds_inorm_silu_images(void* images, const float* x, const float* w, const float* b, int B, int C, int H, int W, float eps,
                         int kind, void* stream);
size_t ds_conv_images_bytes(int B, int C, int H, int W);
int ds_conv2d_h3_img(float* out, const void* images, const void* w_packed, int wshift, const float* bias, const float* shift,
                     int shift_stride, const float* res1, const float* res2, int B, int Cin, int Cout, int H, int W,
                     int flags , float* tile_stats, unsigned* out_amax, void* stream);
int ds_gnorm1_apply_images(void* images, const float* x, const float* stats, const float* w, const float* b,
                           const float* film_scale, const float* film_shift, int film_stride, int B, int C, int Ho, int Wo,
                           int kind, int pool, void* stream);

int ds_table_apply_images(void* images, const float* x, const float* table, int B, int C, int H, int W, void* stream);

int ds_conv2d_h3_up_supported(int Hl, int Wl);
size_t ds_conv2d_h3_up_packed_bytes(int Cout, int Cin);
int ds_conv2d_h3_up_pack_weights(void* packed, const float* w, int Cout, int Cin, int wshift, void* stream);
int ds_conv2d_h3_up(float* out, const float* in, const void* w_packed, int wshift, const float* bias,
                    const float* shift, int shift_stride, const float* res1, const float* res2,
                    int B, int Cin, int Cout, int Hl, int Wl, int flags, const float* prenorm, float* tile_stats,
                    const unsigned* in_amax, unsigned* out_amax, void* stream);
int ds_conv2d_h3_up_img(float* out, const void* images, const void* w_packed, int wshift, const float* bias,
                        const float* shift, int shift_stride, const float* res1, const float* res2,
                        int B, int Cin, int Cout, int Hl, int Wl, float* tile_stats, unsigned* out_amax, void* stream);


int ds_inorm_table(float* table, const float* tile_stats, const float* w, const float* b, int B, int C, int ntiles,
                   int count, float eps, int kind, void* stream);

int ds_gnorm1_table(float* table, const float* stats_a, int Ca, int ntiles_a, const float* stats_b, int Cb,
                    int ntiles_b, const float* w, const float* b, const float* film_scale, const float* film_shift,
                    int film_stride, int B, long long count, float eps, int kind, void* stream);
int ds_gnorm1_stats_tiles(float* stats, const float* stats_a, int Ca, int ntiles_a, const float* stats_b, int Cb,
                          int ntiles_b, int B, long long count, float eps, int kind, void* stream);

int ds_conv2d_direct(float* out, const float* in, const float* w, const float* bias, int B, int Cin, int Cout,
                     int H, int W, int circular, void* stream);

int ds_conv3d_direct(float* out, const float* in, const float* w, const float* bias, const float* shift,
                     int shift_stride, const float* res1, const float* res2, int B, int Cin, int Cout, int D, int H,
                     int W, int load_mode, void* stream);

int ds_volume_to_slices(float* slices, const float* x, int B, int C, int D, size_t HW, int depth_mode, int circular,
                        int pad , void* stream);
int ds_slices_to_volume(float* y, const float* slices, const float* res1, const float* res2, int B, int C, int D,
                        size_t HW, int pad, void* stream);

int ds_volume_stat_tiles(int D, size_t HW);
int ds_volume_to_slices_act(float* slices, const float* x, const float* table, int B, int C, int D, size_t HW, int circular,
                            void* stream);
int ds_wrap_pad_slices(float* slices, int B, int C, int D, size_t HW, void* stream);
int ds_slices_to_volume_stats(float* y, const float* slices, const float* res1, const float* res2, float* stats, int B, int C,
                              int D, size_t HW, int pad, void* stream);
int ds_slice_tables(float* table, const float* tile_stats, const float* w, const float* b, int B, int C, int D, int ntiles,
                    long long count, float eps, int kind, int circular, void* stream);

int ds_avgpool3d(float* out, const float* x, int planes, int Do, int Ho, int Wo, void* stream);
int ds_upsample3d(float* out, const float* x, int planes, int Di, int Hi, int Wi, void* stream);

int ds_avgpool3d_f(float* out, const float* x, int planes, int Di, int Hi, int Wi, int factor, void* stream);
int ds_upsample_f(float* out, const float* x, int planes, int Di, int Hi, int Wi, int factor, int volume, void* stream);

size_t ds_conv1x1_h3_packed_bytes(int Cout, int Cin);
int ds_conv1x1_h3_pack_weights(void* packed, const float* w, int Cout, int Cin, int wshift, void* stream);
int ds_conv1x1_h3(float* out, const float* in, const void* w_packed, int wshift, const float* bias,
                  const float* shift, int shift_stride, const float* res1, const float* res2,
                  int B, int Cin, int Cout, int H, int W, int load_mode, float* tile_stats,
                  const unsigned* in_amax, unsigned* out_amax, int amax_split, void* stream);

int ds_attention(float* out, const float* qkv, int B, int E, int L, void* stream);

int ds_attention_generic(float* out, const float* qkv, int B, int E, int L, void* stream);

int ds_token_l2_normalize(float* x, int B, int Ctot, int c0, int C, int L, float eps, float gain, void* stream);

int ds_attention_h3(float* out, const float* qkv, int B, int E, int L, const unsigned* in_amax, unsigned* out_amax, void* stream);
size_t ds_attention_h3_workspace_bytes(int B, int E, int L);
int ds_attention_h3_ws(float* out, const float* qkv, void* workspace, int B, int E, int L, const unsigned* in_amax,
                       unsigned* out_amax, void* stream);
size_t ds_attention_h3_heads_workspace_bytes(int B, int E, int heads, int L);
int ds_attention_h3_heads(float* out, const float* qkv, void* workspace, int B, int E, int heads, int L, const unsigned* in_amax,
                          unsigned* out_amax, void* stream);
int ds_attention_heads_generic(float* out, const float* qkv, int B, int E, int heads, int L, void* stream);

int ds_linear(float* y, const float* x, const float* w, const float* b, int M, int K, int N, int act, void* stream);

int ds_fourier_features(float* out, const float* t, const float* W, const float* add, int add_rows,
                        int M, int half, void* stream);

int ds_fourier_channels(float* out, const float* x, const float* W, int B, int C, int D, size_t HW, void* stream);


size_t ds_gnorm1_workspace_bytes(int B);
int ds_gnorm1_stats(float* stats, void* workspace, const float* x, int B, int C, int HW, float eps, int kind,
                    void* stream);

int ds_gnorm1_apply(float* out, const float* x, const float* stats, const float* w, const float* b,
                    const float* film_scale, const float* film_shift, int film_stride,
                    int B, int C, int H, int W, int kind, int pool, void* stream);

int ds_gnorm1_apply_poolf(float* out, const float* x, const float* stats, const float* w, const float* b,
                          const float* film_scale, const float* film_shift, int film_stride,
                          int B, int C, int H, int W, int kind, int factor, void* stream);

int ds_concat2(float* out, const float* a, const float* b, int B, size_t na, size_t nb, void* stream);

int ds_add_act(float* out, const float* a, const float* add, int add_rows, int M, int N, int act, void* stream);

int ds_mask_blend(float* out, const float* x, const float* y, const float* mask, size_t n_per_sample, int B,
                  void* stream);

int ds_axpby(float* out, const float* x, float a, const float* y, float b, size_t n, void* stream);
int ds_div_scalar(float* out, const float* x, float s, size_t n, void* stream);

int ds_batchnorm_eval(float* out, const float* x, const float* mean, const float* var, const float* weight,
                      const float* bias, float eps, float sigma, int inverse, int B, int C, int nc, size_t HW,
                      void* stream);

int ds_lerp_stack(float* out, const float* x1, const float* x2, int n, size_t numel, void* stream);

int ds_add(float* out, const float* a, const float* b, size_t n, void* stream);

typedef struct ds_graph ds_graph;
int ds_graph_begin_capture(void* stream);
int ds_graph_end_capture(void* stream, ds_graph** out_graph, int* node_count);
int ds_graph_launch(ds_graph* g, void* stream);
int ds_graph_destroy(ds_graph* g);

#ifdef __cplusplus
}
#endif
#endif
```

Baseline: 83.58.

## Fuse 2x2 max-pool output into last down-block conv epilogue

The persistent conv kernel can now write a 2x2 max-pooled copy of its output, computed with DPP lane exchanges in the store epilogue, when it runs the last residual block of a down level. The downsampler then reads the pooled tensor as a plain input and takes the persistent raw-input path, instead of running the MAXPOOL2 load kernel. This is meant to replace the downsampler's strided full-resolution reads and its slower pooled-load form with a quarter-size read. In exchange it adds an extra store in the epilogue and a new template variant of the kernel, limited to prenorm, non-circular, four-producer shapes.

```diff
diff --git a/diffsci_amd/_native.py b/diffsci_amd/_native.py
--- a/diffsci_amd/_native.py
+++ b/diffsci_amd/_native.py
@@ -10,6 +10,7 @@
 DS_LOAD_PLAIN, DS_LOAD_MAXPOOL2, DS_LOAD_UPSAMPLE2, DS_LOAD_AVGPOOL2 = 0, 1, 2, 3
 DS_PAD_CIRCULAR = 16
 DS_RES1_UPSAMPLED = 32
+DS_PC_RAW = 64
 
 
 class EvalCoef(Structure):
@@ -50,6 +51,8 @@
     "ds_conv2d_h3_packed_bytes": (c_size_t, [c_int, c_int]),
     "ds_conv2d_h3_pack_weights": (c_int, [_P, _P, c_int, c_int, c_int, _P]),
     "ds_conv2d_h3": (c_int, [_P, _P, _P, c_int, _P, _P, c_int, _P, _P, c_int, c_int, c_int, c_int, c_int, c_int, _P, _P, _P, _P, _P]),
+    "ds_conv2d_h3_pool_supported": (c_int, [c_int, c_int, c_int, c_int, c_int, c_int]),
+    "ds_conv2d_h3_pool": (c_int, [_P, _P, _P, _P, c_int, _P, _P, c_int, _P, _P, c_int, c_int, c_int, c_int, c_int, _P, _P, _P, _P]),
     "ds_absmax_rows": (c_int, [_P, _P, c_int, c_size_t, c_size_t, _P]),
     "ds_amax_merge": (c_int, [_P, _P, _P, c_int, _P]),
     "ds_absmax_channels": (c_int, [_P, _P, _P, _P, _P, c_int, c_int, c_size_t, c_int, _P]),
diff --git a/diffsci_amd/csrc/ds_conv3h.hip b/diffsci_amd/csrc/ds_conv3h.hip
--- a/diffsci_amd/csrc/ds_conv3h.hip
+++ b/diffsci_amd/csrc/ds_conv3h.hip
@@ -711,19 +711,21 @@
   return DS_OK;
 }
 
-int ds_conv2d_h3(float* out, const float* in, const void* w_packed, int wshift, const float* bias, const float* shift,
-                 int shift_stride, const float* res1, const float* res2, int B, int Cin, int Cout, int H, int W,
-                 int load_mode, const float* prenorm, float* tile_stats, const unsigned* in_amax, unsigned* out_amax,
-                 void* stream) {
+namespace {
+int conv2d_h3(float* out, float* pool_out, const float* in, const void* w_packed, int wshift, const float* bias, const float* shift,
+              int shift_stride, const float* res1, const float* res2, int B, int Cin, int Cout, int H, int W,
+              int load_mode, const float* prenorm, float* tile_stats, const unsigned* in_amax, unsigned* out_amax,
+              void* stream) {
   DS_REQUIRE(out && in && w_packed, DS_ERR_NULL, "ds_conv2d_h3: NULL pointer");
   DS_REQUIRE(!(prenorm && in_amax), DS_ERR_UNSUPPORTED, "ds_conv2d_h3: in_amax is for raw inputs (with prenorm the table's fourth column carries the exponent)");
   DS_REQUIRE(B >= 0 && Cin > 0 && Cout > 0 && H > 0 && W > 0, DS_ERR_SHAPE,
              "ds_conv2d_h3: bad shape B=%d Cin=%d Cout=%d H=%d W=%d", B, Cin, Cout, H, W);
   const int circular = (load_mode & DS_PAD_CIRCULAR) ? 1 : 0;
   const int res1_up = (load_mode & DS_RES1_UPSAMPLED) ? 1 : 0;
+  const bool raw_pc = (load_mode & DS_PC_RAW) != 0;
   const int oy = (int)((load_mode >> 8) & 15) - (((load_mode >> 8) & 8) ? 16 : 0);
   const int ox = (int)((load_mode >> 12) & 15) - (((load_mode >> 12) & 8) ? 16 : 0);
-  load_mode &= ~(DS_PAD_CIRCULAR | DS_RES1_UPSAMPLED | 0xff00);
+  load_mode &= ~(DS_PAD_CIRCULAR | DS_RES1_UPSAMPLED | DS_PC_RAW | 0xff00);
   DS_REQUIRE(!circular || (H >= (oy < 0 ? -oy : oy) + 1 && W >= (ox < 0 ? -ox : ox) + 1), DS_ERR_SHAPE,
              "ds_conv2d_h3: periodic padding with tap offset (%d, %d) needs a field at least as large as the window's reach (%d x %d)", oy, ox, H, W);
   DS_REQUIRE(!res1_up || (res1 && H % 2 == 0 && W % 2 == 0), DS_ERR_SHAPE, "ds_conv2d_h3: RES1_UPSAMPLED needs res1 and even H, W");
@@ -743,6 +745,7 @@
   Conv3hArgs a;
   a.prenorm = prenorm; a.tile_stats = tile_stats; a.circular = circular; a.res1_up = res1_up; a.oy = oy; a.ox = ox;
   a.ntiles_magic40 = 0; a.ncot_magic40 = 0; a.pc_prio = 0; a.pc_skew_mask = 0;
+  a.pool_out = pool_out;
   {
     static const int early = [] { const char* e = getenv("DS_CONV_TWO_EARLY"); return e ? atoi(e) : 1; }();
     a.two_early = early;
@@ -776,9 +779,10 @@
   hipStream_t s = ds::as_stream(stream);
   if (!w16 && load_mode == DS_LOAD_PLAIN && conv3h_shape16()) {
     bool launched = false;
-    const int rc = conv3p_try_launch(a, s, &launched);
+    const int rc = conv3p_try_launch(a, s, &launched, raw_pc);
     if (rc != DS_OK || launched) return rc;
   }
+  DS_REQUIRE(!pool_out, DS_ERR_UNSUPPORTED, "ds_conv2d_h3_pool: not a launch of the persistent kernel (ds_conv2d_h3_pool_supported)");
 #define DS_L3(M, W) (prenorm ? launch_conv3h<M, W, true>(a, s) : launch_conv3h<M, W, false>(a, s))
   if (w16) {
     if (load_mode == DS_LOAD_PLAIN) return DS_L3(DS_LOAD_PLAIN, true);
@@ -789,6 +793,29 @@
   if (load_mode == DS_LOAD_MAXPOOL2) return launch_conv3h<DS_LOAD_MAXPOOL2, false, false>(a, s);
   return DS_L3(DS_LOAD_UPSAMPLE2, false);
 #undef DS_L3
+}
+}
+
+int ds_conv2d_h3(float* out, const float* in, const void* w_packed, int wshift, const float* bias, const float* shift,
+                 int shift_stride, const float* res1, const float* res2, int B, int Cin, int Cout, int H, int W,
+                 int load_mode, const float* prenorm, float* tile_stats, const unsigned* in_amax, unsigned* out_amax,
+                 void* stream) {
+  return conv2d_h3(out, nullptr, in, w_packed, wshift, bias, shift, shift_stride, res1, res2, B, Cin, Cout, H, W, load_mode, prenorm,
+                   tile_stats, in_amax, out_amax, stream);
+}
+
+int ds_conv2d_h3_pool_supported(int B, int Cin, int Cout, int H, int W, int Cout_next) {
+  return conv3h_shape16() && ds_conv3::conv3p_pool_ok(B, Cin, Cout, H, W, Cout_next) ? 1 : 0;
+}
+
+int ds_conv2d_h3_pool(float* out, float* pooled, const float* in, const void* w_packed, int wshift, const float* bias, const float* shift,
+                      int shift_stride, const float* res1, const float* res2, int B, int Cin, int Cout, int H, int W,
+                      const float* prenorm, float* tile_stats, unsigned* out_amax, void* stream) {
+  DS_REQUIRE(pooled && prenorm, DS_ERR_NULL, "ds_conv2d_h3_pool: NULL pointer");
+  DS_REQUIRE(B > 0 && Cout > 0 && ds_conv2d_h3_pool_supported(B, Cin, Cout, H, W, 0), DS_ERR_UNSUPPORTED,
+             "ds_conv2d_h3_pool: [%d, %d -> %d, %d x %d] is not a shape of the persistent kernel's pooled form", B, Cin, Cout, H, W);
+  return conv2d_h3(out, pooled, in, w_packed, wshift, bias, shift, shift_stride, res1, res2, B, Cin, Cout, H, W, DS_LOAD_PLAIN, prenorm,
+                   tile_stats, nullptr, out_amax, stream);
 }
 
 size_t ds_conv_images_bytes(int B, int C, int H, int W) {
diff --git a/diffsci_amd/csrc/ds_conv3h_args.h b/diffsci_amd/csrc/ds_conv3h_args.h
--- a/diffsci_amd/csrc/ds_conv3h_args.h
+++ b/diffsci_amd/csrc/ds_conv3h_args.h
@@ -59,6 +59,7 @@
   int pc_prio;
   int pc_skew_mask;
   int two_early;
+  float* pool_out;
 #ifdef DS_STAMP
   unsigned long long* stamps;
   unsigned stagger_lo, stagger_hi, stagger_ticks;
@@ -67,7 +68,8 @@
 };
 
 
-int conv3p_try_launch(const Conv3hArgs& a, hipStream_t s, bool* launched);
+int conv3p_try_launch(const Conv3hArgs& a, hipStream_t s, bool* launched, bool raw_pc = false);
+bool conv3p_pool_ok(int B, int Cin, int Cout, int H, int W, int Cout_next);
 int conv3p_try_launch_img(const Conv3hArgs& a, hipStream_t s, bool* launched);
 
 }
diff --git a/diffsci_amd/csrc/ds_conv3p.hip b/diffsci_amd/csrc/ds_conv3p.hip
--- a/diffsci_amd/csrc/ds_conv3p.hip
+++ b/diffsci_amd/csrc/ds_conv3p.hip
@@ -75,11 +75,12 @@
   return ((cptr)p)[i];
 }
 
-template <bool PRE, bool CIRC, int NRES, int NPW, bool VEC = false, bool IMG = false>
+template <bool PRE, bool CIRC, int NRES, int NPW, bool VEC = false, bool IMG = false, bool POOL = false>
 __global__ __launch_bounds__(256 + 64 * NPW, NPW == 4 ? 2 : 3) void k_conv3p(const Conv3hArgs a) {
   static_assert(NPW == 4 || NPW == 8, "four or eight producer waves");
   static_assert(!VEC || NPW == 4, "16-byte patch loads: the four-producer form");
   static_assert(!IMG || (!PRE && !CIRC && !VEC && NPW == 4), "image input: plain zero-padded four-producer form");
+  static_assert(!POOL || (!CIRC && !IMG && NPW == 4), "pooled copy: zero-padded four-producer staging forms");
   constexpr int XI = NPW == 4 ? 3 : 2;
   constexpr int BK = NPW == 4 ? 4 : 2;
   using Packed = ds_conv3::Packed<XI>;
@@ -502,6 +503,7 @@
   int s_b = 0, s_cot = 0, s_tile = 0;
   f32x4 pend0[BK];
   size_t s_idx = 0;
+  size_t s_pidx = 0;
   const size_t s_step = 4 * (size_t)HW;
   float s_amax = 0.f;
   const int p4 = 4 * (lane & 7);
@@ -512,6 +514,7 @@
     const int gy = it.y0 + 2 * rws + ((lane >> 3) & 1), gx = it.x0 + p4;
     const size_t ch = (size_t)it.b * a.Cout + it.cot * COT + 4 * joff + (lane >> 4);
     s_idx = ch * HW + (size_t)gy * a.W + gx;
+    if constexpr (POOL) s_pidx = ch * (size_t)(HW >> 2) + (size_t)(gy >> 1) * (a.W >> 1) + (gx >> 1) + ((lane >> 3) & 1);
     s_amax = 0.f;
   };
   auto res_prefetch = [&](ResRegs& R, int half) __attribute__((always_inline)) {
@@ -541,6 +544,17 @@
     }
 #pragma unroll
     for (int k = 0; k < BK; ++k) *reinterpret_cast<f32x4*>(a.out + s_idx + (size_t)(half * BK + k) * s_step) = v[k];
+    if constexpr (POOL) {
+      const bool bot = (lane & 8) != 0;
+#pragma unroll
+      for (int k = 0; k < BK; ++k) {
+        const float g0 = __builtin_bit_cast(float, __builtin_amdgcn_update_dpp(0, __builtin_bit_cast(int, bot ? v[k].x : v[k].z), 0x128, 0xF, 0xF, true));
+        const float g1 = __builtin_bit_cast(float, __builtin_amdgcn_update_dpp(0, __builtin_bit_cast(int, bot ? v[k].y : v[k].w), 0x128, 0xF, 0xF, true));
+        const float t0 = bot ? g0 : v[k].x, t1 = bot ? g1 : v[k].y;
+        const float b0 = bot ? v[k].z : g0, b1 = bot ? v[k].w : g1;
+        a.pool_out[s_pidx + (size_t)(half * BK + k) * HW] = fmaxf(fmaxf(t0, t1), fmaxf(b0, b1));
+      }
+    }
     if (want_amax) {
 #pragma unroll
       for (int k = 0; k < BK; ++k) s_amax = fmaxf(s_amax, ds_epi::abs_max4(v[k]));
@@ -854,11 +868,11 @@
   return v;
 }
 
-template <bool PRE, bool CIRC, int NRES, int NPW, bool VEC = false, bool IMG = false>
+template <bool PRE, bool CIRC, int NRES, int NPW, bool VEC = false, bool IMG = false, bool POOL = false>
 int launch_conv3p_w(const Conv3hArgs& a, int wgs, hipStream_t s) {
-  const int rc = ds::ensure_dynamic_lds<&k_conv3p<PRE, CIRC, NRES, NPW, VEC, IMG>>(P_LDS, "hipFuncSetAttribute(conv3p)");
+  const int rc = ds::ensure_dynamic_lds<&k_conv3p<PRE, CIRC, NRES, NPW, VEC, IMG, POOL>>(P_LDS, "hipFuncSetAttribute(conv3p)");
   if (rc != DS_OK) return rc;
-  hipLaunchKernelGGL((k_conv3p<PRE, CIRC, NRES, NPW, VEC, IMG>), dim3((unsigned)wgs), dim3(256 + 64 * NPW), P_LDS, s, a);
+  hipLaunchKernelGGL((k_conv3p<PRE, CIRC, NRES, NPW, VEC, IMG, POOL>), dim3((unsigned)wgs), dim3(256 + 64 * NPW), P_LDS, s, a);
   DS_CHECK_LAUNCH("ds_conv2d_h3 (persistent)");
   return DS_OK;
 }
@@ -866,11 +880,13 @@
   static const bool on = [] { const char* e = getenv("DS_CONV_VEC"); return !(e && atoi(e) == 0); }();
   return on;
 }
-template <bool PRE, bool CIRC, int NRES>
+template <bool PRE, bool CIRC, int NRES, bool POOL = false>
 int launch_conv3p_r(const Conv3hArgs& a, int wgs, hipStream_t s) {
-  if (conv3p_producer_waves() == 8) return launch_conv3p_w<PRE, CIRC, NRES, 8>(a, wgs, s);
-  if (conv3p_vec() && a.ox == 0 && (reinterpret_cast<uintptr_t>(a.in) & 15u) == 0) return launch_conv3p_w<PRE, CIRC, NRES, 4, true>(a, wgs, s);
-  return launch_conv3p_w<PRE, CIRC, NRES, 4>(a, wgs, s);
+  if constexpr (!POOL) {
+    if (conv3p_producer_waves() == 8) return launch_conv3p_w<PRE, CIRC, NRES, 8>(a, wgs, s);
+  }
+  if (conv3p_vec() && a.ox == 0 && (reinterpret_cast<uintptr_t>(a.in) & 15u) == 0) return launch_conv3p_w<PRE, CIRC, NRES, 4, true, false, POOL>(a, wgs, s);
+  return launch_conv3p_w<PRE, CIRC, NRES, 4, false, false, POOL>(a, wgs, s);
 }
 void conv3p_fill_args(Conv3hArgs& a) {
   a.ntiles_magic40 = (1ull << 40) / (unsigned long long)(a.tiles_x * a.tiles_y) + 1ull;
@@ -884,6 +900,12 @@
 template <bool PRE, bool CIRC>
 int launch_conv3p(Conv3hArgs a, int wgs, hipStream_t s) {
   conv3p_fill_args(a);
+  if constexpr (PRE && !CIRC) {
+    if (a.pool_out) {
+      if (!a.res1) return launch_conv3p_r<PRE, CIRC, 0, true>(a, wgs, s);
+      return a.res2 ? launch_conv3p_r<PRE, CIRC, 2, true>(a, wgs, s) : launch_conv3p_r<PRE, CIRC, 1, true>(a, wgs, s);
+    }
+  }
   if (!a.res1) return launch_conv3p_r<PRE, CIRC, 0>(a, wgs, s);
   return a.res2 ? launch_conv3p_r<PRE, CIRC, 2>(a, wgs, s) : launch_conv3p_r<PRE, CIRC, 1>(a, wgs, s);
 }
@@ -895,6 +917,10 @@
 int conv3p_min_items() {
   static const int v = [] { const char* e = getenv("DS_CONV_PC_MIN"); const int n = e ? atoi(e) : 1; return n < 1 ? 1 : n; }();
   return v;
+}
+bool conv3p_pool_on() {
+  static const bool on = [] { const char* e = getenv("DS_CONV_PC_POOL"); return !(e && atoi(e) == 0); }();
+  return on;
 }
 int conv3p_cus() {
   static std::atomic<int> cus[64];
@@ -909,6 +935,24 @@
   return c;
 }
 
+bool conv3p_takes(int B, int Cin, int Cout, int H, int W, bool prenorm, bool raw_pc) {
+  const int mode = conv3p_mode();
+  if (mode == 0) return false;
+  if (H % 8 != 0 || W % 32 != 0 || Cout % COT != 0 || Cin % (4 * KC) != 0) return false;
+  const int n_cot = Cout / COT;
+  const long long total = (long long)n_cot * (W / 32) * (H / 8) * B;
+  const int wgs = conv3p_cus() / 8 * 8;
+  if (wgs <= 0 || total < (long long)wgs * conv3p_min_items() || total >= (1ll << 22)) return false;
+  if (n_cot % 2 == 0 && prenorm && mode < 2) return false;
+  if (!prenorm && mode < 3 && !raw_pc) return false;
+  return true;
+}
+
+}
+
+bool conv3p_pool_ok(int B, int Cin, int Cout, int H, int W, int Cout_next) {
+  if (!conv3p_pool_on() || conv3p_producer_waves() != 4 || B <= 0 || H % 16 != 0 || W % 64 != 0) return false;
+  return conv3p_takes(B, Cin, Cout, H, W, true, false) && (Cout_next <= 0 || conv3p_takes(B, Cout, Cout_next, H / 2, W / 2, false, true));
 }
 
 int conv3p_try_launch_img(const Conv3hArgs& a0, hipStream_t s, bool* launched) {
@@ -929,17 +973,12 @@
   return rc;
 }
 
-int conv3p_try_launch(const Conv3hArgs& a, hipStream_t s, bool* launched) {
+int conv3p_try_launch(const Conv3hArgs& a, hipStream_t s, bool* launched, bool raw_pc) {
   *launched = false;
-  const int mode = conv3p_mode();
-  if (mode == 0) return DS_OK;
-  if (a.H % 8 != 0 || a.W % 32 != 0 || a.Cout % COT != 0 || a.Cin % (4 * KC) != 0) return DS_OK;
   if (a.Hin != a.H || a.Win != a.W || a.res1_up) return DS_OK;
-  const long long total = (long long)a.n_cot * a.tiles_x * a.tiles_y * a.B;
+  if (!conv3p_takes(a.B, a.Cin, a.Cout, a.H, a.W, a.prenorm != nullptr, raw_pc)) return DS_OK;
+  if (a.pool_out && (!a.prenorm || a.circular || conv3p_producer_waves() != 4)) return DS_OK;
   const int wgs = conv3p_cus() / 8 * 8;
-  if (wgs <= 0 || total < (long long)wgs * conv3p_min_items() || total >= (1ll << 22)) return DS_OK;
-  if (a.n_cot % 2 == 0 && a.prenorm && mode < 2) return DS_OK;
-  if (!a.prenorm && mode < 3) return DS_OK;
   int rc;
   if (a.prenorm) rc = a.circular ? launch_conv3p<true, true>(a, wgs, s) : launch_conv3p<true, false>(a, wgs, s);
   else rc = a.circular ? launch_conv3p<false, true>(a, wgs, s) : launch_conv3p<false, false>(a, wgs, s);
diff --git a/diffsci_amd/models/nets/punetg.py b/diffsci_amd/models/nets/punetg.py
--- a/diffsci_amd/models/nets/punetg.py
+++ b/diffsci_amd/models/nets/punetg.py
@@ -719,10 +719,12 @@
             return None
         return ws.take((B, C, ops.conv_tile_count(H, W), 4), dev)
 
-    def _res(self, blk, x, shift, pk, ws, res2=None, xs=None, want_stats=True, out_amax=None):
+    def _res(self, blk, x, shift, pk, ws, res2=None, xs=None, want_stats=True, out_amax=None, pool_out=None):
         B, C, H, W = x.shape
         dev = x.device
         if self.extra_residual is not None:
+            if pool_out is not None:
+                raise ValueError("pool_out: not with extra_residual")
             er = self.extra_residual(x)
             ops.require_device(er, "extra_residual output")
             if tuple(er.shape) != tuple(x.shape):
@@ -740,22 +742,33 @@
             return y, None
         if isinstance(shift, _FieldShifts):
             yt = self._field_shift(blk, shift, H, W)
-            got = self._res_body(blk, x, None, yt, pk, ws, res2, xs, want_stats, out_amax)
+            got = self._res_body(blk, x, None, yt, pk, ws, res2, xs, want_stats, out_amax, pool_out)
             ws.give(yt)
             return got
         yt = None
         if shift is not None and shift.dim() == 4:
             yt, shift = self._rescale_shift_field(shift, H, W), None
-        return self._res_body(blk, x, shift, yt, pk, ws, res2, xs, want_stats, out_amax)
-
-    def _res_body(self, blk, x, shift, yt, pk, ws, res2, xs, want_stats, out_amax):
+        return self._res_body(blk, x, shift, yt, pk, ws, res2, xs, want_stats, out_amax, pool_out)
+
+    def _folds(self, C, xs):
+        k1, k2 = self.norm_kinds
+        return (self._fused() and xs is not None and (C + 63) // 64 <= self.fuse_max_cot and k1 != 3 and k2 != 3
+                and self.config.kernel_size == 3)
+
+    def _pool_route(self, blk, x, xs, ds, pk):
+        B, C, H, W = x.shape
+        pd = pk[id(ds)]
+        return (self.extra_residual is None and not self.circular and self._folds(C, xs)
+                and blk.conv2.out_channels == C and pd.kind == "fp16x3" and pd.ks == 3 and pd.subs is None
+                and ops.conv_pool_supported(B, C, C, H, W, ds.out_channels))
+
+    def _res_body(self, blk, x, shift, yt, pk, ws, res2, xs, want_stats, out_amax, pool_out=None):
         B, C, H, W = x.shape
         dev = x.device
         k1, k2 = self.norm_kinds
         w1, b1 = getattr(blk.gnorm1, "weight", None), getattr(blk.gnorm1, "bias", None)
         w2, b2 = getattr(blk.gnorm2, "weight", None), getattr(blk.gnorm2, "bias", None)
-        if (self._fused() and xs is not None and (C + 63) // 64 <= self.fuse_max_cot and k1 != 3 and k2 != 3
-                and self.config.kernel_size == 3):
+        if self._folds(C, xs):
             tab = ws.take((B, ops.table_channels(C), 4), dev)
             ops.inorm_table(xs, w1, b1, k1, H * W, eps=1e-5, out=tab)
             ys = self._stats_buf(ws, B, C, H, W, dev)
@@ -763,11 +776,13 @@
             ops.inorm_table(ys, w2, b2, k2, H * W, eps=1e-5, out=tab)
             os_ = self._stats_buf(ws, B, C, H, W, dev) if want_stats else None
             out = self._conv(blk.conv2, y, pk, res1=x, res2=res2, prenorm=tab, tile_stats=os_, out=ws.take(x.shape, dev),
-                             out_amax=out_amax)
+                             out_amax=out_amax, **({} if pool_out is None else {"pool_out": pool_out}))
             ws.give(y)
             ws.give(ys)
             ws.give(tab)
             return out, os_
+        if pool_out is not None:
+            raise ValueError("pool_out: the folded route only (_pool_route)")
         windowed = k1 in (0, 1) and k2 in (0, 1) and self._norms_in_window(blk)
         if windowed and self._norm_images_ok(blk, C, H, W, k1, k2):
             img = ops.inorm_silu_images(x, w1, b1, k1, eps=1e-5, out=ws.take((ops.conv_images_floats(B, C, H, W),), dev))
@@ -925,21 +940,30 @@
                 ws.give(xe)
             skips = []
             for lv, blocks in enumerate(self.downward_blocks):
+                ds = self.downsamplers[lv].conv
+                pooled = None
                 for j, blk in enumerate(blocks):
-                    ha2 = slot(j == len(blocks) - 1)
+                    last = j == len(blocks) - 1
+                    ha2 = slot(last)
                     nxt = blocks[j + 1] if j + 1 < len(blocks) else None
-                    h2, hs2 = self._res(blk, h, sh(), pk, ws, xs=hs, out_amax=ha2,
+                    if last and h3 and self._pool_route(blk, h, hs, ds, pk):
+                        pooled = ws.take((B, h.shape[1], h.shape[2] // 2, h.shape[3] // 2), dev)
+                    h2, hs2 = self._res(blk, h, sh(), pk, ws, xs=hs, out_amax=ha2, pool_out=pooled,
                                         want_stats=self._consumes_stats(nxt, h.shape[1], h.shape[2], h.shape[3]))
                     give(h, hs)
                     h, hs, ha = h2, hs2, ha2
                 skips.append(h)
                 if hs is not None:
                     ws.give(hs)
-                ds = self.downsamplers[lv].conv
                 Ho, Wo = h.shape[2] // 2, h.shape[3] // 2
                 hs = stats_for(first_block_after_level(lv), ds.out_channels, Ho, Wo)
-                h = self._conv(ds, h, pk, load_mode=DS_LOAD_MAXPOOL2, tile_stats=hs,
-                               out=ws.take((B, ds.out_channels, Ho, Wo), dev), in_amax=amax_of(h, ha))
+                if pooled is not None:
+                    h = self._conv(ds, pooled, pk, pc_raw=True, tile_stats=hs,
+                                   out=ws.take((B, ds.out_channels, Ho, Wo), dev), in_amax=amax_of(h, ha))
+                    ws.give(pooled)
+                else:
+                    h = self._conv(ds, h, pk, load_mode=DS_LOAD_MAXPOOL2, tile_stats=hs,
+                                   out=ws.take((B, ds.out_channels, Ho, Wo), dev), in_amax=amax_of(h, ha))
                 ha = None
             nattn, nafter = len(self.attn_resnet_block), len(self.after_block)
             for j, blk in enumerate(self.before_block):
diff --git a/diffsci_amd/ops.py b/diffsci_amd/ops.py
--- a/diffsci_amd/ops.py
+++ b/diffsci_amd/ops.py
@@ -713,6 +713,8 @@
         return conv2d(x, pw.data, pw.Cout, pw.ks, kind=pw.kind, wshift=pw.wshift, w_up=pw.up, up_wshift=pw.up_wshift, **kw)
     if kw.get("res1_upsampled", False):
         raise NotImplementedError("res1_upsampled with kernels larger than 3x3")
+    if kw.get("pool_out", None) is not None:
+        raise NotImplementedError("pool_out with kernels larger than 3x3")
     stats, out, out_amax = kw.pop("tile_stats", None), kw.pop("out", None), kw.pop("out_amax", None)
     first = dict(bias=kw.pop("bias", None), shift=kw.pop("shift", None), res1=kw.pop("res1", None), res2=kw.pop("res2", None))
     if kw.get("in_amax", None) is None and kw.get("prenorm", None) is None:
@@ -792,9 +794,14 @@
     return stats
 
 
+def conv_pool_supported(B, Cin, Cout, H, W, Cout_next):
+    return bool(N.lib().ds_conv2d_h3_pool_supported(int(B), int(Cin), int(Cout), int(H), int(W), int(Cout_next)))
+
+
 def conv2d(x, w_packed, Cout, ks, bias=None, shift=None, res1=None, res2=None,
            load_mode=N.DS_LOAD_PLAIN, out=None, kind="fp32", wshift=0, prenorm=None, tile_stats=None, circular=False,
-           res1_upsampled=False, w_up=None, up_wshift=0, tap_offset=None, in_amax=None, out_amax=None, amax_split=0):
+           res1_upsampled=False, w_up=None, up_wshift=0, tap_offset=None, in_amax=None, out_amax=None, amax_split=0,
+           pool_out=None, pc_raw=False):
     B, Cin, Hin, Win = x.shape
     if load_mode in (N.DS_LOAD_MAXPOOL2, N.DS_LOAD_AVGPOOL2):
         if Hin % 2 or Win % 2:
@@ -831,6 +838,8 @@
         raise ValueError("bias must have Cout entries")
     if (prenorm is not None or tile_stats is not None) and kind != "fp16x3":
         raise ValueError("prenorm / tile_stats are features of the fp16x3 kernels")
+    if (pool_out is not None or pc_raw) and (kind != "fp16x3" or ks != 3):
+        raise ValueError("pool_out / pc_raw are features of the fp16x3 3x3 convolution")
     pin = pout = None
     if kind == "fp16x3":
         pin = _in_amax(x, in_amax, B, raw=prenorm is None)
@@ -864,10 +873,19 @@
                                         _p(res1), _p(res2), B, Cin, Cout, Hin, Win,
                                         (N.DS_PAD_CIRCULAR if circular else 0) | (N.DS_RES1_UPSAMPLED if res1_upsampled else 0),
                                         _p(prenorm), _p(tile_stats), pin, pout, _stream()), "ds_conv2d_h3_up")
+    elif kind == "fp16x3" and pool_out is not None:
+        if (ks != 3 or load_mode != N.DS_LOAD_PLAIN or prenorm is None or circular or tap or res1_upsampled
+                or tuple(pool_out.shape) != (B, Cout, H // 2, W // 2)):
+            raise ValueError(f"pool_out: a plain zero-padded fp16x3 3x3 convolution with prenorm and pool_out of shape {(B, Cout, H // 2, W // 2)}")
+        require_device(pool_out, "pool_out")
+        N.check(N.lib().ds_conv2d_h3_pool(_p(out), _p(pool_out), _p(x), _p(w_packed), int(wshift), _p(bias), _p(shift), stride,
+                                          _p(res1), _p(res2), B, Cin, Cout, H, W, _p(prenorm), _p(tile_stats), pout,
+                                          _stream()), "ds_conv2d_h3_pool")
     elif kind == "fp16x3":
         N.check(N.lib().ds_conv2d_h3(_p(out), _p(x), _p(w_packed), int(wshift), _p(bias), _p(shift), stride,
                                      _p(res1), _p(res2), B, Cin, Cout, H, W,
-                                     load_mode | tap | (N.DS_PAD_CIRCULAR if circular else 0) | (N.DS_RES1_UPSAMPLED if res1_upsampled else 0),
+                                     load_mode | tap | (N.DS_PAD_CIRCULAR if circular else 0) | (N.DS_RES1_UPSAMPLED if res1_upsampled else 0)
+                                     | (N.DS_PC_RAW if pc_raw else 0),
                                      _p(prenorm), _p(tile_stats), pin, pout,
                                      _stream()), "ds_conv2d_h3")
     elif kind == "bf16x6":
diff --git a/include/diffsci_hip.h b/include/diffsci_hip.h
--- a/include/diffsci_hip.h
+++ b/include/diffsci_hip.h
@@ -79,7 +79,8 @@
 
 enum { DS_LOAD_PLAIN = 0, DS_LOAD_MAXPOOL2 = 1, DS_LOAD_UPSAMPLE2 = 2, DS_LOAD_AVGPOOL2 = 3 ,
        DS_RES1_UPSAMPLED = 32 ,
-       DS_PAD_CIRCULAR = 16  };
+       DS_PAD_CIRCULAR = 16 ,
+       DS_PC_RAW = 64  };
 #define DS_TAP_OFFSET(oy, ox) ((((oy) & 15) << 8) | (((ox) & 15) << 12))
 
 int ds_conv2d(float* out, const float* in, const float* w_packed, const float* bias,
@@ -98,6 +99,11 @@
                  const float* shift, int shift_stride, const float* res1, const float* res2,
                  int B, int Cin, int Cout, int H, int W, int load_mode,
                  const float* prenorm, float* tile_stats, const unsigned* in_amax, unsigned* out_amax, void* stream);
+int ds_conv2d_h3_pool_supported(int B, int Cin, int Cout, int H, int W, int Cout_next);
+int ds_conv2d_h3_pool(float* out, float* pooled, const float* in, const void* w_packed, int wshift, const float* bias,
+                      const float* shift, int shift_stride, const float* res1, const float* res2,
+                      int B, int Cin, int Cout, int H, int W,
+                      const float* prenorm, float* tile_stats, unsigned* out_amax, void* stream);
 int ds_absmax_rows(unsigned* out, const float* x, int rows, size_t n_per_row, size_t row_stride, void* stream);
 int ds_amax_merge(unsigned* out, const unsigned* a, const unsigned* b , int n, void* stream);
 int ds_fill_u32(unsigned* p, unsigned value, size_t n, void* stream);
```

Result: no change. 84.34 (median of 6 runs) (+0.9%).
